# penn-graphics-research/HOT

Measured on AMD Instinct MI355X. Metric: ms per nonlinear (L-BFGS) iteration; P2G+G2P Mparticles/s; achieved HBM GB/s vs roofline, lower is better.
Workload: dtype f64; 1 GPU; C2: one 63^3-cell cube x 8 ppc (63^3 cells per GPU), fixed-corotated E=50000 nu=0.3, dx=0.01, dt=1/24, -lsolver 3 -mg_level 3 -smoother 5 -coarseSolver 2 --project --linesearch --bcproject --usecn -cneps 1e-7; particles_per_gpu=2000376, particles_total=2000376, nodes_total=267566, levels=3, parallelism=1 GPU

## Files before the change

### hot_amd/csrc/force.hip

```cpp
#include "hot_impl.h"
#include "hot_constitutive.h"
#include "hot_collision.h"
#include <cmath>

namespace hot {

template <class T>
__device__ __forceinline__ int tile_slot2(int t, const int32_t* __restrict__ nb8)
{
    using G = Geo<T>;
    constexpr int TY = G::BY + 2, TZ = G::BZ + 2;
    int tz = t % TZ, ty = (t / TZ) % TY, tx = t / (TZ * TY);
    int ox = tx >> G::xb, oy = ty >> G::yb, oz = tz >> G::zb;
    int elem = ((tx & (G::BX - 1)) << (G::yb + G::zb)) | ((ty & (G::BY - 1)) << G::zb) | (tz & (G::BZ - 1));
    return nb8[ox * 4 + oy * 2 + oz] * G::EPB + elem;
}

template <class T>
__global__ void k_hs_flag(const int32_t* __restrict__ id2coord, const double* __restrict__ hs, int nhs, int32_t* flags, int nn, T dx)
{
    int n = blockIdx.x * blockDim.x + threadIdx.x;
    if (n >= nn) return;
    bool inside = false;
    for (int h = 0; h < nhs; ++h) {
// ... 288 lines not shown
                    gv[0] += v0 * g0, gv[1] += v1 * g0, gv[2] += v2 * g0;
                    gv[3] += v0 * g1, gv[4] += v1 * g1, gv[5] += v2 * g1;
                    gv[6] += v0 * g2, gv[7] += v1 * g2, gv[8] += v2 * g2;
                }
            }
        }
        return;
    }
    T gx[3] = { 0, 0, 0 }, gy[3] = { 0, 0, 0 }, gz[3] = { 0, 0, 0 };
#pragma unroll
    for (int i = 0; i < 3; ++i) {
        T a[3] = { 0, 0, 0 }, b[3] = { 0, 0, 0 }, c[3] = { 0, 0, 0 };
#pragma unroll
        for (int j = 0; j < 3; ++j) {
            const int t = t0 + i * sx + j * sy;
            const T v0[3] = { n0[t], n0[t + 1], n0[t + 2] }, v1[3] = { n1[t], n1[t + 1], n1[t + 2] }, v2[3] = { n2[t], n2[t + 1], n2[t + 2] };
            const T s0 = w[2][0] * v0[0] + w[2][1] * v0[1] + w[2][2] * v0[2], d0 = dw[2][0] * v0[0] + dw[2][1] * v0[1] + dw[2][2] * v0[2];
            const T s1 = w[2][0] * v1[0] + w[2][1] * v1[1] + w[2][2] * v1[2], d1 = dw[2][0] * v1[0] + dw[2][1] * v1[1] + dw[2][2] * v1[2];
            const T s2 = w[2][0] * v2[0] + w[2][1] * v2[1] + w[2][2] * v2[2], d2 = dw[2][0] * v2[0] + dw[2][1] * v2[1] + dw[2][2] * v2[2];
            a[0] += w[1][j] * s0, a[1] += w[1][j] * s1, a[2] += w[1][j] * s2;
            b[0] += dw[1][j] * s0, b[1] += dw[1][j] * s1, b[2] += dw[1][j] * s2;
            c[0] += w[1][j] * d0, c[1] += w[1][j] * d1, c[2] += w[1][j] * d2;
        }
#pragma unroll
        for (int q = 0; q < 3; ++q) gx[q] += dw[0][i] * a[q], gy[q] += w[0][i] * b[q], gz[q] += w[0][i] * c[q];
    }
#pragma unroll
    for (int q = 0; q < 3; ++q) gv[q] = one_over_dx * gx[q], gv[3 + q] = one_over_dx * gy[q], gv[6 + q] = one_over_dx * gz[q];
}

template <class T, bool ENERGY_ONLY = false>
__global__ __launch_bounds__(256) __attribute__((amdgpu_waves_per_eu(ENERGY_ONLY ? (sizeof(T) == 8 ? 4 : 6) : (sizeof(T) == 8 ? 3 : 4)))) void k_state(const T* __restrict__ X, const T* __restrict__ Fn, const T* __restrict__ Vol, const T* __restrict__ Mu, const T* __restrict__ Lam,
    T* __restrict__ Ft, T* __restrict__ stress_out, T* __restrict__ gradV_out, int64_t Np, const int32_t* __restrict__ group_first, const int32_t* __restrict__ group_origin,
    const int32_t* __restrict__ group_nb, const int32_t* __restrict__ gIdx, const T* __restrict__ vn, const T* __restrict__ dv, T dx, T one_over_dx, T dt, double* energy, GridRed gr)
{
    using G = Geo<T>;
    constexpr int TY = G::BY + 2, TZ = G::BZ + 2, TILE = (G::BX + 2) * TY * TZ;
    __shared__ T nv[3][TILE];
    __shared__ double red[4];
    const int g = blockIdx.x;
    const int first = group_first[g], last = group_first[g + 1];
    const int p0 = first + threadIdx.x;
    T xpre[3] = { 0, 0, 0 }, fpre[9];
#pragma unroll
    for (int c = 0; c < 9; ++c) fpre[c] = (T)0;
    if (p0 < last) {
#pragma unroll
        for (int d = 0; d < 3; ++d) xpre[d] = X[(int64_t)d * Np + p0];
#pragma unroll
        for (int c = 0; c < 9; ++c) fpre[c] = Fn[(int64_t)c * Np + p0];
    }
    for (int t = threadIdx.x; t < TILE; t += 256) {
        int idx = gIdx[(int64_t)g * TILE + t];
        T a = 0, b = 0, c = 0;
        if (idx >= 0) a = vn[3 * idx] + dv[3 * idx], b = vn[3 * idx + 1] + dv[3 * idx + 1], c = vn[3 * idx + 2] + dv[3 * idx + 2];
        nv[0][t] = a, nv[1][t] = b, nv[2][t] = c;
    }
    __syncthreads();
    const int ox = group_origin[3 * g], oy = group_origin[3 * g + 1], oz = group_origin[3 * g + 2];
    double e = 0, es = 0;
    for (int p = first + threadIdx.x; p < last; p += 256) {
        Mat3<T> Fnew;
        {
            T xp[3];
#pragma unroll
            for (int d = 0; d < 3; ++d) xp[d] = p == p0 ? xpre[d] : X[(int64_t)d * Np + p];
            int base[3];
            T w[3][3], dw[3][3];
#pragma unroll
            for (int d = 0; d < 3; ++d) bspline<T>(one_over_dx, xp[d], base[d], w[d], dw[d]);
            const int cx = base[0] - ox, cy = base[1] - oy, cz = base[2] - oz;
            T gv[9];
            gather_grad(nv[0], nv[1], nv[2], ((cx * TY) + cy) * TZ + cz, TY * TZ, TZ, w, dw, one_over_dx, gv);
            if (gradV_out) {
#pragma unroll
                for (int c = 0; c < 9; ++c) gradV_out[(int64_t)c * Np + p] = gv[c];
            }
            Mat3<T> A, Fo;
#pragma unroll
            for (int c = 0; c < 9; ++c) A.a[c] = dt * gv[c] + ((c % 4 == 0) ? (T)1 : (T)0), Fo.a[c] = p == p0 ? fpre[c] : Fn[(int64_t)c * Np + p];
            Fnew = m3_mul(A, Fo);
        }
        T mu = Mu[p], la = Lam[p];
        T vol = Vol[p];
        if constexpr (ENERGY_ONLY) {
            e += (double)(vol * corotated_psi_sigma(Fnew, mu, la));
            continue;
        }
#pragma unroll
        for (int c = 0; c < 9; ++c) Ft[(int64_t)c * Np + p] = Fnew.a[c];
        T psi, psis;
        Mat3<T> P;
        corotated_state(Fnew, mu, la, psi, P, &psis);
        e += (double)(vol * psi);
        es += (double)(vol * psis);
        asm volatile("" ::: "memory");
#pragma unroll
        for (int c = 0; c < 3; ++c) {
            T f0 = Fn[(int64_t)(0 * 3 + c) * Np + p], f1 = Fn[(int64_t)(1 * 3 + c) * Np + p], f2 = Fn[(int64_t)(2 * 3 + c) * Np + p];
#pragma unroll
            for (int r = 0; r < 3; ++r) stress_out[(int64_t)(c * 3 + r) * Np + p] = vol * (P(r, 0) * f0 + P(r, 1) * f1 + P(r, 2) * f2);
        }
    }
    double tot = block_sum_256<double>(e, red);
    if constexpr (ENERGY_ONLY)
        grid_sum_store(tot, 0.0, 1, gr, energy, nullptr, red);
    else {
        const double tots = block_sum_256<double>(es, red);
        grid_sum_store(tot, tots, 2, gr, energy, energy + 3, red);
    }
}

template <class T, int K>
struct TrialAlphas {
    T a[K];
};
template <class T, int K>
__global__ __launch_bounds__(256) __attribute__((amdgpu_waves_per_eu(3))) void k_state_trials(const T* __restrict__ X, const T* __restrict__ Fn, const T* __restrict__ Vol,
    const T* __restrict__ Mu, const T* __restrict__ Lam, int64_t Np, const int32_t* __restrict__ group_first, const int32_t* __restrict__ group_origin, const int32_t* __restrict__ gIdx,
    const T* __restrict__ vn, const T* __restrict__ dv0, const T* __restrict__ ddv, TrialAlphas<T, K> al, T one_over_dx, T dt, double* energy, GridRed gr)
{
    using G = Geo<T>;
    constexpr int TY = G::BY + 2, TZ = G::BZ + 2, TILE = (G::BX + 2) * TY * TZ;
    __shared__ T nv[2][3][TILE];
    __shared__ double red[4 * K];
    __shared__ double esum[K][256];
    const int g = blockIdx.x;
    const int first = group_first[g], last = group_first[g + 1];
    for (int t = threadIdx.x; t < TILE; t += 256) {
        const int idx = gIdx[(int64_t)g * TILE + t];
        T a = 0, b = 0, c = 0, d0 = 0, d1 = 0, d2 = 0;
        if (idx >= 0) {
            a = vn[3 * idx] + dv0[3 * idx], b = vn[3 * idx + 1] + dv0[3 * idx + 1], c = vn[3 * idx + 2] + dv0[3 * idx + 2];
            d0 = ddv[3 * idx], d1 = ddv[3 * idx + 1], d2 = ddv[3 * idx + 2];
        }
        nv[0][0][t] = a, nv[0][1][t] = b, nv[0][2][t] = c;
        nv[1][0][t] = d0, nv[1][1][t] = d1, nv[1][2][t] = d2;
    }
    __syncthreads();
    const int ox = group_origin[3 * g], oy = group_origin[3 * g + 1], oz = group_origin[3 * g + 2];
#pragma unroll
    for (int k = 0; k < K; ++k) esum[k][threadIdx.x] = 0;
    for (int p = first + threadIdx.x; p < last; p += 256) {
        Mat3<T> A0, A1;
        {
            T xp[3];
#pragma unroll
            for (int d = 0; d < 3; ++d) xp[d] = X[(int64_t)d * Np + p];
            int base[3];
            T w[3][3], dw[3][3];
#pragma unroll
            for (int d = 0; d < 3; ++d) bspline<T>(one_over_dx, xp[d], base[d], w[d], dw[d]);
            const int t0 = (((base[0] - ox) * TY) + (base[1] - oy)) * TZ + (base[2] - oz);
            Mat3<T> Fo;
#pragma unroll
            for (int c = 0; c < 9; ++c) Fo.a[c] = Fn[(int64_t)c * Np + p];
            T gv[9];
            gather_grad(nv[0][0], nv[0][1], nv[0][2], t0, TY * TZ, TZ, w, dw, one_over_dx, gv);
            Mat3<T> A;
#pragma unroll
            for (int c = 0; c < 9; ++c) A.a[c] = dt * gv[c] + ((c % 4 == 0) ? (T)1 : (T)0);
            A0 = m3_mul(A, Fo);
#pragma unroll
            for (int d = 0; d < 3; ++d)
#pragma unroll
                for (int i = 0; i < 3; ++i) asm volatile("" : "+v"(w[d][i]), "+v"(dw[d][i]));
            gather_grad(nv[1][0], nv[1][1], nv[1][2], t0, TY * TZ, TZ, w, dw, one_over_dx, gv);
#pragma unroll
            for (int c = 0; c < 9; ++c) A.a[c] = dt * gv[c];
            A1 = m3_mul(A, Fo);
        }
        const T mu = Mu[p], la = Lam[p], vol = Vol[p];
#pragma unroll 1
        for (int k = 0; k < K; ++k) {
            T ak = al.a[0];
#pragma unroll
            for (int kk = 1; kk < K; ++kk) ak = kk == k ? al.a[kk] : ak;
            Mat3<T> Fk;
#pragma unroll
            for (int c = 0; c < 9; ++c) Fk.a[c] = A0.a[c] + ak * A1.a[c];
            esum[k][threadIdx.x] += (double)(vol * corotated_psi_sigma(Fk, mu, la));
        }
    }
    double e[K];
#pragma unroll
    for (int k = 0; k < K; ++k) e[k] = esum[k][threadIdx.x];
    block_sum_256_n<K>(e, [](int) { return true; }, red);
    grid_sum_store_n<K>(e, [](int k) { return k; }, K, gr, energy, red);
}

template <class T, int K>
__global__ __launch_bounds__(256) void k_inertia_energy_trials(const T* __restrict__ dv0, const T* __restrict__ ddv, TrialAlphas<T, K> al, const T* __restrict__ mass, int nn, T g0, T g1, T g2,
    double* out , GridRed gr, const uint8_t* __restrict__ mask )
{
    __shared__ double red[8 * K];
    double s[2 * K];
#pragma unroll
    for (int k = 0; k < 2 * K; ++k) s[k] = 0;
    const int stride = gridDim.x * 256;
    for (int n0 = blockIdx.x * 256 + threadIdx.x; n0 < nn; n0 += 4 * stride) {
        T b[4][3], d[4][3], m[4];
#pragma unroll
        for (int u = 0; u < 4; ++u) {
            const int n = n0 + u * stride < nn ? n0 + u * stride : n0;
#pragma unroll
            for (int c = 0; c < 3; ++c) b[u][c] = dv0[3 * n + c], d[u][c] = ddv[3 * n + c];
            m[u] = mass[n];
        }
#pragma unroll
        for (int u = 0; u < 4; ++u)
            if (n0 + u * stride < nn && (!mask || mask[n0 + u * stride])) {
#pragma unroll
                for (int k = 0; k < K; ++k) {
                    const T a0 = b[u][0] + d[u][0] * al.a[k], a1 = b[u][1] + d[u][1] * al.a[k], a2 = b[u][2] + d[u][2] * al.a[k];
                    s[k] += (double)((a0 * a0 + a1 * a1 + a2 * a2) * m[u]);
                    s[K + k] += (double)((g0 * a0 + g1 * a1 + g2 * a2) * m[u]);
                }
            }
    }
    block_sum_256_n<2 * K>(s, [](int) { return true; }, red);
    grid_sum_store_n<2 * K>(s, [](int k) { return k; }, 2 * K, gr, out, red);
}

template <class T>
void Ctx<T>::trial_batch(const T* ddv, T alpha, int K, double* Ek_out)
{
    HOT_CHECK(K == 2 || K == 4 || K == 8 || K == 16, HOT_ERR_INVALID, "trial_batch: 2 / 4 / 8 / 16 trials");
    if (halo_mode()) {
        halo_gather(*levels[0], dv0.p);
        halo_gather(*levels[0], const_cast<T*>(ddv));
    }
    constexpr int S0 = 140, S1 = 160;
    const int grid = std::min(div_up(Nn, 1024), 1024);
    auto run = [&](auto kc) {
        constexpr int KK = decltype(kc)::value;
        TrialAlphas<T, KK> al;
        T a = alpha;
        for (int k = 0; k < KK; ++k) al.a[k] = a, a *= (T)0.5;
        GridRed g1 = gred_n(Ng, KK);
        g1.mirror = hscal + S0;
        HOT_LAUNCH(this, KK == 2 ? "state_trials2" : (KK == 4 ? "state_trials4" : (KK == 8 ? "state_trials8" : "state_trials16")), (k_state_trials<T, KK>), Ng, 256, 0, pX.p, pFn.p, pVol.p, pMu.p, pLam.p, Np, group_first.p, group_origin.p, tileDof.p, vn.p, dv0.p, ddv, al, (T)1 / dx, dt,
            dscal.p + S0, g1);
        GridRed g2 = gred_n(grid, 2 * KK);
        g2.mirror = hscal + S1, g2.ticket = hscal + 251, g2.ticket_val = new_ticket();
        HOT_LAUNCH(this, "inertia_trials", (k_inertia_energy_trials<T, KK>), grid, 256, 0, dv0.p, ddv, al, mass.p, Nn, (T)cfg.gravity[0], (T)cfg.gravity[1], (T)cfg.gravity[2], dscal.p + S1, g2, vmask);
    };
    if (K == 2) run(std::integral_constant<int, 2>());
    else if (K == 4) run(std::integral_constant<int, 4>());
    else if (K == 8) run(std::integral_constant<int, 8>());
    else run(std::integral_constant<int, 16>());
    wait_ticket();
    if (sharded()) {
        double buf[48];
        const int nb = halo_mode() ? 3 * K : K;
        for (int k = 0; k < K; ++k) buf[k] = hscal[S0 + k];
        for (int k = 0; k < 2 * K; ++k) buf[K + k] = hscal[S1 + k];
        c_allreduce(buf, nb, HOT_COMM_F64, HOT_COMM_SUM, false);
        for (int k = 0; k < K; ++k) hscal[S0 + k] = buf[k];
        if (halo_mode())
            for (int k = 0; k < 2 * K; ++k) hscal[S1 + k] = buf[K + k];
    }
    for (int k = 0; k < K; ++k) {
        double r = (double)(T)hscal[S0 + k];
        r += hscal[S1 + k] / 2;
        r -= (double)dt * hscal[S1 + K + k];
        Ek_out[k] = r;
    }
}

#ifdef HOT_AB_KERNELS
#include "ab_src/force_ab1.hip"
#endif

#ifdef HOT_AB_KERNELS
#include "ab_src/force_ab2.hip"
#endif

template <class T>
__global__ __launch_bounds__(256) void k_inertia_energy(const T* __restrict__ dv, const T* __restrict__ mass, int nn, T g0, T g1, T g2, double* out, GridRed gr, const uint8_t* __restrict__ mask)
{
    __shared__ double red[4];
    double ke = 0, ge = 0;
    const int stride = gridDim.x * 256;
    for (int n0 = blockIdx.x * 256 + threadIdx.x; n0 < nn; n0 += 4 * stride) {
        T a[4], b[4], c[4], m[4];
#pragma unroll
        for (int u = 0; u < 4; ++u) {
            const int n = n0 + u * stride < nn ? n0 + u * stride : n0;
            a[u] = dv[3 * n], b[u] = dv[3 * n + 1], c[u] = dv[3 * n + 2], m[u] = mass[n];
        }
#pragma unroll
        for (int u = 0; u < 4; ++u)
            if (n0 + u * stride < nn && (!mask || mask[n0 + u * stride])) {
                ke += (double)((a[u] * a[u] + b[u] * b[u] + c[u] * c[u]) * m[u]);
                ge += (double)((g0 * a[u] + g1 * b[u] + g2 * c[u]) * m[u]);
            }
    }
    double k = block_sum_256<double>(ke, red);
    double gg = block_sum_256<double>(ge, red);
    grid_sum_store(k, gg, 2, gr, out, out + 1, red);
}

template <class T>
__global__ __launch_bounds__(256) void k_force_cells2(const T* __restrict__ X, const T* __restrict__ stress, int64_t Np, const int32_t* __restrict__ group_first,
    const int32_t* __restrict__ group_origin, const int32_t* __restrict__ group_cell0, const int32_t* __restrict__ cell_first, T* __restrict__ part, T one_over_dx, T scale)
{
    using G = Geo<T>;
    constexpr int TY = G::BY + 2, TZ = G::BZ + 2, TILE = (G::BX + 2) * TY * TZ, THREADS = 256;
    constexpr int CH = sizeof(T) == 4 ? 512 : 256;
    using AT = AccT<T>;
    __shared__ AT acc[3][TILE];
    __shared__ T sp[12][CH];
    __shared__ int32_t segs[G::EPB + 2];
    __shared__ int32_t nseg;
    const int g = blockIdx.x, tid = threadIdx.x;
    for (int t = tid; t < 3 * TILE; t += THREADS) (&acc[0][0])[t] = (AT)0;
    const int first = group_first[g], last = group_first[g + 1];
    const int c0 = group_cell0[g], c1 = group_cell0[g + 1];
    const int ox = group_origin[3 * g], oy = group_origin[3 * g + 1], oz = group_origin[3 * g + 2];
    for (int ch = first; ch < last; ch += CH) {
        if (tid == 0) nseg = 0;
        __syncthreads();
        for (int l = tid; l < CH && ch + l < last; l += THREADS) {
            const int p = ch + l;
#pragma unroll
            for (int c = 0; c < 9; ++c) sp[c][l] = scale * stress[(int64_t)c * Np + p];
#pragma unroll
            for (int d = 0; d < 3; ++d) sp[9 + d][l] = X[(int64_t)d * Np + p];
        }
        for (int c = c0 + tid; c < c1; c += THREADS) {
            const int s0 = max(cell_first[c], ch), s1 = min(cell_first[c + 1], min(ch + CH, last));
            if (s1 > s0) segs[atomicAdd(&nseg, 1)] = (s0 - ch) | ((s1 - ch) << 16);
        }
        __syncthreads();
        const int ni = nseg * 6;
        for (int it = tid; it < ni; it += THREADS) {
            const int sd = segs[it / 6], j = (it % 6) >> 1, hf = it & 1, s0 = sd & 0xffff, s1 = sd >> 16;
            const int mid = (s0 + s1 + 1) >> 1, l0 = hf ? mid : s0, l1 = hf ? s1 : mid;
            if (l0 >= l1) continue;
            T a[3][3][3];
#pragma unroll
            for (int e = 0; e < 27; ++e) (&a[0][0][0])[e] = (T)0;
            int b0 = 0, b1 = 0, b2 = 0;
            for (int l = l0; l < l1; ++l) {
                T wx[3], dwx[3], wy3[3], dwy3[3], wz[3], dwz[3];
                bspline<T>(one_over_dx, sp[9][l], b0, wx, dwx);
                bspline<T>(one_over_dx, sp[10][l], b1, wy3, dwy3);
                bspline<T>(one_over_dx, sp[11][l], b2, wz, dwz);
                const T wy = j == 0 ? wy3[0] : (j == 1 ? wy3[1] : wy3[2]), dwy = j == 0 ? dwy3[0] : (j == 1 ? dwy3[1] : dwy3[2]);
                T S[9];
#pragma unroll
                for (int c = 0; c < 9; ++c) S[c] = sp[c][l];
#pragma unroll
                for (int i = 0; i < 3; ++i) {
                    const T wi = wx[i], dwi = one_over_dx * dwx[i];
                    const T wij = wi * wy, dwij_i = dwi * wy, dwij_j = wi * one_over_dx * dwy;
#pragma unroll
                    for (int k = 0; k < 3; ++k) {
                        const T g0 = dwij_i * wz[k], g1 = dwij_j * wz[k], g2 = wij * one_over_dx * dwz[k];
                        a[i][k][0] += -(S[0] * g0 + S[3] * g1 + S[6] * g2);
                        a[i][k][1] += -(S[1] * g0 + S[4] * g1 + S[7] * g2);
                        a[i][k][2] += -(S[2] * g0 + S[5] * g1 + S[8] * g2);
                    }
                }
            }
#pragma unroll
            for (int i = 0; i < 3; ++i)
#pragma unroll
                for (int k = 0; k < 3; ++k) {
                    const int t = ((b0 - ox + i) * TY + (b1 - oy + j)) * TZ + (b2 - oz + k);
                    lds_atomic_add(&acc[0][t], (AT)a[i][k][0]), lds_atomic_add(&acc[1][t], (AT)a[i][k][1]), lds_atomic_add(&acc[2][t], (AT)a[i][k][2]);
                }
        }
    }
    __syncthreads();
    T* out = part + (int64_t)g * 3 * TILE;
    for (int t = tid; t < 3 * TILE; t += THREADS) out[t] = (T)(&acc[0][0])[t];
}

template <class T>
__global__ __launch_bounds__(256) void k_force_det(const T* __restrict__ X, const T* __restrict__ stress, int64_t Np, const int32_t* __restrict__ group_first,
    const int32_t* __restrict__ group_origin, const int32_t* __restrict__ group_cell0, const int32_t* __restrict__ cell_first, T* __restrict__ part, T one_over_dx, T scale)
{
    using G = Geo<T>;
    constexpr int TY = G::BY + 2, TZ = G::BZ + 2, TILE = (G::BX + 2) * TY * TZ, THREADS = 256, CH = 256;
    static_assert(TILE <= THREADS, "one thread per tile node");
    using AT = AccT<T>;
    __shared__ T sp[12][CH];
    __shared__ T slab[3][G::EPB][27];
    __shared__ int32_t segs[G::EPB];
    __shared__ int32_t stamp[G::EPB];
    __shared__ int32_t nseg;
    const int g = blockIdx.x, tid = threadIdx.x;
    const int first = group_first[g], last = group_first[g + 1], c0 = group_cell0[g], c1 = group_cell0[g + 1];
    const int ox = group_origin[3 * g], oy = group_origin[3 * g + 1], oz = group_origin[3 * g + 2];
    const int nz = tid % TZ, ny = (tid / TZ) % TY, nx = tid / (TZ * TY);
    AT acc[3] = { (AT)0, (AT)0, (AT)0 };
    if (tid < G::EPB) stamp[tid] = 0;
    for (int ch = first, n = 1; ch < last; ch += CH, ++n) {
        if (tid == 0) nseg = 0;
        __syncthreads();
        for (int l = tid; l < CH && ch + l < last; l += THREADS) {
            const int64_t p = ch + l;
#pragma unroll
            for (int c = 0; c < 9; ++c) sp[c][l] = scale * stress[(int64_t)c * Np + p];
#pragma unroll
            for (int d = 0; d < 3; ++d) sp[9 + d][l] = X[(int64_t)d * Np + p];
        }
        for (int c = c0 + tid; c < c1; c += THREADS) {
            const int s0 = max(cell_first[c], ch), s1 = min(cell_first[c + 1], min(ch + CH, last));
            if (s1 > s0) segs[atomicAdd(&nseg, 1)] = (s0 - ch) | ((s1 - ch) << 16);
        }
        __syncthreads();
        const int ni = nseg * 6;
        for (int it = tid; it < ni; it += THREADS) {
            const int sd = segs[it / 6], j = (it % 6) >> 1, hf = it & 1, s0 = sd & 0xffff, s1 = sd >> 16;
            const int mid = (s0 + s1 + 1) >> 1, l0 = hf ? mid : s0, l1 = hf ? s1 : mid;
            T a[3][3][3];
#pragma unroll
            for (int e = 0; e < 27; ++e) (&a[0][0][0])[e] = (T)0;
            const int b0 = base_node_of<T>(one_over_dx, sp[9][s0]), b1 = base_node_of<T>(one_over_dx, sp[10][s0]), b2 = base_node_of<T>(one_over_dx, sp[11][s0]);
            for (int l = l0; l < l1; ++l) {
                int e0, e1, e2;
                T wx[3], dwx[3], wy3[3], dwy3[3], wz[3], dwz[3];
                bspline<T>(one_over_dx, sp[9][l], e0, wx, dwx);
                bspline<T>(one_over_dx, sp[10][l], e1, wy3, dwy3);
                bspline<T>(one_over_dx, sp[11][l], e2, wz, dwz);
                const T wy = j == 0 ? wy3[0] : (j == 1 ? wy3[1] : wy3[2]), dwy = j == 0 ? dwy3[0] : (j == 1 ? dwy3[1] : dwy3[2]);
                T S[9];
#pragma unroll
                for (int c = 0; c < 9; ++c) S[c] = sp[c][l];
#pragma unroll
                for (int i = 0; i < 3; ++i) {
                    const T wi = wx[i], dwi = one_over_dx * dwx[i];
                    const T wij = wi * wy, dwij_i = dwi * wy, dwij_j = wi * one_over_dx * dwy;
#pragma unroll
                    for (int k = 0; k < 3; ++k) {
                        const T g0 = dwij_i * wz[k], g1 = dwij_j * wz[k], g2 = wij * one_over_dx * dwz[k];
                        a[i][k][0] += -(S[0] * g0 + S[3] * g1 + S[6] * g2);
                        a[i][k][1] += -(S[1] * g0 + S[4] * g1 + S[7] * g2);
                        a[i][k][2] += -(S[2] * g0 + S[5] * g1 + S[8] * g2);
                    }
                }
            }
#pragma unroll
            for (int e = 0; e < 27; ++e) (&a[0][0][0])[e] += dpp_move<0xb1, 0xf>((&a[0][0][0])[e]);
            const int cl = ((b0 - ox) << (G::yb + G::zb)) | ((b1 - oy) << G::zb) | (b2 - oz);
#pragma unroll
            for (int e = 0; e < 27; ++e) {
                const int ik = e / 3, q = e % 3, i = ik / 3, k = ik % 3;
                if ((e < 14) == (hf == 0)) slab[q][cl][(i * 3 + j) * 3 + k] = (&a[0][0][0])[e];
            }
            if (hf == 0 && j == 0) stamp[cl] = n;
        }
        __syncthreads();
        if (tid < TILE) {
#pragma unroll
            for (int i = 0; i < 3; ++i)
#pragma unroll
                for (int j = 0; j < 3; ++j)
#pragma unroll
                    for (int k = 0; k < 3; ++k) {
                        const int cx = nx - i, cy = ny - j, cz = nz - k;
                        if ((unsigned)cx < (unsigned)G::BX && (unsigned)cy < (unsigned)G::BY && (unsigned)cz < (unsigned)G::BZ) {
                            const int cl = (cx << (G::yb + G::zb)) | (cy << G::zb) | cz;
                            if (stamp[cl] == n) {
#pragma unroll
                                for (int q = 0; q < 3; ++q) acc[q] += (AT)slab[q][cl][(i * 3 + j) * 3 + k];
                            }
                        }
                    }
        }
    }
    if (tid < TILE) {
        T* out = part + (int64_t)g * 3 * TILE;
#pragma unroll
        for (int q = 0; q < 3; ++q) out[q * TILE + tid] = (T)acc[q];
    }
}

template <class T>
void Ctx<T>::force_pass()
{
    int64_t slots = (int64_t)Nb * EPB;
    if (cfg.deterministic)
        HOT_LAUNCH(this, "force_scatter_det", k_force_det<T>, Ng, 256, 0, pX.p, pStress.p, Np, group_first.p, group_origin.p, group_cell0.p, cell_first.p, gPart.p, (T)1 / dx, dt);
    else
#ifdef HOT_AB_KERNELS
    if (ab_flag("HOT_FORCE_V1"))
        HOT_LAUNCH(this, "force_scatter", k_force_scatter<T>, Ng, 256, 0, pX.p, pStress.p, Np, group_first.p, group_origin.p, group_nb.p, gPart.p, (T)1 / dx, dt);
    else if (ab_flag("HOT_FORCE_CELLS1"))
        HOT_LAUNCH(this, "force_scatter", k_force_cells<T>, Ng, FORCE_THREADS, 0, pX.p, pStress.p, Np, group_first.p, group_origin.p, group_cell0.p, cell_first.p, gPart.p, (T)1 / dx, dt);
    else
#endif
        HOT_LAUNCH(this, "force_scatter", k_force_cells2<T>, Ng, 256, 0, pX.p, pStress.p, Np, group_first.p, group_origin.p, group_cell0.p, cell_first.p, gPart.p, (T)1 / dx, dt);
    reduce_tiles(3, gF.p, gF.p + slots, gF.p + 2 * slots, nullptr, nullptr, "force_reduce");
    if (halo_mode()) {
        T* arr[3] = { gF.p, gF.p + slots, gF.p + 2 * slots };
        tile_exchange(arr, 3);
    }
    else if (sharded())
        allreduce_tiles(gF.p, 3);
}

template <class T>
double Ctx<T>::state_pass(const T* dv_in, bool want_force, bool energy_only)
{
    if (halo_mode()) halo_gather(*levels[0], const_cast<T*>(dv_in));
    if (energy_only)
        HOT_LAUNCH(this, "state_energy", (k_state<T, true>), Ng, 256, 0, pX.p, pFn.p, pVol.p, pMu.p, pLam.p, (T*)nullptr, (T*)nullptr, (T*)nullptr, Np, group_first.p, group_origin.p,
            group_nb.p, tileDof.p, vn.p, dv_in, dx, (T)1 / dx, dt, dscal.p, gred(Ng, hscal));
    else
        HOT_LAUNCH(this, "state_update", (k_state<T, false>), Ng, 256, 0, pX.p, pFn.p, pVol.p, pMu.p, pLam.p, pFt.p, pStress.p, keep_debug ? pGradV.p : (T*)nullptr, Np, group_first.p, group_origin.p,
            group_nb.p, tileDof.p, vn.p, dv_in, dx, (T)1 / dx, dt, dscal.p, gred2(Ng, hscal, hscal + 3));
    if (want_force) force_pass();
    {
        const int grid = std::min(div_up(Nn, 1024), 1024);
        HOT_LAUNCH(this, "inertia_energy", k_inertia_energy<T>, grid, 256, 0, dv_in, mass.p, Nn, (T)cfg.gravity[0], (T)cfg.gravity[1], (T)cfg.gravity[2], dscal.p + 1, gred(grid, hscal + 1, true), vmask);
    }
    wait_ticket();
    if (energy_only) hscal[3] = hscal[0];
    if (halo_mode())
        c_allreduce(hscal, 4, HOT_COMM_F64, HOT_COMM_SUM, false);
    else if (sharded()) {
        double two[2] = { hscal[0], hscal[3] };
        c_allreduce(two, 2, HOT_COMM_F64, HOT_COMM_SUM, false);
        hscal[0] = two[0], hscal[3] = two[1];
    }
    double result = (double)(T)hscal[0];
    result += hscal[1] / 2;
    result -= (double)dt * hscal[2];
    if (!energy_only) {
        Ek_sigma = (double)(T)hscal[3];
        Ek_sigma += hscal[1] / 2;
        Ek_sigma -= (double)dt * hscal[2];
    }
    return result;
}

template <class T>
void Ctx<T>::update_state(const void* dv_in, double* energy)
{
    need(Nn > 0 && dt > 0, "hot_update_state before hot_begin_step");
    if (dv_in) HOT_HIP(hipMemcpyAsync(dv.p, dv_in, 3 * (size_t)Nn * sizeof(T), hipMemcpyDefault, stream));
    Ek = state_pass(dv.p, true);
    if (energy) *energy = Ek;
}

template <class T>
void Ctx<T>::get_particle_state(void* F, void* stress, void* gradV)
{
    need(Np > 0, "no particles");
    int64_t n = Np;
    DBuf<T> tmp;
    tmp.reserve(9 * n);
    auto out = [&](const T* src, void* dst) {
        if (!dst) return;
        HOT_HIP(hipMemcpyAsync(tmp.p, src, 9 * n * sizeof(T), hipMemcpyDeviceToDevice, stream));
        std::vector<T> h(9 * n), o(9 * n);
        std::vector<int32_t> s2o(n);
        HOT_HIP(hipMemcpyAsync(h.data(), tmp.p, 9 * n * sizeof(T), hipMemcpyDeviceToHost, stream));
        HOT_HIP(hipMemcpyAsync(s2o.data(), slot2orig.p, n * sizeof(int32_t), hipMemcpyDeviceToHost, stream));
        sync();
        for (int64_t p = 0; p < n; ++p)
            for (int c = 0; c < 9; ++c) o[(int64_t)s2o[p] * 9 + c] = h[(int64_t)c * n + p];
        HOT_HIP(hipMemcpy(dst, o.data(), 9 * n * sizeof(T), hipMemcpyDefault));
    };
    out(pFt.p, F), out(pStress.p, stress), out(pGradV.p, gradV);
}

template <class T>
__device__ __forceinline__ void mat3_vec(const T* __restrict__ M, const T* v, T* o)
{
    o[0] = M[0] * v[0] + M[3] * v[1] + M[6] * v[2];
    o[1] = M[1] * v[0] + M[4] * v[1] + M[7] * v[2];
    o[2] = M[2] * v[0] + M[5] * v[1] + M[8] * v[2];
}
template <class T>
__device__ __forceinline__ void bc_project(int c, const T* __restrict__ P, const uint8_t* __restrict__ slip, bool slipmode, T* v)
{
    if (slipmode) {
        if (slip[c])
            v[0] = (T)0;
        else
            v[0] = v[1] = v[2] = (T)0;
    }
    else {
        T o[3];
        mat3_vec(P + 9 * c, v, o);
        v[0] = o[0], v[1] = o[1], v[2] = o[2];
    }
}

template <class T>
__global__ void k_residual(const T* __restrict__ gF, const int32_t* __restrict__ dofSlot, const T* __restrict__ mass, const T* __restrict__ dv, const int32_t* __restrict__ bcIdx,
    const T* __restrict__ bcP, const T* __restrict__ bcR, const uint8_t* __restrict__ bcSlip, T* r, T* r2 , int nn, int64_t slots, T g0, T g1, T g2, T dt, int slipmode)
{
    int n = blockIdx.x * blockDim.x + threadIdx.x;
    if (n >= nn) return;
    int64_t s = dofSlot[n];
    T m = mass[n];
    T v[3] = { g0 * dt * m + gF[s] - dv[3 * n] * m, g1 * dt * m + gF[slots + s] - dv[3 * n + 1] * m, g2 * dt * m + gF[2 * slots + s] - dv[3 * n + 2] * m };
    int c = bcIdx[n];
    if (c >= 0) {
        if (slipmode && bcSlip[c]) {
            T o[3];
            mat3_vec(bcR + 9 * c, v, o);
            v[0] = o[0], v[1] = o[1], v[2] = o[2];
        }
        bc_project(c, bcP, bcSlip, slipmode != 0, v);
    }
    r[3 * n] = v[0], r[3 * n + 1] = v[1], r[3 * n + 2] = v[2];
    r2[3 * n] = v[0], r2[3 * n + 1] = v[1], r2[3 * n + 2] = v[2];
}
template <class T>
__global__ void k_project(const int32_t* __restrict__ bcNode, const T* __restrict__ bcP, const uint8_t* __restrict__ bcSlip, T* v, int nc, int slipmode)
{
    int c = blockIdx.x * blockDim.x + threadIdx.x;
    if (c >= nc) return;
    int n = bcNode[c];
    T x[3] = { v[3 * n], v[3 * n + 1], v[3 * n + 2] };
    bc_project(c, bcP, bcSlip, slipmode != 0, x);
    v[3 * n] = x[0], v[3 * n + 1] = x[1], v[3 * n + 2] = x[2];
}
template <class T>
__global__ void k_transform(const int32_t* __restrict__ bcNode, const T* __restrict__ M, const uint8_t* __restrict__ bcSlip, T* v, int nc)
{
    int c = blockIdx.x * blockDim.x + threadIdx.x;
    if (c >= nc || !bcSlip[c]) return;
    int n = bcNode[c];
    T x[3] = { v[3 * n], v[3 * n + 1], v[3 * n + 2] }, o[3];
    mat3_vec(M + 9 * c, x, o);
    v[3 * n] = o[0], v[3 * n + 1] = o[1], v[3 * n + 2] = o[2];
}

template <class T>
void Ctx<T>::residual_dev(T* r)
{
    int slipmode = (cfg.systemBCProject && cfg.boundaryType == 1) ? 1 : 0;
    HOT_LAUNCH(this, "residual", k_residual<T>, div_up(Nn, 256), 256, 0, gF.p, dofSlot.p, mass.p, dv.p, bcIdx.p, bcP.p, bcR.p, bcSlip.p, r, rhs.p, Nn, (int64_t)Nb * EPB, (T)cfg.gravity[0],
        (T)cfg.gravity[1], (T)cfg.gravity[2], dt, slipmode);
}
template <class T>
void Ctx<T>::project_dev(T* v)
{
    if (Nc == 0) return;
    int slipmode = (cfg.systemBCProject && cfg.boundaryType == 1) ? 1 : 0;
    HOT_LAUNCH(this, "project", k_project<T>, div_up(Nc, 256), 256, 0, bcNode.p, bcP.p, bcSlip.p, v, Nc, slipmode);
}
template <class T>
void Ctx<T>::transform_dev(T* v, bool inverse)
{
    if (Nc == 0 || !(cfg.systemBCProject && cfg.boundaryType == 1)) return;
    HOT_LAUNCH(this, "transform", k_transform<T>, div_up(Nc, 256), 256, 0, bcNode.p, inverse ? bcRinv.p : bcR.p, bcSlip.p, v, Nc);
}

template <class T>
void Ctx<T>::residual(void* r)
{
    need(Nn > 0 && dt > 0, "hot_residual before hot_begin_step/hot_update_state");
    residual_dev(work0.p);
    if (halo_mode()) gather_all(*levels[0], work0.p);
    download(r, work0.p, 3 * (size_t)Nn);
    sync();
}
template <class T>
void Ctx<T>::project(void* v)
{
    need(Nn > 0, "no grid");
    HOT_HIP(hipMemcpyAsync(work0.p, v, 3 * (size_t)Nn * sizeof(T), hipMemcpyDefault, stream));
    project_dev(work0.p);
    download(v, work0.p, 3 * (size_t)Nn);
    sync();
}

template <class T>
__global__ void k_cn_tol(const T* __restrict__ gCN, const int32_t* __restrict__ dofSlot, const T* __restrict__ mass, T* tol, int nn, T scale)
{
    int n = blockIdx.x * blockDim.x + threadIdx.x;
    if (n < nn) tol[n] = gCN[dofSlot[n]] * scale / mass[n];
}
template <class T>
__global__ __launch_bounds__(256) void k_max_dpdf(const T* __restrict__ Mu, const T* __restrict__ Lam, int64_t np, unsigned long long* out)
{
    __shared__ double red[4];
    double mx = 0;
    for (int64_t p = (int64_t)blockIdx.x * 256 + threadIdx.x; p < np; p += (int64_t)gridDim.x * 256) {
        T mu = Mu[p], la = Lam[p];
        double v = (double)hsqrt((T)3 * ((T)2 * mu + la) * ((T)2 * mu + la) + (T)6 * la * la + (T)12 * mu * mu);
        mx = v > mx ? v : mx;
    }
    for (int o = 32; o > 0; o >>= 1) {
        double other = __shfl_xor(mx, o, 64);
        mx = other > mx ? other : mx;
    }
    if ((threadIdx.x & 63) == 0) red[threadIdx.x >> 6] = mx;
    __syncthreads();
    if (threadIdx.x == 0) {
        for (int k = 1; k < 4; ++k) mx = red[k] > mx ? red[k] : mx;
        atomicMax(out, (unsigned long long)__double_as_longlong(mx));
    }
}
template <class T>
void Ctx<T>::cn_tolerance_dev()
{
    T scale = (T)cfg.cneps * 24 * dx * dx * dt;
    HOT_LAUNCH(this, "cn_tolerance", k_cn_tol<T>, div_up(Nn, 256), 256, 0, gCN.p, dofSlot.p, mass.p, cnTol.p, Nn, scale);
    HOT_HIP(hipMemsetAsync(dscal.p + 8, 0, sizeof(double), stream));
    HOT_LAUNCH(this, "max_dpdf_norm", k_max_dpdf<T>, std::min(div_up(Np, 256), 1024), 256, 0, pMu.p, pLam.p, Np, (unsigned long long*)(dscal.p + 8));
    HOT_HIP(hipMemcpyAsync(hscal + 8, dscal.p + 8, sizeof(double), hipMemcpyDeviceToHost, stream));
    sync();
    if (sharded()) c_allreduce(hscal + 8, 1, HOT_COMM_F64, HOT_COMM_MAX, false);
    max_cn_tolerance = (T)cfg.cneps * dt * 24 * (T)std::sqrt((double)Nn) * dx * dx * (T)hscal[8];
}
template <class T>
void Ctx<T>::cn_tolerance(void* tol)
{
    need(Nn > 0 && dt > 0, "hot_cn_tolerance before hot_begin_step");
    need(cfg.useCN, "hot_cn_tolerance needs cfg.useCN (the accumulation is fused into P2G)");
    cn_tolerance_dev();
    if (halo_mode()) gather_all(*levels[0], cnTol.p, 1);
    download(tol, cnTol.p, Nn);
    sync();
}

template <class T>
__global__ __launch_bounds__(256) void k_matfree(const T* __restrict__ X, const T* __restrict__ Fn, const T* __restrict__ Ft, const T* __restrict__ Vol, const T* __restrict__ Mu,
    const T* __restrict__ Lam, int64_t Np, const int32_t* __restrict__ group_first, const int32_t* __restrict__ group_origin, const int32_t* __restrict__ group_nb,
    const int32_t* __restrict__ gIdx, const T* __restrict__ x, T* __restrict__ part, T dx, T one_over_dx, T dt, int project)
{
    using G = Geo<T>;
    constexpr int TY = G::BY + 2, TZ = G::BZ + 2, TILE = (G::BX + 2) * TY * TZ;
    __shared__ T nv[3][TILE];
    using AT = AccT<T>;
    __shared__ AT acc[3][TILE];
    __shared__ int32_t nb8[8];
    const int g = blockIdx.x;
    if (threadIdx.x < 8) nb8[threadIdx.x] = group_nb[g * 8 + threadIdx.x];
    __syncthreads();
    for (int t = threadIdx.x; t < TILE; t += 256) {
        int idx = gIdx[tile_slot2<T>(t, nb8)];
        T a = 0, b = 0, c = 0;
        if (idx >= 0) a = x[3 * idx], b = x[3 * idx + 1], c = x[3 * idx + 2];
        nv[0][t] = a, nv[1][t] = b, nv[2][t] = c;
        acc[0][t] = acc[1][t] = acc[2][t] = (AT)0;
    }
    __syncthreads();
    const int first = group_first[g], last = group_first[g + 1];
    const int ox = group_origin[3 * g], oy = group_origin[3 * g + 1], oz = group_origin[3 * g + 2];
    for (int p = first + threadIdx.x; p < last; p += 256) {
        T xp[3] = { X[p], X[Np + p], X[2 * Np + p] };
        int base[3];
        T w[3][3], dw[3][3];
#pragma unroll
        for (int d = 0; d < 3; ++d) bspline<T>(one_over_dx, xp[d], base[d], w[d], dw[d]);
        const int cx = base[0] - ox, cy = base[1] - oy, cz = base[2] - oz;
        Mat3<T> gx;
#pragma unroll
        for (int c = 0; c < 9; ++c) gx.a[c] = (T)0;
#pragma unroll
        for (int i = 0; i < 3; ++i)
#pragma unroll
            for (int j = 0; j < 3; ++j)
#pragma unroll
                for (int k = 0; k < 3; ++k) {
                    T g0 = one_over_dx * dw[0][i] * w[1][j] * w[2][k], g1 = w[0][i] * one_over_dx * dw[1][j] * w[2][k], g2 = w[0][i] * w[1][j] * one_over_dx * dw[2][k];
                    int t = ((cx + i) * TY + (cy + j)) * TZ + (cz + k);
                    T v0 = nv[0][t], v1 = nv[1][t], v2 = nv[2][t];
                    gx.a[0] += v0 * g0, gx.a[1] += v1 * g0, gx.a[2] += v2 * g0;
                    gx.a[3] += v0 * g1, gx.a[4] += v1 * g1, gx.a[5] += v2 * g1;
                    gx.a[6] += v0 * g2, gx.a[7] += v1 * g2, gx.a[8] += v2 * g2;
                }
        Mat3<T> Fo, Fc;
#pragma unroll
        for (int c = 0; c < 9; ++c) Fo.a[c] = Fn[(int64_t)c * Np + p], Fc.a[c] = Ft[(int64_t)c * Np + p];
        HessBlocks<T> h;
        corotated_hessian(Fc, Mu[p], Lam[p], project != 0, h);
        Mat3<T> dP = hess_apply(h, m3_mul(gx, Fo));
        T vol = Vol[p];
        Mat3<T> S;
#pragma unroll
        for (int c = 0; c < 3; ++c)
#pragma unroll
            for (int r = 0; r < 3; ++r) S(r, c) = vol * (dP(r, 0) * Fo(c, 0) + dP(r, 1) * Fo(c, 1) + dP(r, 2) * Fo(c, 2));
        T sc = dt * dt;
        for (int n = 0; n < 27; ++n) {
            int i = n / 9, j = (n / 3) % 3, k = n % 3;
            T g0 = one_over_dx * dw[0][i] * w[1][j] * w[2][k], g1 = w[0][i] * one_over_dx * dw[1][j] * w[2][k], g2 = w[0][i] * w[1][j] * one_over_dx * dw[2][k];
            int t = ((cx + i) * TY + (cy + j)) * TZ + (cz + k);
            lds_atomic_add(&acc[0][t], (AT)(sc * (S(0, 0) * g0 + S(0, 1) * g1 + S(0, 2) * g2)));
            lds_atomic_add(&acc[1][t], (AT)(sc * (S(1, 0) * g0 + S(1, 1) * g1 + S(1, 2) * g2)));
            lds_atomic_add(&acc[2][t], (AT)(sc * (S(2, 0) * g0 + S(2, 1) * g1 + S(2, 2) * g2)));
        }
    }
    __syncthreads();
    T* out = part + (int64_t)g * 3 * TILE;
    for (int t = threadIdx.x; t < 3 * TILE; t += 256) out[t] = (T)(&acc[0][0])[t];
}
template <class T>
__global__ __launch_bounds__(256) void k_matfree_stress_det(const T* __restrict__ X, const T* __restrict__ Fn, const T* __restrict__ Ft, const T* __restrict__ Vol, const T* __restrict__ Mu,
    const T* __restrict__ Lam, int64_t Np, const int32_t* __restrict__ group_first, const int32_t* __restrict__ group_origin, const int32_t* __restrict__ group_nb,
    const int32_t* __restrict__ gIdx, const T* __restrict__ x, T* __restrict__ out, T one_over_dx, int project)
{
    using G = Geo<T>;
    constexpr int TY = G::BY + 2, TZ = G::BZ + 2, TILE = (G::BX + 2) * TY * TZ;
    __shared__ T nv[3][TILE];
    __shared__ int32_t nb8[8];
    const int g = blockIdx.x;
    if (threadIdx.x < 8) nb8[threadIdx.x] = group_nb[g * 8 + threadIdx.x];
    __syncthreads();
    for (int t = threadIdx.x; t < TILE; t += 256) {
        int idx = gIdx[tile_slot2<T>(t, nb8)];
        T a = 0, b = 0, c = 0;
        if (idx >= 0) a = x[3 * idx], b = x[3 * idx + 1], c = x[3 * idx + 2];
        nv[0][t] = a, nv[1][t] = b, nv[2][t] = c;
    }
    __syncthreads();
    const int first = group_first[g], last = group_first[g + 1];
    const int ox = group_origin[3 * g], oy = group_origin[3 * g + 1], oz = group_origin[3 * g + 2];
    for (int p = first + threadIdx.x; p < last; p += 256) {
        T xp[3] = { X[p], X[Np + p], X[2 * Np + p] };
        int base[3];
        T w[3][3], dw[3][3];
#pragma unroll
        for (int d = 0; d < 3; ++d) bspline<T>(one_over_dx, xp[d], base[d], w[d], dw[d]);
        const int cx = base[0] - ox, cy = base[1] - oy, cz = base[2] - oz;
        Mat3<T> gx;
#pragma unroll
        for (int c = 0; c < 9; ++c) gx.a[c] = (T)0;
#pragma unroll
        for (int i = 0; i < 3; ++i)
#pragma unroll
            for (int j = 0; j < 3; ++j)
#pragma unroll
                for (int k = 0; k < 3; ++k) {
                    T g0 = one_over_dx * dw[0][i] * w[1][j] * w[2][k], g1 = w[0][i] * one_over_dx * dw[1][j] * w[2][k], g2 = w[0][i] * w[1][j] * one_over_dx * dw[2][k];
                    int t = ((cx + i) * TY + (cy + j)) * TZ + (cz + k);
                    T v0 = nv[0][t], v1 = nv[1][t], v2 = nv[2][t];
                    gx.a[0] += v0 * g0, gx.a[1] += v1 * g0, gx.a[2] += v2 * g0;
                    gx.a[3] += v0 * g1, gx.a[4] += v1 * g1, gx.a[5] += v2 * g1;
                    gx.a[6] += v0 * g2, gx.a[7] += v1 * g2, gx.a[8] += v2 * g2;
                }
        Mat3<T> Fo, Fc;
#pragma unroll
        for (int c = 0; c < 9; ++c) Fo.a[c] = Fn[(int64_t)c * Np + p], Fc.a[c] = Ft[(int64_t)c * Np + p];
        HessBlocks<T> h;
        corotated_hessian(Fc, Mu[p], Lam[p], project != 0, h);
        Mat3<T> dP = hess_apply(h, m3_mul(gx, Fo));
        T vol = Vol[p];
#pragma unroll
        for (int c = 0; c < 3; ++c)
#pragma unroll
            for (int r = 0; r < 3; ++r) out[(int64_t)(c * 3 + r) * Np + p] = vol * (dP(r, 0) * Fo(c, 0) + dP(r, 1) * Fo(c, 1) + dP(r, 2) * Fo(c, 2));
    }
}

template <class T>
__global__ void k_matfree_finish(const T* __restrict__ gOut, const int32_t* __restrict__ dofSlot, const T* __restrict__ mass, const T* __restrict__ x, T* y, int nn, int64_t slots)
{
    int n = blockIdx.x * blockDim.x + threadIdx.x;
    if (n >= nn) return;
    int64_t s = dofSlot[n];
    T m = mass[n];
    y[3 * n] = m * x[3 * n] + gOut[s], y[3 * n + 1] = m * x[3 * n + 1] + gOut[slots + s], y[3 * n + 2] = m * x[3 * n + 2] + gOut[2 * slots + s];
}

template <class T>
void Ctx<T>::matfree_dev(const T* x, T* y)
{
    int64_t slots = (int64_t)Nb * EPB;
    DBuf<T>& tile = ap;
    tile.reserve(3 * slots);
    if (halo_mode()) halo_gather(*levels[0], const_cast<T*>(x));
    if (cfg.deterministic) {
        pMfS.reserve(9 * (size_t)Np);
        HOT_LAUNCH(this, "matfree_stress_det", k_matfree_stress_det<T>, Ng, 256, 0, pX.p, pFn.p, pFt.p, pVol.p, pMu.p, pLam.p, Np, group_first.p, group_origin.p, group_nb.p, gIdx.p, x, pMfS.p,
            (T)1 / dx, cfg.project);
        HOT_LAUNCH(this, "matfree_hessian_product_det", k_force_det<T>, Ng, 256, 0, pX.p, pMfS.p, Np, group_first.p, group_origin.p, group_cell0.p, cell_first.p, gPart.p, (T)1 / dx, -dt * dt);
    }
    else
        HOT_LAUNCH(this, "matfree_hessian_product", k_matfree<T>, Ng, 256, 0, pX.p, pFn.p, pFt.p, pVol.p, pMu.p, pLam.p, Np, group_first.p, group_origin.p, group_nb.p, gIdx.p, x, gPart.p, dx,
            (T)1 / dx, dt, cfg.project);
    reduce_tiles(3, tile.p, tile.p + slots, tile.p + 2 * slots, nullptr, nullptr, "matfree_reduce");
    if (halo_mode()) {
        T* arr[3] = { tile.p, tile.p + slots, tile.p + 2 * slots };
        tile_exchange(arr, 3);
    }
    else if (sharded())
        allreduce_tiles(tile.p, 3);
    HOT_LAUNCH(this, "matfree_finish", k_matfree_finish<T>, div_up(Nn, 256), 256, 0, tile.p, dofSlot.p, mass.p, x, y, Nn, slots);
}
template <class T>
void Ctx<T>::matfree_multiply(const void* x, void* y)
{
    need(Nn > 0 && dt > 0, "hot_matfree_multiply before hot_update_state");
    HOT_HIP(hipMemcpyAsync(work0.p, x, 3 * (size_t)Nn * sizeof(T), hipMemcpyDefault, stream));
    matfree_dev(work0.p, work1.p);
    if (halo_mode()) gather_all(*levels[0], work1.p);
    download(y, work1.p, 3 * (size_t)Nn);
    sync();
}

template struct Ctx<float>;
template struct Ctx<double>;

}
```

### hot_amd/csrc/hot_impl.h

```cpp
#pragma once
#include "hot_ctx.h"
#include <atomic>
#include <functional>

namespace hot {

template <class T>
struct GsImg {
    static constexpr size_t hdr_elems = 2 * 64 * 9;
    static constexpr size_t cap_entries = 1340 + 1;
    static constexpr size_t per_dir = cap_entries * 9, per_block = hdr_elems + 2 * per_dir;
    static constexpr size_t idx_per_dir = 64 * 64;
};

struct GsPlan {
    enum Path {
        CHAINED,
        COLOUR,
        PAIR,
        PER_COLOUR,
        SIMPLE,
    } path;
    int sb;
    int nmerge;
// ... 9 lines not shown
template <class T>
__host__ __device__ inline int home_rank(const uint64_t* split, int R, int x, int y, int z, int level)
{
    using G = Geo<T>;
    const uint64_t page = G::linear_offset((x & ~3) << level, (y & ~3) << level, (z & ~3) << level) >> 12;
    int r = 0;
    while (r < R - 1 && page >= split[r]) ++r;
    return r;
}

template <class T>
struct Level {
    int n = 0;
    int id = 0;
    bool built = false;
    long long nnzb = 0;
    DBuf<int32_t> coord;
    DBuf<int32_t> col;
    DBuf<T> val;
    DBuf<T> diagVal, diagInv;
    DBuf<T> diagBlockInv;
    DBuf<uint32_t> ckey;
    DBuf<int32_t> gs_order;
    DBuf<int32_t> gs_block_start;
    double lMin = 1e-8, lMax = 1e2;
    DBuf<T> apv;
    DBuf<int32_t> apc;
    DBuf<int32_t> gs_pad;
    DBuf<int32_t> gs_col;
    DBuf<T> gs_img;
    DBuf<uint16_t> gs_imgi;
    DBuf<T> gs_p1;
    DBuf<int2> gs_slot;
    int gs_nslot = 0;
    int32_t gs_slot_rng[2][2][8] = {};
    DBuf<int32_t> gs_rowpn;
    DBuf<int4> gs_srec;
    int32_t gs_slot_rng2[4][2][8] = {};
    bool gs_fused_ready = false;
    bool gs_img_ready = false;
    long long gs_img_shift[8] = {};
    DBuf<T> gs_w;
    bool gs_w_ready = false;
    DBuf<int32_t> rowcnt;
    bool split = false;
    DBuf<int32_t> ic_col, ic_rowcnt, ic_pad;
    DBuf<T> ic_val, ic_l, ic_d, ic_dinv, ic_dinvT;
    bool ic_ready = false;
    double ic_shift = 0;
    int color_block_begin[9] = { 0 };
    int nblocks = 0;
    DBuf<int32_t> pcol;
    DBuf<T> pw;
    DBuf<int32_t> child;
    DBuf<uint64_t> hkeys;
    DBuf<unsigned long long> hrank;
    DBuf<int32_t> hid;
    HashMap map;
    DBuf<T> residual, initialResidual, sol, du, dAu, tmp;
    bool colored = false;
    bool part = false;
    std::vector<int> nstart;
    DBuf<uint8_t> owner;
    DBuf<uint8_t> own;
    DBuf<uint8_t> block_owner;
    std::vector<uint8_t> block_owner_h;
    std::vector<int> csplit;
    std::pair<int, int> colour_run(int c, int rank, int ranks) const
    {
        const int b0 = color_block_begin[c];
        if (!part) return { b0, color_block_begin[c + 1] };
        return { b0 + csplit[c * (ranks + 1) + rank], b0 + csplit[c * (ranks + 1) + rank + 1] };
    }
    std::vector<int> xbeg, xcnt;
    DBuf<int32_t> dxtab;
    int xmax_full = 0, xmax_col[8] = { 0 };
    const uint8_t* mask() const { return part ? own.p : nullptr; }
    DBuf<T> gsD, gsDinv, gsE;
    bool l1 = false;
    const T* gs_d() const { return l1 ? gsD.p : diagVal.p; }
    const T* gs_dinv() const { return l1 ? gsDinv.p : diagBlockInv.p; }
    struct Halo {
        bool built = false;
        std::vector<int64_t> scnt, soff, rcnt, roff;
        std::vector<int64_t> scol, rcol;
        DBuf<int32_t> send, recv;
        DBuf<uint8_t> need;
        int64_t stot = 0, rtot = 0;
    } halo;
};

template <class T>
struct Ctx : CtxBase {
    using G = Geo<T>;
    static constexpr int EPB = G::EPB;
    static constexpr int TX = G::BX + 2, TY = G::BY + 2, TZ = G::BZ + 2, TILE = TX * TY * TZ;

    T dx = 0, dt = 0;
    int64_t Np = 0;
    DBuf<T> pX, pV, pM, pC, pF, pVol, pMu, pLam, pJp, pFn, pFt, pStress, pGradV;
    DBuf<int32_t> slot2orig;
    DBuf<int32_t> pGid;
    DBuf<int32_t> pCls;
    bool have_cls = false;
    int ncls = 0;
    hot_plasticity_class cls_host[16] = {};
    DBuf<T> clsTab;
    void clear_plasticity_classes() { have_cls = false, ncls = 0; }
    int32_t max_particle_class(int32_t* min_out);
    void reserve_particles(int64_t n);
    void migrate_particles();
    void set_particle_ids(const int32_t* ids) override;
    void get_particle_ids(int32_t* ids) override;
    DBuf<T> spare1, spare3, spare9;
    DBuf<int32_t> sparei;
    bool keep_debug = true;
    DBuf<uint64_t> keys, keys2;
    DBuf<uint32_t> vals, vals2;
    DBuf<char> sort_tmp;
    size_t sort_tmp_bytes = 0;
    DBuf<int32_t> flags, scan;
    DBuf<char> scan_tmp;
    size_t scan_tmp_bytes = 0;
    int Ng = 0, Nb = 0, Nn = 0;
    DBuf<int32_t> group_first;
    DBuf<uint64_t> group_page;
    DBuf<int32_t> group_nb;
    DBuf<int32_t> group_origin;
    DBuf<uint64_t> blocks;
    DBuf<uint64_t> bh_keys;
    DBuf<unsigned long long> bh_rank;
    DBuf<int32_t> bh_id;
    HashMap block_map;
    int Ncell = 0;
    DBuf<int32_t> cell_first;
    DBuf<int32_t> group_cell0;
    DBuf<uint64_t> ch_keys;
    DBuf<unsigned long long> ch_rank;
    DBuf<int32_t> ch_id;
    HashMap cell_map;
    DBuf<T> pMfS;
    DBuf<T> pDP;
    void build_cell_table();
    void matfree_diagonal(T* dinv);
    void assemble_tiles(Level<T>& L);
    void assemble_rows(Level<T>& L);
    void build_gs_winv(Level<T>& L);
    DBuf<int32_t> tile_tab;
    DBuf<int32_t> block_group;
    DBuf<int32_t> block_rev;
    DBuf<T> gPart;
    void reduce_tiles(int Q, T* o0, T* o1, T* o2, T* o3, T* o4, const char* name);
    DBuf<T> gM, gMV, gF, gCN;
    DBuf<int32_t> gIdx;
    DBuf<int32_t> tileDof;
    DBuf<int32_t> block_count;
    DBuf<int32_t> dofSlot, id2coord, bcIdx;
    DBuf<T> mass, vn, dv, dv0, cnTol, nodeV;
    int Nc = 0;
    DBuf<int32_t> bcNode;
    DBuf<T> bcP, bcR, bcRinv, bcDv;
    DBuf<uint8_t> bcSlip, bcHasDv;
    std::vector<double> hs_origin, hs_normal;
    std::vector<hot_collision_object> cobjs;
    DBuf<char> d_cobjs;
    DBuf<double> d_hs;
    double Ek = 0, Ek_sigma = 0;
    bool updated = false;
    int ls_prev_trials = 1;
    T max_cn_tolerance = 0;
    DBuf<T> rhs, work0, work1, work2, work3, solve_keep;
    hot_comm comm{};
    bool sharded() const { return comm.size > 1; }
    std::vector<int> block_first;
    std::vector<uint64_t> page_split;
    std::vector<int> nstart0;
    DBuf<char> xsend, xrecv;
    DBuf<uint8_t> written;
    void set_comm(const hot_comm* c) override;
    void write_partio(const char* path) override;
    void write_restart(const char* path) override;
    void read_restart(const char* path) override;
    void c_allreduce(void* buf, int64_t n, int dtype, int op, bool on_device);
    void c_allgather(const void* send, void* recv, int64_t bytes, bool on_device);
    void c_alltoallv(const void* send, const int64_t* soff, const int64_t* sbytes, void* recv, const int64_t* roff, const int64_t* rbytes);
    void merge_block_lists();
    void color_level(Level<T>& L);
    void level_ownership(Level<T>& L);
    void exchange(Level<T>& L, T* x, int colour, int ncomp = 3);
    void exchange_rows(Level<T>& L, const uint8_t* touched);
    void allreduce_tiles(T* tiles, int q);
    bool halo_mode() const { return sharded() && !cfg.shard_replicated; }
    int64_t comm_calls = 0, comm_calls_index = 0, comm_bytes_index = 0, comm_bytes_data = 0;
    bool comm_index_phase = false;
    struct IndexPhase {
        Ctx<T>* c;
        bool old;
        IndexPhase(Ctx<T>* c_) : c(c_), old(c_->comm_index_phase) { c->comm_index_phase = true; }
        ~IndexPhase() { c->comm_index_phase = old; }
    };
    const char* comm_tag = "other";
    struct CommTag {
        Ctx<T>* c;
        const char* old;
        CommTag(Ctx<T>* c_, const char* t) : c(c_), old(c_->comm_tag) { c->comm_tag = t; }
        ~CommTag() { c->comm_tag = old; }
    };
    void account(int64_t bytes)
    {
        ++comm_calls, comm_calls_index += comm_index_phase ? 1 : 0, (comm_index_phase ? comm_bytes_index : comm_bytes_data) += bytes;
        if (prof.on) {
            auto& r = prof.recs[std::string("commMB_") + (comm_index_phase ? "index" : comm_tag)];
            r.calls++, r.ms += (double)bytes * 1e-6;
        }
    }
    void export_comm_stats() { stats.comm_calls = comm_calls, stats.comm_calls_index = comm_calls_index, stats.comm_bytes_index = comm_bytes_index, stats.comm_bytes_data = comm_bytes_data; }
    DBuf<uint8_t> touch;
    DBuf<uint64_t> sharers;
    DBuf<int32_t> tpos;
    DBuf<int32_t> tlist;
    std::vector<int64_t> tcnt, toff;
    void build_tile_plan();
    void tile_exchange(T* const* arrays, int q);
    void build_halo(Level<T>& L, const std::function<void(uint8_t*)>& mark_extra);
    void halo_gather(Level<T>& L, T* x, int colour = -1, int ncomp = 3);
    void gather_colour(Level<T>& L, T* x, int colour, int ncomp);
    void gather_all(Level<T>& L, T* x, int ncomp = 3);
    void replicate_numbering();
    void level0_ownership();
    void mark_stencil(Level<T>& L, uint8_t* need);
    const uint8_t* vmask = nullptr;
    struct MaskScope {
        Ctx<T>* c;
        const uint8_t* old;
        MaskScope(Ctx<T>* c_, const uint8_t* m) : c(c_), old(c_->vmask) { c->vmask = m; }
        ~MaskScope() { c->vmask = old; }
    };
    void reduce_scalars(double* dev, int n)
    {
        if (!vmask || n <= 0) return;
        CommTag tag(this, "scalars");
        c_allreduce(dev, n, HOT_COMM_F64, HOT_COMM_SUM, true);
    }
    static constexpr int REAL = sizeof(T) == 4 ? HOT_COMM_F32 : HOT_COMM_F64;
    DBuf<double> dscal;
    DBuf<T> speed_part;
    DBuf<double> red_part;
    DBuf<unsigned> red_count;
    GridRed gred(size_t grid, double* mirror = nullptr, bool ticket = false)
    {
        if (2 * grid > red_part.cap) {
            HOT_HIP(hipStreamSynchronize(stream));
            red_part.reserve(2 * grid, 1.5);
        }
        GridRed g{ red_part.p, red_count.p, mirror, nullptr, 0.0 };
        if (ticket) g.ticket = hscal + 251, g.ticket_val = new_ticket();
        return g;
    }
    GridRed gred2(size_t grid, double* mirror, double* mirror1)
    {
        GridRed g = gred(grid, mirror);
        g.mirror1 = mirror1;
        return g;
    }
    GridRed gred_n(size_t grid, int nv)
    {
        if ((size_t)nv * grid > red_part.cap) {
            HOT_HIP(hipStreamSynchronize(stream));
            red_part.reserve((size_t)nv * grid, 1.5);
        }
        return GridRed{ red_part.p, red_count.p, nullptr, nullptr, 0.0 };
    }
    double last_ticket = 0;
    double new_ticket() { return last_ticket += 1.0; }
    void wait_ticket()
    {
        const double want = last_ticket;
        volatile double* t = hscal + 251;
        const double t0 = wall_ms();
        for (unsigned spin = 0; *t != want; ++spin) {
            __builtin_ia32_pause();
            if ((spin & 1023u) == 1023u && wall_ms() - t0 > 20.0) {
                HOT_HIP(hipStreamSynchronize(stream));
                if (*(volatile int*)(hscal + 250) != 0) sync();
                HOT_CHECK(*t == want, HOT_ERR_DEVICE, "a reduction launch did not deliver its result");
                break;
            }
        }
        std::atomic_thread_fence(std::memory_order_acquire);
        if (*(volatile int*)(hscal + 250) != 0) sync();
    }
    DBuf<uint64_t> col_hk;
    DBuf<unsigned long long> col_hr;
    DBuf<int32_t> col_hi, col_cb;
    bool cg_bar_dirty = false;
    DBuf<double> cg_dep;
    unsigned cg_phase = 0;
    int cg_G = 0;
    bool attr_cg_set = false;
    int cg_group = 2;
    bool attr_tiles_set = false, attr_rows_set = false, attr_rows_det_set = false, attr_gs_set = false, attr_winv_set = false;
    double* hscal = nullptr;
    DBuf<T> hist_dx[9], hist_dg[9];
    std::vector<Level<T>*> levels;
    std::vector<Level<T>*> level_pool[12];
    Level<T>* acquire_level(int id)
    {
        Level<T>* l;
        if (!level_pool[id].empty()) {
            l = level_pool[id].back();
            level_pool[id].pop_back();
        }
        else
            l = new Level<T>();
        l->id = id, l->n = 0, l->nnzb = 0, l->nblocks = 0, l->built = false, l->split = false, l->part = false, l->colored = false, l->halo.built = false, l->ic_ready = false;
        return l;
    }
    void release_levels(size_t keep = 0)
    {
        while (levels.size() > keep) {
            Level<T>* l = levels.back();
            levels.pop_back();
            level_pool[l->id < 12 ? l->id : 11].push_back(l);
        }
    }
    DBuf<T> ap;
    std::vector<Ctx<T>*> gmg;
    DBuf<int32_t> orig2slot;
    Ctx<T>* build_gmg_grid(int level);

    Ctx(const hot_config& c);
    ~Ctx();
    template <class U>
    void upload(DBuf<U>& dst, const void* src, size_t n)
    {
        dst.reserve(n);
        if (n) HOT_HIP(hipMemcpyAsync(dst.p, src, n * sizeof(U), hipMemcpyDefault, stream));
    }
    template <class U>
    void download(void* dst, const U* src, size_t n)
    {
        if (dst && n) HOT_HIP(hipMemcpyAsync(dst, src, n * sizeof(U), hipMemcpyDefault, stream));
    }
    static constexpr int ERR_RETRY = -100;
    static constexpr int REARM_STEPS = 32, MAX_TIMEOUTS = 3;
    bool gs_no_chain = false, gs_chain_timed_out = false;
    int gs_timeouts = 0, steps_since_timeout = 0;
    void rearm_chain()
    {
        if (!gs_chain_timed_out || gs_timeouts >= MAX_TIMEOUTS || ++steps_since_timeout < REARM_STEPS) return;
        gs_chain_timed_out = false, steps_since_timeout = 0;
        if (!sharded()) gs_no_chain = false;
    }
    int n_cu = 0;
    int device_cus()
    {
        if (n_cu == 0) {
            int dev = 0;
            HOT_HIP(hipGetDevice(&dev));
            HOT_HIP(hipDeviceGetAttribute(&n_cu, hipDeviceAttributeMultiprocessorCount, dev));
        }
        return n_cu;
    }
    int unset_level = -1;
    int retry_scope = 0, fake_syncs = 0;
    void sync()
    {
        HOT_HIP(hipStreamSynchronize(stream));
        if (retry_scope > 0 && !gs_no_chain && ab_int("HOT_GS_FAKE_TIMEOUT", 0) > 0 && ++fake_syncs == ab_int("HOT_GS_FAKE_TIMEOUT", 0)) *(volatile int*)(hscal + 250) = 1;
        if (*(volatile int*)(hscal + 250) != 0) {
            *(volatile int*)(hscal + 250) = 0;
            cg_bar_dirty = true;
            ++gs_timeouts, steps_since_timeout = 0;
            if (cfg.deterministic) {
                if (gs_timeouts > MAX_TIMEOUTS)
                    throw Error{ HOT_ERR_DEVICE, "deterministic mode: a chained Gauss-Seidel sweep or persistent PCG timed out more than 3 times on this context; the launch-per-pass fallback would change the bits, so the operation fails" };
                throw Error{ ERR_RETRY, "k_gs_sweep: wait on a neighbouring block timed out; deterministic mode: redoing the operation with the same launch structure" };
            }
            gs_no_chain = gs_chain_timed_out = true;
            throw Error{ ERR_RETRY, "k_gs_sweep: wait on a neighbouring block timed out; redoing the operation with one launch per pass" };
        }
    }
    template <class Fn>
    void with_gs_retry(Fn&& fn)
    {
        struct Scope {
            int& n;
            Scope(int& n_) : n(n_) { ++n; }
            ~Scope() { --n; }
        } scope(retry_scope);
        for (;;) {
            try {
                fn();
                return;
            }
            catch (const Error& e) {
                if (e.code != ERR_RETRY) throw;
                if (!cfg.deterministic) break;
            }
        }
        fn();
    }
    int32_t exclusive_scan_i32(const int32_t* in, int32_t* out, size_t n);
    void need(bool cond, const char* what) { HOT_CHECK(cond, HOT_ERR_INVALID, what); }

    void set_particles(int64_t Np, const void* X, const void* V, const void* mass, const void* C, const void* F, const void* vol, const void* mu, const void* lambda, const void* Jp) override;
    void get_particles(void* X, void* V, void* C, void* F, void* mu, void* lambda, void* Jp) override;
    void sort() override;
    void get_counts(int64_t* Np, int32_t* Ng, int32_t* Nb, int32_t* Nn) override;
    void get_indexing(int32_t* order, uint64_t* base_offset, int32_t* group, uint64_t* block_offset, uint64_t* blocks) override;
    void p2g() override;
    void get_grid(int32_t* id2coord, void* mass, void* v) override;
    void set_bc(int32_t Nc, const int32_t* node_id, const void* P, const void* R, const void* Rinv, const uint8_t* slip, const void* dvc) override;
    void set_halfspaces(int32_t n, const double* origin, const double* normal) override;
    void set_collision_objects(int32_t n, const hot_collision_object* objs) override;
    void begin_step(double dt) override;
    void get_dv(void* dv) override;
    void set_dv(const void* dv) override;
    void update_state(const void* dv, double* energy) override;
    void get_particle_state(void* F, void* stress, void* gradV) override;
    void residual(void* r) override;
    void project(void* v) override;
    void cn_tolerance(void* tol) override;
    void build_hessian() override;
    void matfree_multiply(const void* x, void* y) override;
    void build_mg() override;
    void get_level(int32_t level, int32_t* nrows, int32_t* colsize, int32_t* id2coord) override;
    void get_matrix(int32_t level, int32_t* entryCol, void* entryVal) override;
    long long get_level_nnzb(int32_t level) override
    {
        need(level >= 0 && level < (int)levels.size(), "level out of range");
        if (levels[level]->nnzb < 0) count_nnzb(*levels[level]);
        return levels[level]->nnzb;
    }
    long long get_level_inblock_nnzb(int32_t level) override
    {
        need(level >= 0 && level < (int)levels.size() && levels[level]->split, "hot_get_level_inblock_nnzb: level out of range or not coloured (hot_build_mg)");
        Level<T>& L = *levels[level];
        std::vector<int32_t> rc(4 * (size_t)L.n);
        HOT_HIP(hipMemcpyAsync(rc.data(), L.rowcnt.p, rc.size() * sizeof(int32_t), hipMemcpyDeviceToHost, stream));
        sync();
        long long tot = 0;
        for (int i = 0; i < L.n; ++i) tot += rc[4 * (size_t)i + 1] + rc[4 * (size_t)i + 2];
        return tot;
    }
    void get_prolongation(int32_t level, int32_t* entryCol, void* weight) override;
    void spmv(int32_t level, const void* x, void* y) override;
    void restrict_(int32_t level, const void* fine, void* coarse) override;
    void prolong(int32_t level, const void* coarse, void* fine) override;
    void smooth(int32_t level, int32_t kind, int32_t iterations, double tol, void* u, void* r, const void* r0) override;
    void vcycle(const void* in, void* out) override;
    void solve(hot_stats* st) override;
    void g2p(double dt, int32_t* flags) override;
    void constitutive_eval(int32_t n, const void* F, const void* mu, const void* lambda, int32_t project, void* psi, void* P, void* dPdF) override;
    void plasticity_eval(int32_t kind, int32_t n, void* F, void* mu, void* lambda, void* Jp) override;
    void set_plasticity_classes(int32_t n, const hot_plasticity_class* classes, const int32_t* particle_class) override;
    void get_plasticity_classes(int32_t* n, hot_plasticity_class* classes, int32_t* particle_class) override;
    void plasticity_eval_classes(int32_t n, void* F, void* mu, void* lambda, void* Jp, const int32_t* cls) override;
    void advance(double dt, hot_stats* st) override;
    void calculate_dt(double max_dt, double* dt, double* max_speed, double* min_corner, double* max_corner) override;
    void advance_frame(double frame_dt, double min_dt, double max_dt, int32_t* substeps, int32_t* iterations_total, hot_stats* st) override;

    void eval_halfspaces();
    void eval_collision_objects();
    void trial_batch(const T* ddv, T alpha, int K, double* Ek_out);
    double state_pass(const T* dv_in, bool want_force, bool energy_only = false);
    void force_pass();
    void residual_dev(T* r);
    void project_dev(T* v);
    void transform_dev(T* v, bool inverse);
    void cn_tolerance_dev();
    void build_diagonal(Level<T>& L);
    void build_ic(Level<T>& L);
    void count_nnzb(Level<T>& L);
    std::string lname(const char* base, int level) { return std::string(base) + "_L" + std::to_string(level); }
    void spmv_dev(Level<T>& L, const T* x, T* y);
    void scale_dev(Level<T>& L, const T* in, T* out);
    void block_apply_dev(const T* D, const T* in, T* out, int n);
    void estimate_2norm(Level<T>& L, double tol);
    int minres_dev(const std::function<void(const T*, T*)>& Amul, const std::function<void(const T*, T*)>& prec, T* x, const T* b, T relative_tolerance, T tolerance, int max_iterations);
    void scal(size_t n, T a, T* x);
    int smoother_kind(int level, bool top = false) const;
    GsPlan gs_plan(const Level<T>& L) const;
    GsBuild gs_build(const Level<T>& L) const;
    bool gs_marks_wanted(int level) const;
    void restrict_dev(int level, const T* fine, T* coarse, T* zero_coarse = nullptr);
    void prolong_dev(int level, const T* coarse, T* fine);
    void smooth_dev(int level, int kind, int iterations, T tol, T* u, T* r, T* du, T* dAu, bool final_residual = true);
    void gs_smooth_dev(int level, int iterations, T* u, T* r, T* du, T* dAu, bool final_residual, bool tmp_marked);
    void ic_smooth_dev(Level<T>& L, T* u, T* r, T* dAu);
    void vcycle_dev(const T* in, T* out);
    void precondition_dev(const T* in, T* out);
    void matfree_dev(const T* x, T* y);
    void axpy(size_t n, T a, const T* x, T* y);
    void axpy_dev(size_t n, const double* a, double sign, const T* x, T* y);
    void copy(size_t n, const T* x, T* y);
    void zero(size_t n, T* y);
    void dot_to(size_t n, const T* x, const T* y, double* out, double* mirror = nullptr);
    double dot_host(size_t n, const T* x, const T* y);
    bool should_exit(const T* r);
    T line_search(T* ddv, T* residual_out, T alpha);
    bool lbfgs_solve();
    bool newton_solve();
    void compute_step_dev(const T* residual, T* step);
    DBuf<T> nw_step, nw_r, nw_p, nw_q, nw_t, nw_diag;
    void line_search_api(void* ddv, void* residual, double alpha, double* alpha_out) override;
    void should_exit_api(const void* residual, int32_t* exit_now, double* scaled) override;
    void transform_api(void* v, bool inverse) override;
    void compute_step_api(const void* residual, void* step) override;
};

inline int div_up(size_t a, size_t b) { return (int)((a + b - 1) / b); }

__device__ __forceinline__ int xcd_block() { return (int)((blockIdx.x & 7) * (gridDim.x >> 3) + (blockIdx.x >> 3)); }
static inline int xcd_grid(int nwg) { return 8 * div_up(nwg, 8); }
template <class U>
__device__ __forceinline__ U nt_load(const U* p)
{
    return *p;
}
template <class T>
struct GsUnset;
template <>
struct GsUnset<double> {
    static constexpr unsigned long long bits = 0x7ff4dead0badf00dull;
    static __device__ __forceinline__ bool is(double v) { return (unsigned long long)__double_as_longlong(v) == bits; }
};
template <>
struct GsUnset<float> {
    static constexpr unsigned bits = 0x7fa0f00du;
    static __device__ __forceinline__ bool is(float v) { return (unsigned)__float_as_int(v) == bits; }
};
template <class T>
__device__ __forceinline__ void gs_store_unset(T* p)
{
    if constexpr (sizeof(T) == 8)
        *(unsigned long long*)p = GsUnset<double>::bits;
    else
        *(unsigned*)p = GsUnset<float>::bits;
}
template <class T>
__global__ void k_gs_fill_unset(size_t n, T* x);

#define HOT_LAUNCH(ctx, name, kernel, grid, block, shmem, ...)                       \
    do {                                                                             \
        (ctx)->prof.begin(name, (ctx)->stream);                                      \
        hipLaunchKernelGGL(kernel, dim3(grid), dim3(block), shmem, (ctx)->stream, __VA_ARGS__); \
        (ctx)->prof.end((ctx)->stream);                                              \
    } while (0)

}
```

### hot_amd/csrc/mg_solve.hip

```cpp
#include "hot_impl.h"
#include "hot_svd.h"

namespace hot {

template <class T>
__global__ void k_axpy(size_t n, T a, const T* __restrict__ x, T* y)
{
    size_t i = (size_t)blockIdx.x * blockDim.x + threadIdx.x;
    if (i < n) y[i] += a * x[i];
}
template <class T>
__global__ void k_axpy_dev(size_t n, const double* a, double sign, const T* __restrict__ x, T* y)
{
    size_t i = (size_t)blockIdx.x * blockDim.x + threadIdx.x;
    T s = (T)(sign * (*a));
    if (i < n) y[i] += s * x[i];
}
template <class T>
__global__ void k_xpay_dev(size_t n, const double* a, const T* __restrict__ x, T* y)
{
    size_t i = (size_t)blockIdx.x * blockDim.x + threadIdx.x;
    T s = (T)(*a);
    if (i < n) y[i] = x[i] + s * y[i];
}
template <class T>
__global__ __launch_bounds__(256) void k_dot(size_t n, const T* __restrict__ x, const T* __restrict__ y, double* out, GridRed gr, const uint8_t* __restrict__ mask)
{
    __shared__ double red[4];
    double s = 0;
    const size_t stride = (size_t)gridDim.x * 256;
    for (size_t i0 = (size_t)blockIdx.x * 256 + threadIdx.x; i0 < n; i0 += 4 * stride) {
        T xv[4], yv[4];
        bool on[4];
#pragma unroll
        for (int u = 0; u < 4; ++u) {
            const size_t i = i0 + u * stride, ic = i < n ? i : i0;
            on[u] = i < n && (!mask || mask[ic / 3]);
            xv[u] = on[u] ? x[ic] : (T)0, yv[u] = on[u] ? y[ic] : (T)0;
        }
#pragma unroll
        for (int u = 0; u < 4; ++u)
            if (on[u]) s += (double)(xv[u] * yv[u]);
    }
    double t = block_sum_256<double>(s, red);
    grid_sum_store(t, 0.0, 1, gr, out, nullptr, red);
}
template <class T>
void Ctx<T>::axpy(size_t n, T a, const T* x, T* y)
{
    HOT_LAUNCH(this, "axpy", k_axpy<T>, div_up(n, 256), 256, 0, n, a, x, y);
}
template <class T>
void Ctx<T>::axpy_dev(size_t n, const double* a, double sign, const T* x, T* y)
{
    HOT_LAUNCH(this, "axpy", k_axpy_dev<T>, div_up(n, 256), 256, 0, n, a, sign, x, y);
}
template <class T>
__global__ __launch_bounds__(256) void k_copy(size_t n, const T* __restrict__ x, T* __restrict__ y)
{
    for (size_t i = (size_t)blockIdx.x * 256 + threadIdx.x; i < n; i += (size_t)gridDim.x * 256) y[i] = x[i];
}
template <class T>
__global__ __launch_bounds__(256) void k_vcycle_start(size_t n, const T* __restrict__ x, T* __restrict__ y, T* __restrict__ y2, T* __restrict__ z)
{
    for (size_t i = (size_t)blockIdx.x * 256 + threadIdx.x; i < n; i += (size_t)gridDim.x * 256) {
        const T v = x[i];
        y[i] = v, z[i] = (T)0;
        if (y2) y2[i] = v;
    }
}
template <class T>
void Ctx<T>::copy(size_t n, const T* x, T* y)
{
    if (n) HOT_LAUNCH(this, "copy", k_copy<T>, (int)std::min<size_t>(div_up(n, 256), 2048), 256, 0, n, x, y);
}
template <class T>
void Ctx<T>::zero(size_t n, T* y)
{
    HOT_HIP(hipMemsetAsync(y, 0, n * sizeof(T), stream));
}
template <class T>
void Ctx<T>::dot_to(size_t n, const T* x, const T* y, double* out, double* mirror)
{
    const int grid = std::min(div_up(n, 1024), 256);
    if (vmask) {
        HOT_LAUNCH(this, "dot", k_dot<T>, grid, 256, 0, n, x, y, out, gred(grid), vmask);
        reduce_scalars(out, 1);
        if (mirror) HOT_HIP(hipMemcpyAsync(mirror, out, sizeof(double), hipMemcpyDeviceToHost, stream));
        return;
    }
    HOT_LAUNCH(this, "dot", k_dot<T>, grid, 256, 0, n, x, y, out, gred(grid, mirror), (const uint8_t*)nullptr);
}
template <class T>
double Ctx<T>::dot_host(size_t n, const T* x, const T* y)
{
    const int grid = std::min(div_up(n, 1024), 256);
    HOT_LAUNCH(this, "dot", k_dot<T>, grid, 256, 0, n, x, y, dscal.p + 100, gred(grid, hscal + 100, true), vmask);
    wait_ticket();
    if (vmask) c_allreduce(hscal + 100, 1, HOT_COMM_F64, HOT_COMM_SUM, false);
    return hscal[100];
}

template <class T>
__global__ __launch_bounds__(256) void k_spmv(const int32_t* __restrict__ col, const T* __restrict__ val, const T* __restrict__ x, T* __restrict__ y, int n, const uint8_t* __restrict__ own)
{
    const int lane = threadIdx.x & 63;
    const int row = xcd_block() * 4 + (threadIdx.x >> 6);
    if (row >= n || (own && !own[row])) return;
    const int32_t* c = col + (int64_t)row * 125;
    const T* v = val + (int64_t)row * 1125;
    T s0 = 0, s1 = 0, s2 = 0;
#pragma unroll
    for (int r = 0; r < 2; ++r) {
        int k = lane + 64 * r;
        if (k < 125) {
            int j = c[k];
            const T* b = v + k * 9;
            T x0 = x[3 * (int64_t)j], x1 = x[3 * (int64_t)j + 1], x2 = x[3 * (int64_t)j + 2];
            s0 += b[0] * x0 + b[3] * x1 + b[6] * x2;
            s1 += b[1] * x0 + b[4] * x1 + b[7] * x2;
            s2 += b[2] * x0 + b[5] * x1 + b[8] * x2;
        }
    }
    s0 = wave_sum(s0), s1 = wave_sum(s1), s2 = wave_sum(s2);
    if (lane == 0) y[3 * (int64_t)row] = s0, y[3 * (int64_t)row + 1] = s1, y[3 * (int64_t)row + 2] = s2;
}
template <class T>
__global__ __launch_bounds__(256) void k_apmv_sub(const int32_t* __restrict__ apc, const T* __restrict__ apv, const T* __restrict__ e, T* __restrict__ r, int n, const uint8_t* __restrict__ own,
    T* unset )
{
    const int lane = threadIdx.x & 63;
    const int row = xcd_block() * 4 + (threadIdx.x >> 6);
    if (row >= n) return;
    if (unset && lane < 3) gs_store_unset(unset + 3 * (int64_t)row + lane);
    if (own && !own[row]) return;
    const int j = nt_load(apc + (int64_t)row * 64 + lane);
    const int slot = __popcll(__ballot(j >= 0) & ((1ull << lane) - 1ull));
    T s0 = (T)0, s1 = (T)0, s2 = (T)0;
    if (j >= 0) {
        const T* bp = apv + ((int64_t)row * 64 + slot) * 9;
        T b[9];
#pragma unroll
        for (int t = 0; t < 9; ++t) b[t] = nt_load(bp + t);
        const T x0 = e[3 * (int64_t)j], x1 = e[3 * (int64_t)j + 1], x2 = e[3 * (int64_t)j + 2];
        s0 = b[0] * x0 + b[3] * x1 + b[6] * x2;
        s1 = b[1] * x0 + b[4] * x1 + b[7] * x2;
        s2 = b[2] * x0 + b[5] * x1 + b[8] * x2;
    }
    s0 = wave_sum(s0), s1 = wave_sum(s1), s2 = wave_sum(s2);
    if (lane == 0) r[3 * (int64_t)row] -= s0, r[3 * (int64_t)row + 1] -= s1, r[3 * (int64_t)row + 2] -= s2;
}
__device__ __forceinline__ bool cg_active(double zTr, double tol) { return !(zTr < tol); }
template <class T>
__global__ void k_cg_setup(double* s, double* hm)
{
    const double tol = (double)(T)(s[7] * 0.25);
    s[8] = tol;
    s[1] = s[2] = s[3] = s[4] = s[5] = s[6] = s[9] = 0.0;
    hm[0] = s[0], hm[1] = 0.0, hm[2] = tol;
}
template <class T>
__global__ __launch_bounds__(256) void k_cg_spmv_dot(const int32_t* __restrict__ col, const T* __restrict__ val, const T* __restrict__ du, T* __restrict__ dAu, int n, double* s, GridRed gr)
{
    __shared__ double red[4];
    const bool roll = s[6] != 0.0;
    const double cur = roll ? s[4] : s[0];
    if (blockIdx.x == 0 && threadIdx.x == 0 && roll) s[0] = s[4];
    if (!cg_active(cur, s[8])) return;
    const int lane = threadIdx.x & 63;
    const int row = blockIdx.x * 4 + (threadIdx.x >> 6);
    double part = 0;
    if (row < n) {
        const int32_t* c = col + (int64_t)row * 125;
        const T* v = val + (int64_t)row * 1125;
        T s0 = 0, s1 = 0, s2 = 0;
#pragma unroll
        for (int r = 0; r < 2; ++r) {
            int k = lane + 64 * r;
            if (k < 125) {
                int j = c[k];
                const T* b = v + k * 9;
                T x0 = du[3 * (int64_t)j], x1 = du[3 * (int64_t)j + 1], x2 = du[3 * (int64_t)j + 2];
                s0 += b[0] * x0 + b[3] * x1 + b[6] * x2;
                s1 += b[1] * x0 + b[4] * x1 + b[7] * x2;
                s2 += b[2] * x0 + b[5] * x1 + b[8] * x2;
            }
        }
        s0 = wave_sum(s0), s1 = wave_sum(s1), s2 = wave_sum(s2);
        if (lane == 0) {
            dAu[3 * (int64_t)row] = s0, dAu[3 * (int64_t)row + 1] = s1, dAu[3 * (int64_t)row + 2] = s2;
            part = (double)(s0 * du[3 * (int64_t)row]) + (double)(s1 * du[3 * (int64_t)row + 1]) + (double)(s2 * du[3 * (int64_t)row + 2]);
        }
    }
    if (lane == 0) red[threadIdx.x >> 6] = part;
    __syncthreads();
    const double t = threadIdx.x == 0 ? red[0] + red[1] + red[2] + red[3] : 0.0;
    __syncthreads();
    grid_sum_store(t, 0.0, 1, gr, s + 1, nullptr, red);
}
template <class T>
__global__ __launch_bounds__(256) void k_cg_update(const T* __restrict__ Dinv, const T* __restrict__ du, const T* __restrict__ dAu, T* __restrict__ u, T* __restrict__ r, T* __restrict__ z, int n, double* s, GridRed gr)
{
    __shared__ double red[4];
    const int i = blockIdx.x * 256 + threadIdx.x;
    if (!cg_active(s[0], s[8])) return;
    const double omega = s[0] / s[1];
    const T wp = (T)omega, wm = (T)(-omega);
    double part = 0;
    if (i < n) {
        T rr[3];
#pragma unroll
        for (int c = 0; c < 3; ++c) {
            u[3 * (int64_t)i + c] += wp * du[3 * (int64_t)i + c];
            rr[c] = r[3 * (int64_t)i + c] + wm * dAu[3 * (int64_t)i + c];
            r[3 * (int64_t)i + c] = rr[c];
        }
        const T* d = Dinv + 9 * (int64_t)i;
        const T z0 = d[0] * rr[0] + d[3] * rr[1] + d[6] * rr[2], z1 = d[1] * rr[0] + d[4] * rr[1] + d[7] * rr[2], z2 = d[2] * rr[0] + d[5] * rr[1] + d[8] * rr[2];
        z[3 * (int64_t)i] = z0, z[3 * (int64_t)i + 1] = z1, z[3 * (int64_t)i + 2] = z2;
        part = (double)(z0 * rr[0]) + (double)(z1 * rr[1]) + (double)(z2 * rr[2]);
    }
    const double t = block_sum_256<double>(part, red);
    grid_sum_store(t, 0.0, 1, gr, s + 4, nullptr, red);
}
template <class T>
__global__ void k_cg_direction(size_t n3, const T* __restrict__ z, T* __restrict__ du, double* s, double* hm, double* ticket, double ticket_val)
{
    const size_t i = (size_t)blockIdx.x * blockDim.x + threadIdx.x;
    const bool act = cg_active(s[0], s[8]);
    if (act && i < n3) du[i] = z[i] + (T)(s[4] / s[0]) * du[i];
    if (i == 0) {
        if (act) {
            s[6] = 1.0;
            const double cnt = s[9] + 1.0;
            s[9] = cnt;
            hm[0] = s[4], hm[1] = cnt;
        }
        if (ticket) host_ticket_store(ticket, ticket_val);
    }
}
template <class T, int RPW = 0>
__global__ __launch_bounds__(1024) void k_cg_persist(const int32_t* __restrict__ col, const T* __restrict__ val, const T* __restrict__ Dinv, const T* __restrict__ init, T* __restrict__ u,
    T* __restrict__ r, T* __restrict__ z, T* du, T* __restrict__ dAu, int n, int max_iters, unsigned phase0 , double* dep , int SS , double* hm, double* ticket, double ticket_val,
    int* err )
{
    __shared__ double red[32], sres[2];
    __shared__ int s_bail;
    enum { CG_DI = 0, CG_U = 9, CG_R = 12, CG_Z = 15, CG_D = 18, CG_AD = 21 };
    __shared__ T cg_row[RPW > 0 ? 16 : 1][RPW > 0 ? RPW : 1][24];
    const int tid = threadIdx.x, lane = tid & 63, w = __builtin_amdgcn_readfirstlane(tid >> 6);
    const int G = gridDim.x, wg = blockIdx.x;
    unsigned phase = phase0;
    if (tid == 0) s_bail = 0;
    auto ldu = [&](int64_t j, int c) { return __hip_atomic_load(du + 3 * j + c, __ATOMIC_RELAXED, __HIP_MEMORY_SCOPE_AGENT); };
    auto sdu = [&](int64_t j, int c, T v) { __hip_atomic_store(du + 3 * j + c, v, __ATOMIC_RELAXED, __HIP_MEMORY_SCOPE_AGENT); };
    auto all_sum = [&](double v0, double v1, double& o0, double& o1) -> bool {
        asm volatile("s_waitcnt vmcnt(0)" ::: "memory");
        if (lane == 0) red[w] = v0, red[16 + w] = v1;
        __syncthreads();
        double* d = dep + (size_t)(phase & 3u) * G * SS;
        if (tid == 0) {
            double t0 = 0, t1 = 0;
            for (int k = 0; k < 16; ++k) t0 += red[k], t1 += red[16 + k];
            double* dn = dep + (size_t)((phase + 2u) & 3u) * G * SS + (size_t)wg * SS;
            __hip_atomic_store((unsigned long long*)dn, GsUnset<double>::bits, __ATOMIC_RELAXED, __HIP_MEMORY_SCOPE_AGENT);
            __hip_atomic_store((unsigned long long*)(dn + 1), GsUnset<double>::bits, __ATOMIC_RELAXED, __HIP_MEMORY_SCOPE_AGENT);
            __hip_atomic_store(d + (size_t)wg * SS, t0, __ATOMIC_RELAXED, __HIP_MEMORY_SCOPE_AGENT);
            __hip_atomic_store(d + (size_t)wg * SS + 1, t1, __ATOMIC_RELAXED, __HIP_MEMORY_SCOPE_AGENT);
        }
        if (w < 2) {
            const double* dv = d + w;
            double a = 0;
            int spins = 0, bail = 0;
            for (;;) {
                bool all = true;
                a = 0;
                for (int k = lane; k < G; k += 64) {
                    const double x = __hip_atomic_load(dv + (size_t)k * SS, __ATOMIC_RELAXED, __HIP_MEMORY_SCOPE_AGENT);
                    all = all && !GsUnset<double>::is(x);
                    a += x;
                }
                if (__all(all)) break;
                __builtin_amdgcn_s_sleep(1);
                if (++spins > (1 << 21) || ((spins & 255) == 0 && *(volatile int*)err)) {
                    *(volatile int*)err = 1;
                    bail = 1;
                    break;
                }
            }
            a = wave_sum(a);
            if (lane == 0) {
                sres[w] = a;
                if (bail) s_bail = 1;
            }
        }
        __syncthreads();
        if (s_bail) return false;
        o0 = wave_first(sres[0]), o1 = wave_first(sres[1]);
        ++phase;
        return true;
    };
    auto scale = [&](int64_t i, const T (&v)[3], T (&o)[3]) {
        const T* d = Dinv + 9 * i;
        o[0] = d[0] * v[0] + d[3] * v[1] + d[6] * v[2], o[1] = d[1] * v[0] + d[4] * v[1] + d[7] * v[2], o[2] = d[2] * v[0] + d[5] * v[1] + d[8] * v[2];
    };
    const int stride = 16 * G;
    if constexpr (RPW > 0) {
        int rowq[RPW];
        int32_t mc[RPW][2];
        T mv[RPW][2][9];
        double p0 = 0, p1 = 0;
#pragma unroll
        for (int q = 0; q < RPW; ++q) {
            const int row = wg * 16 + w + q * stride;
            rowq[q] = row < n ? row : -1;
            const int64_t rc = row < n ? row : 0;
#pragma unroll
            for (int h = 0; h < 2; ++h) {
                const int k = min(lane + 64 * h, 124);
                mc[q][h] = col[rc * 125 + k];
#pragma unroll
                for (int e = 0; e < 9; ++e) mv[q][h][e] = (lane + 64 * h < 125) ? val[rc * 1125 + k * 9 + e] : (T)0;
            }
            if (lane == 0) {
                T* st = cg_row[w][q];
                T di[9], a[3], za[3], rr[3], zz[3];
#pragma unroll
                for (int e = 0; e < 9; ++e) di[e] = Dinv[9 * rc + e], st[CG_DI + e] = di[e];
#pragma unroll
                for (int c = 0; c < 3; ++c) a[c] = init[3 * rc + c], rr[c] = r[3 * rc + c], st[CG_U + c] = u[3 * rc + c], st[CG_AD + c] = (T)0;
#pragma unroll
                for (int c = 0; c < 3; ++c) za[c] = di[c] * a[0] + di[3 + c] * a[1] + di[6 + c] * a[2], zz[c] = di[c] * rr[0] + di[3 + c] * rr[1] + di[6 + c] * rr[2];
                if (rowq[q] >= 0) {
                    p0 += (double)(za[0] * a[0]) + (double)(za[1] * a[1]) + (double)(za[2] * a[2]);
                    p1 += (double)(zz[0] * rr[0]) + (double)(zz[1] * rr[1]) + (double)(zz[2] * rr[2]);
                    for (int c = 0; c < 3; ++c) sdu(row, c, zz[c]);
                }
#pragma unroll
                for (int c = 0; c < 3; ++c) st[CG_R + c] = rr[c], st[CG_Z + c] = zz[c], st[CG_D + c] = zz[c];
            }
        }
        double zTr0, zTr;
        if (!all_sum(p0, p1, zTr0, zTr)) return;
        const double tol = (double)(T)(zTr0 * 0.25);
        extern __shared__ double cg_lds[];
        T* ldsdu = (T*)cg_lds;
        const int n3 = 3 * n;
        auto pull_du = [&]() {
            const int n16 = n3 >> 1;
            for (int e0 = 0; e0 < n16; e0 += 4 * 1024) {
                double2 v[4];
#pragma unroll
                for (int k = 0; k < 4; ++k) {
                    const unsigned eb = 16u * (unsigned)min(e0 + k * 1024 + tid, n16 - 1);
                    asm volatile("global_load_dwordx4 %0, %1, %2 sc0 sc1" : "=v"(v[k]) : "v"(eb), "s"(du) : "memory");
                }
                asm volatile("s_waitcnt vmcnt(0)" ::: "memory");
#pragma unroll
                for (int k = 0; k < 4; ++k) {
                    const int e = e0 + k * 1024 + tid;
                    if (e < n16) ((double2*)ldsdu)[e] = v[k];
                }
            }
            if ((n3 & 1) && tid == 0) ldsdu[n3 - 1] = ldu(n - 1, 2);
            __syncthreads();
        };
        int cnt = 0;
#ifdef HOT_AB_KERNELS
        unsigned long long tk[8] = { 0, 0, 0, 0, 0, 0, 0, 0 }, t0_ = wall_clock64();
#define CG_TK(i) \
    do { \
        const unsigned long long t_ = wall_clock64(); \
        tk[i] += t_ - t0_, t0_ = t_; \
    } while (0)
#else
#define CG_TK(i)
#endif
        for (; cnt < max_iters && cg_active(zTr, tol); ++cnt) {
            pull_du();
            CG_TK(0);
            double pd = 0;
#pragma unroll
            for (int q = 0; q < RPW; ++q) {
                T s0 = 0, s1 = 0, s2 = 0;
#pragma unroll
                for (int h = 0; h < 2; ++h) {
                    if (lane + 64 * h < 125) {
                        const int j = mc[q][h];
                        const T* b = mv[q][h];
                        const T x0 = ldsdu[3 * j], x1 = ldsdu[3 * j + 1], x2 = ldsdu[3 * j + 2];
                        s0 += b[0] * x0 + b[3] * x1 + b[6] * x2;
                        s1 += b[1] * x0 + b[4] * x1 + b[7] * x2;
                        s2 += b[2] * x0 + b[5] * x1 + b[8] * x2;
                    }
                }
                s0 = wave_sum(s0), s1 = wave_sum(s1), s2 = wave_sum(s2);
                if (lane == 0) {
                    T* st = cg_row[w][q];
                    st[CG_AD] = s0, st[CG_AD + 1] = s1, st[CG_AD + 2] = s2;
                    if (rowq[q] >= 0) pd += (double)(s0 * st[CG_D]) + (double)(s1 * st[CG_D + 1]) + (double)(s2 * st[CG_D + 2]);
                }
            }
            CG_TK(1);
            double dAd, unused;
            if (!all_sum(pd, 0.0, dAd, unused)) return;
            CG_TK(2);
            const double omega = zTr / dAd;
            const T wp = (T)omega, wm = (T)(-omega);
            double pz = 0;
            if (lane == 0) {
#pragma unroll
                for (int q = 0; q < RPW; ++q) {
                    T* st = cg_row[w][q];
                    T rr[3], zz[3];
#pragma unroll
                    for (int c = 0; c < 3; ++c) st[CG_U + c] += wp * st[CG_D + c], rr[c] = st[CG_R + c] + wm * st[CG_AD + c];
#pragma unroll
                    for (int c = 0; c < 3; ++c) zz[c] = st[CG_DI + c] * rr[0] + st[CG_DI + 3 + c] * rr[1] + st[CG_DI + 6 + c] * rr[2];
                    if (rowq[q] >= 0) pz += (double)(zz[0] * rr[0]) + (double)(zz[1] * rr[1]) + (double)(zz[2] * rr[2]);
#pragma unroll
                    for (int c = 0; c < 3; ++c) st[CG_R + c] = rr[c], st[CG_Z + c] = zz[c];
                }
            }
            CG_TK(3);
            double zTrNew;
            if (!all_sum(pz, 0.0, zTrNew, unused)) return;
            CG_TK(4);
            const T beta = (T)(zTrNew / zTr);
            if (lane == 0) {
#pragma unroll
                for (int q = 0; q < RPW; ++q) {
                    T* st = cg_row[w][q];
                    T dd[3];
#pragma unroll
                    for (int c = 0; c < 3; ++c) dd[c] = st[CG_Z + c] + beta * st[CG_D + c], st[CG_D + c] = dd[c];
                    if (rowq[q] >= 0)
                        for (int c = 0; c < 3; ++c) sdu(rowq[q], c, dd[c]);
                }
// ... 138 lines not shown
        const T w = ((q / 9 != 1) ? (T)0.5 : (T)1) * (((q / 3) % 3 != 1) ? (T)0.5 : (T)1) * ((q % 3 != 1) ? (T)0.5 : (T)1);
        s = (ci[q] < 0 || (fine_own && !fine_own[ci[q]])) ? s : s + w * fv[q];
    }
    coarse[e] = s;
}
template <class T>
__global__ void k_prolong(const int32_t* __restrict__ pcol, const T* __restrict__ pw, const T* __restrict__ coarse, T* fine, int n, const uint8_t* __restrict__ own)
{
    int e = blockIdx.x * blockDim.x + threadIdx.x;
    if (e >= 3 * n) return;
    int i = e / 3, d = e - 3 * i;
    if (own && !own[i]) return;
    T s = 0;
    for (int l = 0; l < 8; ++l) s += pw[8 * (int64_t)i + l] * coarse[3 * (int64_t)pcol[8 * (int64_t)i + l] + d];
    fine[e] = s;
}
template <class T>
int Ctx<T>::smoother_kind(int level, bool top) const
{
    const bool baseline = cfg.useBaselineMultigrid != 0;
    const int splitLevel = cfg.topDownMGS ? 1 : cfg.levelCnt - 1;
    return (level < splitLevel && !top) ? (baseline ? 5 : cfg.smoother) : (baseline ? 2 : cfg.coarseSolver);
}
template <class T>
bool Ctx<T>::gs_marks_wanted(int level) const
{
    return smoother_kind(level) == 5 && gs_plan(*levels[level]).marks;
}
template <class T>
void Ctx<T>::restrict_dev(int level, const T* fine, T* coarse, T* zero_coarse)
{
    Level<T>& C = *levels[level + 1];
    Level<T>& F = *levels[level];
    if (F.part && halo_mode()) {
        if (zero_coarse) zero(3 * (size_t)C.n, zero_coarse);
        if (C.part) {
            halo_gather(F, const_cast<T*>(fine));
            HOT_LAUNCH(this, "restrict", k_restrict<T>, div_up(3 * (size_t)C.n, 256), 256, 0, C.child.p, fine, coarse, C.n, C.own.p, (const uint8_t*)nullptr, (T*)nullptr);
        }
        else {
            HOT_LAUNCH(this, "restrict", k_restrict<T>, div_up(3 * (size_t)C.n, 256), 256, 0, C.child.p, fine, coarse, C.n, (const uint8_t*)nullptr, F.own.p, (T*)nullptr);
            CommTag tag(this, "coarse_vector_allreduce");
            c_allreduce(coarse, 3 * (int64_t)C.n, REAL, HOT_COMM_SUM, true);
        }
        return;
    }
    T* mark = gs_marks_wanted(level + 1) ? C.tmp.p : (T*)nullptr;
    HOT_LAUNCH(this, "restrict", k_restrict<T>, div_up(3 * (size_t)C.n, 256), 256, 0, C.child.p, fine, coarse, C.n, (const uint8_t*)nullptr, (const uint8_t*)nullptr, mark, zero_coarse);
    unset_level = mark ? level + 1 : -1;
}
template <class T>
void Ctx<T>::prolong_dev(int level, const T* coarse, T* fine)
{
    Level<T>& F = *levels[level];
    Level<T>& C = *levels[level + 1];
    const bool hm = F.part && halo_mode();
    if (hm && C.part) halo_gather(C, const_cast<T*>(coarse));
    HOT_LAUNCH(this, "prolong", k_prolong<T>, div_up(3 * (size_t)F.n, 256), 256, 0, F.pcol.p, F.pw.p, coarse, fine, F.n, hm ? F.own.p : (const uint8_t*)nullptr);
}

template <class T>
__global__ void k_scale(const T* __restrict__ D, const T* __restrict__ r, T* mr, int n)
{
    int i = blockIdx.x * blockDim.x + threadIdx.x;
    if (i >= n) return;
    const T* d = D + 9 * (int64_t)i;
    T a = r[3 * (int64_t)i], b = r[3 * (int64_t)i + 1], c = r[3 * (int64_t)i + 2];
    mr[3 * (int64_t)i] = d[0] * a + d[3] * b + d[6] * c;
    mr[3 * (int64_t)i + 1] = d[1] * a + d[4] * b + d[7] * c;
    mr[3 * (int64_t)i + 2] = d[2] * a + d[5] * b + d[8] * c;
}

template <class T>
__global__ void k_cheb_start(T* v, size_t n3)
{
    size_t e = (size_t)blockIdx.x * blockDim.x + threadIdx.x;
    if (e < n3) v[e] = ((((unsigned)e * 2654435761u) >> 16) & 1u) ? (T)1 : (T)-1;
}
template <class T>
__global__ void k_abs(T* v, size_t n3)
{
    size_t e = (size_t)blockIdx.x * blockDim.x + threadIdx.x;
    if (e < n3) v[e] = v[e] < 0 ? -v[e] : v[e];
}
template <class T>
__global__ void k_div1(T* v, T c, size_t n3)
{
    size_t e = (size_t)blockIdx.x * blockDim.x + threadIdx.x;
    if (e < n3) v[e] = v[e] / c;
}
template <class T>
void Ctx<T>::estimate_2norm(Level<T>& L, double tol)
{
    MaskScope mscope(this, halo_mode() ? L.mask() : nullptr);
    constexpr int MaxIters = 512;
    size_t n3 = 3 * (size_t)L.n;
    T *v = L.du.p, *x = L.dAu.p;
    HOT_LAUNCH(this, "cheb_start", k_cheb_start<T>, div_up(n3, 256), 256, 0, v, n3);
    spmv_dev(L, v, x);
    HOT_LAUNCH(this, "cheb_abs", k_abs<T>, div_up(n3, 256), 256, 0, x, n3);
    T e = (T)std::sqrt(dot_host(n3, x, x));
    if (e == 0) {
        L.lMin = L.lMax = 0;
        return;
    }
    HOT_LAUNCH(this, "cheb_div", k_div1<T>, div_up(n3, 256), 256, 0, x, e, n3);
    T e0 = 0;
    for (int iter = 0; iter < MaxIters && std::abs(e - e0) > (T)tol * e; ++iter) {
        e0 = e;
        spmv_dev(L, x, v);
        spmv_dev(L, v, x);
        T normx = (T)std::sqrt(dot_host(n3, x, x));
        e = normx / (T)std::sqrt(dot_host(n3, v, v));
        HOT_LAUNCH(this, "cheb_div", k_div1<T>, div_up(n3, 256), 256, 0, x, normx, n3);
    }
    L.lMax = e;
    L.lMin = L.lMax / 30;
}

template <class T>
void Ctx<T>::block_apply_dev(const T* D, const T* in, T* out, int n)
{
    HOT_LAUNCH(this, "diag_scale", k_scale<T>, div_up(n, 256), 256, 0, D, in, out, n);
}
template <class T>
void Ctx<T>::scale_dev(Level<T>& L, const T* in, T* out)
{
    HOT_LAUNCH(this, "diag_scale", k_scale<T>, div_up(L.n, 256), 256, 0, L.diagInv.p, in, out, L.n);
}

template <class T>
__global__ void k_cg_scalars(double* s, int what)
{
    if (what == 0) {
        s[2] = s[0] / s[1];
        s[3] = -s[2];
    }
    else {
        s[5] = s[4] / s[0];
        s[0] = s[4];
    }
}

template <class T>
void Ctx<T>::smooth_dev(int level, int kind, int iterations, T tolerance, T* u, T* r, T* du, T* dAu, bool final_residual)
{
    Level<T>& L = *levels[level];
    size_t n3 = 3 * (size_t)L.n;
    MaskScope mscope(this, halo_mode() ? L.mask() : nullptr);
    const bool tmp_marked = unset_level == level;
    unset_level = -1;
    auto Aproject = [&](T* v) {
        if (level == 0 && !cfg.systemBCProject) project_dev(v);
    };
    auto scaler = [&](const T* in, T* out) { scale_dev(L, in, out); };
    if (kind == 0) {
        for (; iterations--;) {
            scaler(r, du);
            scal(n3, (T)cfg.topomega, du);
            axpy(n3, (T)1, du, u);
            if (!final_residual && iterations == 0) break;
            spmv_dev(L, du, dAu);
            Aproject(dAu);
            axpy(n3, (T)-1, dAu, r);
        }
    }
    else if (kind == 1) {
        for (; iterations--;) {
            double rr = dot_host(n3, r, r);
            if (std::sqrt(rr) < (double)tolerance) break;
            scaler(r, du);
            spmv_dev(L, du, dAu);
            Aproject(dAu);
            double a = dot_host(n3, du, r), b = dot_host(n3, du, dAu);
            T omega = (T)(a / b);
            axpy(n3, omega, du, u);
            axpy(n3, -omega, dAu, r);
        }
    }
    else if (kind == 2) {
        T* z = L.tmp.p;
        double* s = dscal.p + 40;
        const bool cg_unfused = ab_flag("HOT_CG_UNFUSED");
        const bool fused = !cg_unfused && !(level == 0 && !cfg.systemBCProject) && !L.part;
        int cnt = 0;
        double zTrk = 0, tol = 0;
        if (fused && sizeof(T) == 8 && L.n <= 65536 && !gs_no_chain && !sharded() && !ab_flag("HOT_CG_LAUNCHES")) {
            const int G = std::min(std::min(ab_int("HOT_CG_WGS", 256), device_cus()), div_up(L.n, 16));
            const int cg_ss = ab_int("HOT_CG_SLOT_STRIDE", 32);
            if (!cg_dep.p || cg_bar_dirty || cg_G != G) {
                cg_dep.reserve((size_t)4 * 256 * cg_ss);
                HOT_LAUNCH(this, "gs_fill_unset", k_gs_fill_unset<double>, div_up((size_t)4 * 256 * cg_ss, 256), 256, 0, (size_t)4 * 256 * cg_ss, cg_dep.p);
                cg_bar_dirty = false, cg_G = G, cg_phase = 0;
            }
            const bool cg_resident = L.n <= 2 * 16 * G && 3 * (size_t)L.n * sizeof(double) <= 150 * 1024 && !ab_flag("HOT_CG_STREAM");
            if (cg_resident && !attr_cg_set) {
                HOT_HIP(hipFuncSetAttribute((const void*)k_cg_persist<T, 2>, hipFuncAttributeMaxDynamicSharedMemorySize, 150 * 1024));
                attr_cg_set = true;
            }
            if (cg_resident)
                HOT_LAUNCH(this, lname("cg_persistent", L.id).c_str(), (k_cg_persist<T, 2>), G, 1024, 3 * (size_t)L.n * sizeof(double), L.col.p, L.val.p, L.diagInv.p, L.initialResidual.p, u, r, z, du, dAu, L.n, iterations, cg_phase, cg_dep.p, cg_ss,
                    hscal + 40, hscal + 251, new_ticket(), (int*)(hscal + 250));
            else
                HOT_LAUNCH(this, lname("cg_persistent", L.id).c_str(), k_cg_persist<T>, G, 1024, 0, L.col.p, L.val.p, L.diagInv.p, L.initialResidual.p, u, r, z, du, dAu, L.n, iterations, cg_phase, cg_dep.p, cg_ss,
                    hscal + 40, hscal + 251, new_ticket(), (int*)(hscal + 250));
            wait_ticket();
            cnt = (int)hscal[41];
            if (ab_flag("HOT_CG_DBG"))
                fprintf(stderr, "cg_persistent level %d: %d rows, %d workgroups, %d iterations; ticks pull %.0f product %.0f barrier1 %.0f update %.0f barrier2 %.0f direction %.0f barrier3 %.0f\n", L.id, L.n, G, cnt,
                    hscal[48], hscal[49], hscal[50], hscal[51], hscal[52], hscal[53], hscal[54]);
            cg_phase = (cg_phase + 1u + 3u * (unsigned)cnt) & 3u;
            HOT_CHECK((unsigned)hscal[43] == cg_phase, HOT_ERR_DEVICE, "k_cg_persist passed another number of barriers than the host counts: the next launch would start on the wrong set of deposit slots");
            iterations = 0;
        }
        else if (fused) {
            scaler(L.initialResidual.p, z);
            dot_to(n3, z, L.initialResidual.p, s + 7);
            scaler(r, z);
            copy(n3, z, du);
            dot_to(n3, z, r, s);
            HOT_LAUNCH(this, "cg_setup", k_cg_setup<T>, 1, 1, 0, s, hscal + 40);
            int group = std::max(1, std::min(cg_group, 16));
            bool active = true;
            while (iterations > 0 && active) {
                const int g = std::min(group, iterations);
                for (int k = 0; k < g; ++k) {
                    HOT_LAUNCH(this, lname("spmv", L.id).c_str(), k_cg_spmv_dot<T>, div_up(L.n, 4), 256, 0, L.col.p, L.val.p, du, dAu, L.n, s, gred(div_up(L.n, 4)));
                    HOT_LAUNCH(this, "cg_update", k_cg_update<T>, div_up(L.n, 256), 256, 0, L.diagInv.p, du, dAu, u, r, z, L.n, s, gred(div_up(L.n, 256)));
                    const bool last = k + 1 == g;
                    HOT_LAUNCH(this, "cg_direction", k_cg_direction<T>, div_up(n3, 256), 256, 0, n3, z, du, s, hscal + 40, last ? hscal + 251 : (double*)nullptr, last ? new_ticket() : 0.0);
                }
                iterations -= g;
                wait_ticket();
                active = !(hscal[40] < hscal[42]);
                group = 2;
            }
            cnt = (int)hscal[41];
            cg_group = cnt;
            iterations = 0;
        }
        else {
            scaler(L.initialResidual.p, z);
            double zTrk0 = dot_host(n3, z, L.initialResidual.p);
            scaler(r, z);
            copy(n3, z, du);
            zTrk = dot_host(n3, z, r);
            tol = (double)(T)(zTrk0 * 0.25);
            HOT_HIP(hipMemcpyAsync(s, &zTrk, sizeof(double), hipMemcpyHostToDevice, stream));
        }
        for (; iterations-- > 0;) {
            if (zTrk < tol) break;
            spmv_dev(L, du, dAu);
            Aproject(dAu);
            dot_to(n3, dAu, du, s + 1);
            HOT_LAUNCH(this, "cg_scalars", k_cg_scalars<T>, 1, 1, 0, s, 0);
            axpy_dev(n3, s + 2, 1.0, du, u);
            axpy_dev(n3, s + 3, 1.0, dAu, r);
            scaler(r, z);
            dot_to(n3, z, r, s + 4);
            HOT_LAUNCH(this, "cg_scalars", k_cg_scalars<T>, 1, 1, 0, s, 1);
            HOT_LAUNCH(this, "xpay", k_xpay_dev<T>, div_up(n3, 256), 256, 0, n3, s + 5, z, du);
            HOT_HIP(hipMemcpyAsync(hscal + 40, s, sizeof(double), hipMemcpyDeviceToHost, stream));
            sync();
            zTrk = hscal[40];
            ++cnt;
        }
        stats.linear_iterations += cnt;
    }
    else if (kind == 6) {
        T* p = L.tmp.p;
        T d = (T)((L.lMax + L.lMin) / 2), c = (T)((L.lMax - L.lMin) / 2);
        int cnt = 1;
        iterations--;
        scaler(r, p);
        T alpha = 1 / d, beta;
        copy(n3, p, du);
        spmv_dev(L, du, dAu);
        Aproject(dAu);
        axpy(n3, alpha, du, u);
        axpy(n3, -alpha, dAu, r);
        for (; iterations-- > 0; ++cnt) {
            scaler(r, p);
            beta = (T)0.5 * c * c * alpha * alpha;
            if (cnt > 1) beta *= (T)0.5;
            alpha = 1 / (d - beta / alpha);
            scal(n3, beta, du);
            axpy(n3, (T)1, p, du);
            spmv_dev(L, du, dAu);
            Aproject(dAu);
            axpy(n3, alpha, du, u);
            if (!final_residual && iterations <= 0) break;
            axpy(n3, -alpha, dAu, r);
        }
    }
    else if (kind == 7)
        ic_smooth_dev(L, u, r, dAu);
    else if (kind == 5)
        gs_smooth_dev(level, iterations, u, r, du, dAu, final_residual, tmp_marked);
    else
        HOT_CHECK(false, HOT_ERR_INVALID, "unsupported smoother kind");
}

template <class T>
void Ctx<T>::vcycle_dev(const T* in, T* out)
{
    int levelCnt = (int)levels.size();
    int times = cfg.times, levelscale = cfg.levelscale;
    int splitLevel;
    auto downIter = [&](int level) { return times + level * levelscale; };
    auto upIter = [&](int level) { return cfg.topDownMGS ? 0 : times + level * levelscale; };
    const bool baseline = cfg.useBaselineMultigrid != 0;
    auto topIter = [&](int level) {
        if (cfg.topDownMGS || baseline) return 10000;
        if (cfg.levelCnt == 1) return times + level * levelscale;
        if (!(cfg.coarseSolver == 2 || cfg.coarseSolver == 6)) return (times + level * levelscale) * 3;
        return 10000;
    };
    splitLevel = cfg.topDownMGS ? 1 : cfg.levelCnt - 1;
    T tolTop = (T)(cfg.cneps * cfg.cneps);
    auto run = [&](bool regular, int level, T* sol, int its, bool final_residual = true) {
        Level<T>& L = *levels[level];
        smooth_dev(level, smoother_kind(level, !regular), its, regular ? (T)0 : tolTop, sol, L.residual.p, L.du.p, L.dAu.p, final_residual);
    };
    stats.vcycles++;
    Level<T>& L0 = *levels[0];
    size_t n0 = 3 * (size_t)L0.n;
    HOT_LAUNCH(this, "vcycle_start", k_vcycle_start<T>, (int)std::min<size_t>(div_up(n0, 256), 2048), 256, 0, n0, in, L0.residual.p, levelCnt > 1 ? (T*)nullptr : L0.initialResidual.p, out);
    if (levelCnt > 1) restrict_dev(0, L0.residual.p, levels[1]->initialResidual.p);
    for (int l = 1; l < levelCnt - 1; ++l) restrict_dev(l, levels[l]->initialResidual.p, levels[l + 1]->initialResidual.p);
    int level;
    for (level = 0; level < levelCnt - 1; ++level) {
        T* sol = level == 0 ? out : levels[level]->sol.p;
        run(level < splitLevel, level, sol, level < splitLevel ? upIter(level) : topIter(level));
        restrict_dev(level, levels[level]->residual.p, levels[level + 1]->residual.p, levels[level + 1]->sol.p);
    }
    run(false, level, level == 0 ? out : levels[level]->sol.p, topIter(level));
    for (--level; level >= 0; --level) {
        Level<T>& L = *levels[level];
        T* sol = level == 0 ? out : L.sol.p;
        size_t n3 = 3 * (size_t)L.n;
        prolong_dev(level, levels[level + 1]->sol.p, L.du.p);
        axpy(n3, (T)1, L.du.p, sol);
        const bool full_spmv = ab_flag("HOT_MG_FULL_SPMV");
        if (full_spmv) {
            spmv_dev(L, L.du.p, L.dAu.p);
            axpy(n3, (T)-1, L.dAu.p, L.residual.p);
        }
        else
        {
            T* mark = gs_marks_wanted(level) ? L.tmp.p : (T*)nullptr;
            HOT_LAUNCH(this, lname("apmv", L.id).c_str(), k_apmv_sub<T>, xcd_grid(div_up(L.n, 4)), 256, 0, L.apc.p, L.apv.p, levels[level + 1]->sol.p, L.residual.p, L.n, L.mask(), mark);
            unset_level = mark ? level : -1;
        }
        if (L.part && !halo_mode() && smoother_kind(level) != 5)
            exchange(L, L.residual.p, -1);
        run(level < splitLevel, level, sol, level < splitLevel ? downIter(level) : topIter(level), false);
    }
}

template <class T>
void Ctx<T>::precondition_dev(const T* in, T* out)
{
    HOT_CHECK(!levels.empty() && levels[0]->built, HOT_ERR_INVALID, "preconditioner used before hot_build_mg");
    vcycle_dev(in, out);
}

template <class T>
void Ctx<T>::spmv(int32_t level, const void* x, void* y)
{
    need(level >= 0 && level < (int)levels.size(), "level out of range");
    Level<T>& L = *levels[level];
    size_t n3 = 3 * (size_t)L.n;
    DBuf<T> a, b;
    a.reserve(n3), b.reserve(n3);
    HOT_HIP(hipMemcpyAsync(a.p, x, n3 * sizeof(T), hipMemcpyDefault, stream));
    spmv_dev(L, a.p, b.p);
    if (halo_mode()) gather_all(L, b.p);
    download(y, b.p, n3);
    sync();
}
template <class T>
void Ctx<T>::restrict_(int32_t level, const void* fine, void* coarse)
{
    need(level >= 0 && level + 1 < (int)levels.size(), "level out of range");
    size_t nf = 3 * (size_t)levels[level]->n, nc = 3 * (size_t)levels[level + 1]->n;
    DBuf<T> a, b;
    a.reserve(nf), b.reserve(nc);
    HOT_HIP(hipMemcpyAsync(a.p, fine, nf * sizeof(T), hipMemcpyDefault, stream));
    restrict_dev(level, a.p, b.p);
    if (halo_mode()) gather_all(*levels[level + 1], b.p);
    download(coarse, b.p, nc);
    sync();
}
template <class T>
void Ctx<T>::prolong(int32_t level, const void* coarse, void* fine)
{
    need(level >= 0 && level + 1 < (int)levels.size(), "level out of range");
    size_t nf = 3 * (size_t)levels[level]->n, nc = 3 * (size_t)levels[level + 1]->n;
    DBuf<T> a, b;
    a.reserve(nc), b.reserve(nf);
    HOT_HIP(hipMemcpyAsync(a.p, coarse, nc * sizeof(T), hipMemcpyDefault, stream));
    prolong_dev(level, a.p, b.p);
    if (halo_mode()) gather_all(*levels[level], b.p);
    download(fine, b.p, nf);
    sync();
}
template <class T>
void Ctx<T>::smooth(int32_t level, int32_t kind, int32_t iterations, double tol, void* u, void* r, const void* r0)
{
    need(level >= 0 && level < (int)levels.size() && levels[level]->built, "hot_smooth: level not built (hot_build_mg)");
    Level<T>& L = *levels[level];
    size_t n3 = 3 * (size_t)L.n;
    DBuf<T> du_, dr_, r0_;
    du_.reserve(n3), dr_.reserve(n3), r0_.reserve(n3);
    HOT_HIP(hipMemcpyAsync(r0_.p, r0 ? r0 : r, n3 * sizeof(T), hipMemcpyDefault, stream));
    with_gs_retry([&] {
        HOT_HIP(hipMemcpyAsync(du_.p, u, n3 * sizeof(T), hipMemcpyDefault, stream));
        HOT_HIP(hipMemcpyAsync(dr_.p, r, n3 * sizeof(T), hipMemcpyDefault, stream));
        HOT_HIP(hipMemcpyAsync(L.initialResidual.p, r0_.p, n3 * sizeof(T), hipMemcpyDeviceToDevice, stream));
        smooth_dev(level, kind, iterations, (T)tol, du_.p, dr_.p, L.du.p, L.dAu.p);
        if (halo_mode()) gather_all(L, du_.p), gather_all(L, dr_.p);
        sync();
    });
    download(u, du_.p, n3);
    download(r, dr_.p, n3);
    sync();
}
template <class T>
void Ctx<T>::vcycle(const void* in, void* out)
{
    need(!levels.empty() && levels[0]->built, "hot_vcycle before hot_build_mg");
    size_t n3 = 3 * (size_t)Nn;
    HOT_HIP(hipMemcpyAsync(work0.p, in, n3 * sizeof(T), hipMemcpyDefault, stream));
    with_gs_retry([&] {
        vcycle_dev(work0.p, work1.p);
        if (halo_mode()) gather_all(*levels[0], work1.p);
        sync();
    });
    download(out, work1.p, n3);
    sync();
}

template struct Ctx<float>;
template struct Ctx<double>;

}
```

### hot_amd/csrc/solve.hip

```cpp
#include "hot_impl.h"
#include "hot_svd.h"
#include "hot_collision.h"
#include <cmath>

namespace hot {

template <class T>
__global__ __launch_bounds__(256) void k_scaled_norm(const T* __restrict__ r, const T* __restrict__ tol, int nn, int useCN, double* out, GridRed gr, const uint8_t* __restrict__ mask)
{
    __shared__ double red[4];
    double s = 0;
    const int stride = gridDim.x * 256;
    for (int n0 = blockIdx.x * 256 + threadIdx.x; n0 < nn; n0 += 2 * stride) {
        const int n1 = n0 + stride < nn ? n0 + stride : n0;
        if (mask) {
            double q = 0;
            for (int u = 0; u < 2; ++u) {
                const int n = u ? n1 : n0;
                if ((u && n1 == n0) || !mask[n]) continue;
                const T a = r[3 * n], b = r[3 * n + 1], c = r[3 * n + 2], t = useCN ? tol[n] : (T)1;
                T qq = a * a + b * b + c * c;
                if (useCN) qq = qq / (t * t);
                q += (double)qq;
            }
            s += q;
            continue;
        }
        const T a0 = r[3 * n0], b0 = r[3 * n0 + 1], c0 = r[3 * n0 + 2], t0 = useCN ? tol[n0] : (T)1;
        const T a1 = r[3 * n1], b1 = r[3 * n1 + 1], c1 = r[3 * n1 + 2], t1 = useCN ? tol[n1] : (T)1;
        T q = a0 * a0 + b0 * b0 + c0 * c0;
        if (useCN) q = q / (t0 * t0);
        s += (double)q;
        if (n1 != n0) {
            T q1 = a1 * a1 + b1 * b1 + c1 * c1;
            if (useCN) q1 = q1 / (t1 * t1);
            s += (double)q1;
        }
    }
    double t = block_sum_256<double>(s, red);
    grid_sum_store(t, 0.0, 1, gr, out, nullptr, red);
}
template <class T>
__global__ void k_combine(size_t n, const T* __restrict__ a, T alpha, const T* __restrict__ b, T* out, T* out2)
{
    size_t i = (size_t)blockIdx.x * blockDim.x + threadIdx.x;
    if (i < n) out[i] = out2[i] = a[i] + b[i] * alpha;
}
template <class T>
__global__ void k_scal(size_t n, T alpha, T* x)
{
    size_t i = (size_t)blockIdx.x * blockDim.x + threadIdx.x;
    if (i < n) x[i] *= alpha;
}
__global__ void k_lbfgs_scalar(double* s, int i, int what)
{
    if (what == 0)
        s[50 + i] = s[70] * s[60 + i];
    else
        s[80] = s[50 + i] - s[70] * s[60 + i];
}

constexpr int LB_MAXV = 17;
constexpr int LB_B = 512, LB_E = 536, LB_G = 560, LB_M = 600;
template <class T>
struct LbVecs {
    const T* dx[8];
    const T* dg[8];
    int ph[8];
    int m;
};
template <class T>
__global__ __launch_bounds__(256) void k_lbfgs_dots(size_t n, LbVecs<T> hv, int use_dg, const T* __restrict__ y, double* out, GridRed gr, const uint8_t* __restrict__ mask)
{
    __shared__ double red[4 * 8];
    double acc[8];
#pragma unroll
    for (int k = 0; k < 8; ++k) acc[k] = 0;
    const size_t stride = (size_t)gridDim.x * 256;
    for (size_t i = (size_t)blockIdx.x * 256 + threadIdx.x; i < n; i += stride) {
        if (mask && !mask[i / 3]) continue;
        const T yv = y[i];
#pragma unroll
        for (int k = 0; k < 8; ++k)
            if (k < hv.m) acc[k] += (double)(use_dg ? hv.dg[k][i] : hv.dx[k][i]) * (double)yv;
    }
    const int m = hv.m;
    block_sum_256_n<8>(acc, [m](int k) { return k < m; }, red);
    grid_sum_store_n<8>(acc, [m](int k) { return k < m ? k : -1; }, m, gr, out, red);
}
template <class T>
__global__ __launch_bounds__(256) void k_lbfgs_apply(size_t n, double* s, LbVecs<T> hv, int mode, T* __restrict__ y, T* __restrict__ keep, const uint8_t* __restrict__ mask)
{
    __shared__ double coef[8];
    if (threadIdx.x == 0) {
        const int m = hv.m;
        double t[8];
        if (mode == 0) {
            for (int i = m - 1; i >= 0; --i) {
                double v = s[LB_B + i];
                for (int j = i + 1; j < m; ++j) v -= t[j] * s[LB_M + 9 * hv.ph[i] + hv.ph[j]];
                t[i] = v * s[60 + hv.ph[i]];
                coef[i] = -t[i];
                if (blockIdx.x == 0) s[50 + hv.ph[i]] = t[i];
            }
        }
        else {
            for (int i = 0; i < m; ++i) {
                double v = s[LB_E + i];
                for (int j = 0; j < i; ++j) v += t[j] * s[LB_M + 9 * hv.ph[j] + hv.ph[i]];
                t[i] = s[50 + hv.ph[i]] - s[60 + hv.ph[i]] * v;
                coef[i] = t[i];
            }
        }
    }
    __syncthreads();
    const size_t stride = (size_t)gridDim.x * 256;
    for (size_t i = (size_t)blockIdx.x * 256 + threadIdx.x; i < n; i += stride) {
        if (mask && !mask[i / 3]) continue;
        T v = y[i];
        if (keep) keep[i] = v;
        if (mode == 0) {
#pragma unroll
            for (int k = 7; k >= 0; --k)
                if (k < hv.m) v = v + (T)coef[k] * hv.dg[k][i];
        }
        else {
#pragma unroll
            for (int k = 0; k < 8; ++k)
                if (k < hv.m) v = v + (T)coef[k] * hv.dx[k][i];
        }
        y[i] = v;
    }
}
template <class T>
__global__ __launch_bounds__(256) void k_lbfgs_pair(size_t n, LbVecs<T> hv, const T* __restrict__ dxw, T* __restrict__ dgw, const T* __restrict__ rnew, double* out, GridRed gr, const uint8_t* __restrict__ mask)
{
    __shared__ double red[4 * LB_MAXV];
    double acc[LB_MAXV];
#pragma unroll
    for (int k = 0; k < LB_MAXV; ++k) acc[k] = 0;
    const size_t stride = (size_t)gridDim.x * 256;
    for (size_t i = (size_t)blockIdx.x * 256 + threadIdx.x; i < n; i += stride) {
        if (mask && !mask[i / 3]) continue;
        const T g = dgw[i] - rnew[i], x = dxw[i];
        dgw[i] = g;
        acc[0] += (double)g * (double)x;
#pragma unroll
        for (int k = 0; k < 8; ++k)
            if (k < hv.m) acc[1 + k] += (double)x * (double)hv.dg[k][i];
#pragma unroll
        for (int k = 0; k < 8; ++k)
            if (k < hv.m) acc[9 + k] += (double)hv.dx[k][i] * (double)g;
    }
    const int m = hv.m;
    block_sum_256_n<LB_MAXV>(acc, [m](int k) { return k == 0 || ((k - 1) & 7) < m; }, red);
    grid_sum_store_n<LB_MAXV>(acc, [m](int k) { return k == 0 ? 0 : (((k - 1) & 7) < m ? (k <= 8 ? k : k - 8 + m) : -1); }, 2 * m + 1, gr, out, red);
}
template <class T>
__global__ void k_lbfgs_file(double* s, LbVecs<T> hv, int wk, double* host_curv)
{
    const double* g = s + LB_G;
    s[71] = g[0];
    *host_curv = g[0];
    s[60 + wk] = (double)((T)1 / (T)g[0]);
    for (int j = 0; j < hv.m; ++j) s[LB_M + 9 * wk + hv.ph[j]] = g[1 + j], s[LB_M + 9 * hv.ph[j] + wk] = g[1 + hv.m + j];
}
template <class T>
__global__ void k_lbfgs_rho(double* s, int src, int dst)
{
    s[dst] = (double)((T)1 / (T)s[src]);
}

template <class T>
bool Ctx<T>::should_exit(const T* r)
{
    if (Nn == 0) return true;
    {
        const int grid = std::min(div_up(Nn, 512), 1024);
        HOT_LAUNCH(this, "exit_norm", k_scaled_norm<T>, grid, 256, 0, r, cnTol.p, Nn, cfg.useCN, dscal.p + 90, gred(grid, hscal + 90, true), vmask);
    }
    wait_ticket();
    if (vmask) c_allreduce(hscal + 90, 1, HOT_COMM_F64, HOT_COMM_SUM, false);
    double v = hscal[90];
    HOT_CHECK(v == v, HOT_ERR_NUMERIC, "NaN in the residual norm");
    if (!cfg.useCN) {
        double res = std::sqrt(v);
        stats.final_scaled_residual = res;
        return res < cfg.cneps;
    }
    stats.final_scaled_residual = std::sqrt(v / Nn);
    return (T)v < (T)Nn;
}

template <class T>
T Ctx<T>::line_search(T* ddv, T* residual_out, T alpha)
{
    size_t n3 = 3 * (size_t)Nn;
    T* dvnew = work3.p;
    transform_dev(ddv, true);
    const double Ek0 = Ek, Ek0_sigma = Ek_sigma;
    int guard = 0;
    const int eo_mode = cfg.ls_energy_only;
    bool eo = eo_mode == 2 || (eo_mode == 0 && ls_prev_trials > 1), last_eo = false;
    int trials = 0;
    const bool batched = !ab_flag("HOT_LS_NO_BATCH");
    bool last_from_batch = false;
    int batches = 0;
    do {
        if (eo && batched && guard + 2 <= 59) {
            const int pv = ls_prev_trials;
            int K = batches == 0 ? (pv <= 2 ? 2 : (pv <= 4 ? 4 : (pv <= 8 ? 8 : 16))) : 8;
            ++batches;
            while (guard + K > 59) K >>= 1;
            double Eb[16];
            trial_batch(ddv, alpha, K, Eb);
            int k = 0;
            for (;; ++k) {
                Ek = Eb[k];
                ++trials, stats.linesearch_trials++;
                if (ab_flag("HOT_DEBUG")) fprintf(stderr, "[hot]   linesearch alpha=%g Ek=%.12e Ek0=%.12e (batch of %d)\n", (double)alpha, Ek, Ek0, K);
                alpha *= (T)0.5;
                if (Ek <= Ek0_sigma || k == K - 1) break;
                ++guard;
            }
            last_eo = true, last_from_batch = true;
            continue;
        }
        last_from_batch = false;
        HOT_LAUNCH(this, "linesearch_combine", k_combine<T>, div_up(n3, 256), 256, 0, n3, dv0.p, alpha, ddv, dvnew, dv.p);
        Ek = state_pass(dv.p, false, eo);
        last_eo = eo;
        if (eo_mode != 1) eo = true;
        ++trials;
        stats.linesearch_trials++;
        alpha *= (T)0.5;
        if (ab_flag("HOT_DEBUG")) fprintf(stderr, "[hot]   linesearch alpha=%g Ek=%.12e Ek0=%.12e\n", (double)alpha * 2, Ek, Ek0);
    } while (!(Ek <= (last_eo ? Ek0_sigma : Ek0)) && ++guard < 60);
    if (last_from_batch)
        HOT_LAUNCH(this, "linesearch_combine", k_combine<T>, div_up(n3, 256), 256, 0, n3, dv0.p, alpha * 2, ddv, dvnew, dv.p);
    if (!(Ek == Ek)) {
        double dd = dot_host(n3, ddv, ddv), d0 = dot_host(n3, dv0.p, dv0.p);
        char msg[256];
        snprintf(msg, sizeof(msg), "NaN energy in line search (iteration %d, after %d halvings, |direction|^2 %g, |dv|^2 %g, E0 %g)", stats.iterations, guard, dd, d0, Ek0);
        HOT_CHECK(false, HOT_ERR_NUMERIC, msg);
    }
    alpha *= 2;
    ls_prev_trials = trials;
    if (last_eo) Ek = state_pass(dv.p, false, false);
    HOT_LAUNCH(this, "scal", k_scal<T>, div_up(n3, 256), 256, 0, n3, alpha, ddv);
    transform_dev(ddv, false);
    force_pass();
    residual_dev(residual_out);
    updated = true;
    std::swap(dv0.p, work3.p), std::swap(dv0.cap, work3.cap);
    return alpha;
}

template <class T>
bool Ctx<T>::lbfgs_solve()
{
    constexpr int historySize = 8;
    size_t n3 = 3 * (size_t)Nn;
    T* x = dv.p;
    T* residual = work2.p;
    for (int k = 0; k < historySize + 1; ++k) hist_dx[k].reserve(n3, 1.25), hist_dg[k].reserve(n3, 1.25);
    if (!updated) {
        Ek = state_pass(x, true);
        residual_dev(residual);
    }
    std::vector<int> order;
    std::vector<int> freeSlots;
    for (int k = historySize; k >= 0; --k) freeSlots.push_back(k);
    auto push_back = [&]() {
        if ((int)order.size() == historySize + 1) {
            freeSlots.push_back(order.front());
            order.erase(order.begin());
        }
        order.push_back(freeSlots.back());
        freeSlots.pop_back();
    };
    auto pop_back = [&]() {
        freeSlots.push_back(order.back());
        order.pop_back();
    };
    push_back();
    double* s = dscal.p;
    bool pending = false;
    auto resolve_pair = [&]() {
        if (!pending) return;
        pending = false;
        T dgTdx = (T)1 / (T)hscal[91];
        if (dgTdx <= (T)0 || !(dgTdx == dgTdx)) {
            if (!(dgTdx <= (T)0)) HOT_CHECK(false, HOT_ERR_NUMERIC, "NaN curvature in L-BFGS");
            pop_back();
            stats.dropped_pairs++;
        }
        push_back();
    };
    for (int it = 0; it < cfg.max_iterations; ++it) {
        stats.iterations = it;
        bool ex = should_exit(residual);
        resolve_pair();
        if (ab_flag("HOT_DEBUG")) fprintf(stderr, "[hot] lbfgs it=%d scaled_res=%.6e Ek=%.12e hist=%d\n", it, stats.final_scaled_residual, Ek, (int)order.size() - 1);
        if (ex) {
            stats.converged = 1;
            return true;
        }
        bool rebuild = cfg.useAdaptiveHessian ? ((it & 0xf) == 0) : (it == 0);
        if (rebuild) {
            build_hessian();
            build_mg();
            while (!order.empty()) pop_back();
            push_back();
        }
        int wk = order.back();
        const int m = (int)order.size() - 1;
        const bool unfused = ab_flag("HOT_LBFGS_UNFUSED");
#ifndef HOT_LB_PER_WG
#define HOT_LB_PER_WG 1024
#define HOT_LB_MAX_WG 1024
#endif
        const int vgrid = (int)std::min<size_t>(div_up(n3, HOT_LB_PER_WG), HOT_LB_MAX_WG);
        LbVecs<T> hv{};
        if (unfused) {
            copy(n3, residual, hist_dg[wk].p);
            for (int i = m - 1; i >= 0; --i) {
                int ph = order[i];
                dot_to(n3, hist_dx[ph].p, residual, s + 70);
                HOT_LAUNCH(this, "lbfgs_scalar", k_lbfgs_scalar, 1, 1, 0, s, ph, 0);
                axpy_dev(n3, s + 50 + ph, -1.0, hist_dg[ph].p, residual);
            }
        }
        else {
            for (int i = 0; i < m; ++i) hv.dx[i] = hist_dx[order[i]].p, hv.dg[i] = hist_dg[order[i]].p, hv.ph[i] = order[i];
            hv.m = m;
            if (m > 0) {
                HOT_LAUNCH(this, "lbfgs_dots", k_lbfgs_dots<T>, vgrid, 256, 0, n3, hv, 0, residual, s + LB_B, gred_n(vgrid, 8), vmask);
                reduce_scalars(s + LB_B, m);
            }
            HOT_LAUNCH(this, "lbfgs_apply", k_lbfgs_apply<T>, vgrid, 256, 0, n3, s, hv, 0, residual, hist_dg[wk].p, vmask);
        }
        precondition_dev(residual, hist_dx[wk].p);
        project_dev(hist_dx[wk].p);
        if (unfused) {
            for (int i = 0; i < m; ++i) {
                int ph = order[i];
                dot_to(n3, hist_dg[ph].p, hist_dx[wk].p, s + 70);
                HOT_LAUNCH(this, "lbfgs_scalar", k_lbfgs_scalar, 1, 1, 0, s, ph, 1);
                axpy_dev(n3, s + 80, 1.0, hist_dx[ph].p, hist_dx[wk].p);
            }
        }
        else if (m > 0) {
            HOT_LAUNCH(this, "lbfgs_dots", k_lbfgs_dots<T>, vgrid, 256, 0, n3, hv, 1, hist_dx[wk].p, s + LB_E, gred_n(vgrid, 8), vmask);
            reduce_scalars(s + LB_E, m);
            HOT_LAUNCH(this, "lbfgs_apply", k_lbfgs_apply<T>, vgrid, 256, 0, n3, s, hv, 1, hist_dx[wk].p, (T*)nullptr, vmask);
        }
        if (cfg.linesearch) line_search(hist_dx[wk].p, residual, (T)1);
        transform_dev(hist_dx[wk].p, true);
        axpy(n3, (T)1, hist_dx[wk].p, x);
        transform_dev(hist_dx[wk].p, false);
        if (!updated) {
            Ek = state_pass(x, true);
            residual_dev(residual);
        }
        if (unfused) {
            axpy(n3, (T)-1, residual, hist_dg[wk].p);
            dot_to(n3, hist_dg[wk].p, hist_dx[wk].p, s + 71, hscal + 91);
            HOT_LAUNCH(this, "lbfgs_rho", k_lbfgs_rho<T>, 1, 1, 0, s, 71, 60 + wk);
        }
        else {
            HOT_LAUNCH(this, "lbfgs_pair", k_lbfgs_pair<T>, vgrid, 256, 0, n3, hv, hist_dx[wk].p, hist_dg[wk].p, residual, s + LB_G, gred_n(vgrid, LB_MAXV), vmask);
            reduce_scalars(s + LB_G, 2 * m + 1);
            HOT_LAUNCH(this, "lbfgs_file", k_lbfgs_file<T>, 1, 1, 0, s, hv, wk, hscal + 91);
        }
        pending = true;
    }
    sync();
    resolve_pair();
    stats.iterations = cfg.max_iterations;
    return false;
}

template <class T>
__global__ void k_sub(size_t n, const T* __restrict__ a, const T* __restrict__ b, T* out)
{
    size_t i = (size_t)blockIdx.x * blockDim.x + threadIdx.x;
    if (i < n) out[i] = a[i] - b[i];
}

template <class T>
__global__ void k_mass_scale(const T* __restrict__ mass, const T* __restrict__ in, T* out, int nn)
{
    int e = blockIdx.x * blockDim.x + threadIdx.x;
    if (e >= 3 * nn) return;
    out[e] = in[e] * ((T)1 / mass[e / 3]);
}
template <class T>
__global__ void k_minres_comb(size_t n, T* y, T a, const T* __restrict__ x1, T b, const T* __restrict__ x2, T c)
{
    size_t i = (size_t)blockIdx.x * blockDim.x + threadIdx.x;
    if (i < n) y[i] = (y[i] - a * x1[i] - b * x2[i]) / c;
}
template <class T>
__global__ void k_div2(size_t n, T* y, T* z, T c)
{
    size_t i = (size_t)blockIdx.x * blockDim.x + threadIdx.x;
    if (i < n) y[i] = y[i] / c, z[i] = z[i] / c;
}

template <class T>
int Ctx<T>::minres_dev(const std::function<void(const T*, T*)>& Amul, const std::function<void(const T*, T*)>& prec, T* x, const T* b, T relative_tolerance, T tolerance, int max_iterations)
{
    size_t n3 = 3 * (size_t)Nn;
    DBuf<T> bufs[7];
    for (auto& v : bufs) v.reserve(n3), zero(n3, v.p);
    T *mk = bufs[0].p, *mkm1 = bufs[1].p, *mkm2 = bufs[2].p, *z = bufs[3].p, *qkm1 = bufs[4].p, *qk = bufs[5].p, *qkp1 = bufs[6].p;
    T gamma = 0, delta = 0, epsilon = 0, beta_kp1 = 0, alpha_k = 0, beta_k = 0, tk = 0;
    struct G2 {
        T c = 1, s = 0;
        void compute(T a, T b)
        {
            T d = a * a + b * b;
            c = 1, s = 0;
            T sq = std::sqrt(d);
            if (sq) {
                T t = 1 / sq;
                c = a * t, s = -b * t;
            }
        }
        void rot(T& a, T& b) const
        {
            T t1 = a, t2 = b;
            a = c * t1 - s * t2, b = s * t1 + c * t2;
        }
    } Gk, Gkm1, Gkm2;
    Amul(x, qkp1);
    HOT_LAUNCH(this, "sub", k_sub<T>, div_up(n3, 256), 256, 0, n3, b, qkp1, qkp1);
    project_dev(qkp1);
    prec(qkp1, z);
    T rpn = (T)std::sqrt(dot_host(n3, z, qkp1));
    beta_kp1 = rpn;
    HOT_CHECK(beta_kp1 == beta_kp1, HOT_ERR_NUMERIC, "NaN in MINRES");
    T local_tolerance = std::min(relative_tolerance * rpn, tolerance);
    if (rpn < local_tolerance) return 0;
    if (rpn > 0) HOT_LAUNCH(this, "minres_div", k_div2<T>, div_up(n3, 256), 256, 0, n3, qkp1, z, beta_kp1);
    T rhs0 = rpn, rhs1 = 0;
    for (int k = 0; k < max_iterations; ++k) {
        if (rpn < local_tolerance) return k;
        std::swap(mkm2, mkm1);
        std::swap(mkm1, mk);
        copy(n3, z, mk);
        beta_k = beta_kp1;
        std::swap(qkm1, qkp1);
        std::swap(qkm1, qk);
        Amul(mk, qkp1);
        project_dev(qkp1);
        alpha_k = (T)dot_host(n3, mk, qkp1);
        axpy(n3, -alpha_k, qk, qkp1);
        axpy(n3, -beta_k, qkm1, qkp1);
        prec(qkp1, z);
        beta_kp1 = (T)std::sqrt(std::max(0.0, dot_host(n3, z, qkp1)));
        if (beta_kp1 > 0) HOT_LAUNCH(this, "minres_div", k_div2<T>, div_up(n3, 256), 256, 0, n3, qkp1, z, beta_kp1);
        Gkm2 = Gkm1;
        Gkm1 = Gk;
        T e0 = 0, e1 = beta_k;
        Gkm2.rot(e0, e1);
        epsilon = e0;
        T d0 = e1, d1 = alpha_k;
        Gkm1.rot(d0, d1);
        delta = d0;
        T t0 = d1, t1 = beta_kp1;
        Gk.compute(t0, t1);
        Gk.rot(t0, t1);
        gamma = t0;
        Gk.rot(rhs0, rhs1);
        tk = rhs0;
        T res = rhs1;
        rhs0 = res, rhs1 = 0;
        rpn = res < 0 ? -res : res;
        HOT_LAUNCH(this, "minres_comb", k_minres_comb<T>, div_up(n3, 256), 256, 0, n3, mk, delta, mkm1, epsilon, mkm2, gamma);
        axpy(n3, tk, mk, x);
    }
    return max_iterations;
}

template <class T>
void Ctx<T>::compute_step_dev(const T* residual, T* step)
{
    size_t n3 = 3 * (size_t)Nn;
    DBuf<T>&r = nw_r, &p = nw_p, &q = nw_q, &temp = nw_t;
    r.reserve(n3, 1.25), p.reserve(n3, 1.25), q.reserve(n3, 1.25), temp.reserve(n3, 1.25);
    T cg_tolerance = cfg.useCN ? max_cn_tolerance : (T)1e-4;
    zero(n3, step);
    const bool massPrec = !cfg.matrixFree && (cfg.lsolver == 1 || cfg.lsolver == 2) && cfg.Ainv == 2;
    if (cfg.matrixFree) {
        nw_diag.reserve(9 * (size_t)Nn, 1.25);
        matfree_diagonal(nw_diag.p);
    }
    else {
        build_hessian();
        if (!massPrec) build_mg();
    }
    bool diagPrec = (cfg.levelCnt == 1 && cfg.times == 1);
    std::function<void(const T*, T*)> prec = [&](const T* in, T* out) {
        if (cfg.matrixFree)
            block_apply_dev(nw_diag.p, in, out, Nn);
        else if (massPrec)
            HOT_LAUNCH(this, "mass_scale", k_mass_scale<T>, div_up(n3, 256), 256, 0, mass.p, in, out, Nn);
        else if (diagPrec)
            scale_dev(*levels[0], in, out);
        else
            vcycle_dev(in, out);
    };
    std::function<void(const T*, T*)> Amul = [&](const T* xx, T* bb) {
        if (cfg.matrixFree)
            matfree_dev(xx, bb);
        else
            spmv_dev(*levels[0], xx, bb);
    };
    if (cfg.lsolver == 1) {
        T residual_norm = (T)std::sqrt(dot_host(n3, residual, residual));
        T newton_tol = cfg.useCN ? max_cn_tolerance : (T)cfg.cneps;
        T rel = std::min((T)0.5, (T)std::sqrt(std::max(residual_norm, newton_tol)));
        stats.linear_iterations += minres_dev(Amul, prec, step, residual, rel, cg_tolerance, cfg.linear_iteration_cap > 0 ? cfg.linear_iteration_cap : 10000);
        return;
    }
    Amul(step, temp.p);
    HOT_LAUNCH(this, "sub", k_sub<T>, div_up(n3, 256), 256, 0, n3, residual, temp.p, r.p);
    project_dev(r.p);
    prec(r.p, q.p);
    copy(n3, q.p, p.p);
    double zTrk = dot_host(n3, r.p, q.p);
    T rpn = (T)std::sqrt(zTrk);
    T forcing = std::min((T)0.5, (T)std::sqrt(std::max(rpn, cg_tolerance)));
    T local_tol = forcing * rpn;
    int cnt = 0;
    for (; cnt < (cfg.linear_iteration_cap > 0 ? cfg.linear_iteration_cap : 10000); ++cnt) {
        if (rpn < local_tol) break;
        Amul(p.p, temp.p);
        project_dev(temp.p);
        T alpha = (T)(zTrk / dot_host(n3, temp.p, p.p));
        axpy(n3, alpha, p.p, step);
        axpy(n3, -alpha, temp.p, r.p);
        prec(r.p, q.p);
        double zlast = zTrk;
        zTrk = dot_host(n3, q.p, r.p);
        T beta = (T)(zTrk / zlast);
        HOT_LAUNCH(this, "scal", k_scal<T>, div_up(n3, 256), 256, 0, n3, beta, p.p);
        axpy(n3, (T)1, q.p, p.p);
        rpn = (T)std::sqrt(zTrk);
    }
    stats.linear_iterations += cnt;
}

template <class T>
bool Ctx<T>::newton_solve()
{
    size_t n3 = 3 * (size_t)Nn;
    T* x = dv.p;
    T* residual = work2.p;
    nw_step.reserve(n3, 1.25);
    for (int it = 0; it < cfg.max_iterations; ++it) {
        stats.iterations = it;
        if (!updated) {
            Ek = state_pass(x, true);
            residual_dev(residual);
        }
        if (should_exit(residual)) {
            stats.converged = 1;
            return true;
        }
        compute_step_dev(residual, nw_step.p);
        if (cfg.linesearch) line_search(nw_step.p, residual, (T)1);
        transform_dev(nw_step.p, true);
        axpy(n3, (T)1, nw_step.p, x);
        transform_dev(nw_step.p, false);
    }
    stats.iterations = cfg.max_iterations;
    return false;
}

template <class T>
void Ctx<T>::line_search_api(void* ddv, void* residual, double alpha, double* alpha_out)
{
    need(Nn > 0 && dt > 0, "hot_line_search before hot_begin_step / hot_update_state");
    size_t n3 = 3 * (size_t)Nn;
    HOT_HIP(hipMemcpyAsync(work0.p, ddv, n3 * sizeof(T), hipMemcpyDefault, stream));
    T a = line_search(work0.p, work1.p, (T)alpha);
    if (halo_mode()) gather_all(*levels[0], work0.p), gather_all(*levels[0], work1.p);
    download(ddv, work0.p, n3), download(residual, work1.p, n3);
    sync();
    if (alpha_out) *alpha_out = (double)a;
}
template <class T>
void Ctx<T>::should_exit_api(const void* residual, int32_t* exit_now, double* scaled)
{
    need(Nn > 0 && dt > 0, "hot_should_exit before hot_begin_step");
    if (cfg.useCN) cn_tolerance_dev();
    HOT_HIP(hipMemcpyAsync(work0.p, residual, 3 * (size_t)Nn * sizeof(T), hipMemcpyDefault, stream));
    bool e = should_exit(work0.p);
    if (exit_now) *exit_now = e ? 1 : 0;
    if (scaled) *scaled = stats.final_scaled_residual;
}
template <class T>
void Ctx<T>::transform_api(void* v, bool inverse)
{
    need(Nn > 0, "no grid");
    HOT_HIP(hipMemcpyAsync(work0.p, v, 3 * (size_t)Nn * sizeof(T), hipMemcpyDefault, stream));
    transform_dev(work0.p, inverse);
    download(v, work0.p, 3 * (size_t)Nn);
    sync();
}
template <class T>
void Ctx<T>::compute_step_api(const void* residual, void* step)
{
    need(Nn > 0 && dt > 0, "hot_compute_step before hot_update_state");
    need(cfg.lsolver == 1 || cfg.lsolver == 2, "hot_compute_step is the projected-Newton step (lsolver 1 / 2)");
    size_t n3 = 3 * (size_t)Nn;
    if (cfg.useCN) cn_tolerance_dev();
    nw_step.reserve(n3, 1.25);
    HOT_HIP(hipMemcpyAsync(work2.p, residual, n3 * sizeof(T), hipMemcpyDefault, stream));
    with_gs_retry([&] {
        release_levels(halo_mode() ? 1 : 0);
        compute_step_dev(work2.p, nw_step.p);
        if (halo_mode()) gather_all(*levels[0], nw_step.p);
        sync();
    });
    download(step, nw_step.p, n3);
    sync();
}

template <class T>
void Ctx<T>::solve(hot_stats* st)
{
    need(Nn > 0 && dt > 0, "hot_solve before hot_begin_step");
    need(cfg.lsolver == 1 || cfg.lsolver == 2 || cfg.lsolver == 3, "lsolver must be 1 (PN + MINRES), 2 (PN + PCG) or 3 (L-BFGS); 0 performs no linear solve in the reference and 4 is the SimplicialLLT direct solver (out of scope)");
    need(!(cfg.matrixFree && cfg.lsolver == 3), "matrixFree applies to the projected-Newton solvers (lsolver 1 / 2)");
    need(!(cfg.Ainv == 2 && cfg.lsolver == 3), "Ainv 2 (lumped-mass preconditioner) applies to lsolver 1 / 2 (Configurations.h:30)");
    double keep_sort = stats.ms_sort, keep_p2g = stats.ms_p2g, keep_begin = stats.ms_begin;
    std::memset(&stats, 0, sizeof(stats));
    stats.ms_sort = keep_sort, stats.ms_p2g = keep_p2g, stats.ms_begin = keep_begin;
    double t0 = wall_ms();
    if (cfg.useCN) cn_tolerance_dev();
    const size_t n3 = 3 * (size_t)Nn;
    solve_keep.reserve(2 * n3, 1.25);
    copy(n3, dv.p, solve_keep.p), copy(n3, dv0.p, solve_keep.p + n3);
    const double Ek_in = Ek;
    const hot_stats stats_in = stats;
    bool first_try = true;
    with_gs_retry([&] {
        if (!first_try) {
            copy(n3, solve_keep.p, dv.p), copy(n3, solve_keep.p + n3, dv0.p);
            updated = false, Ek = Ek_in, stats = stats_in;
        }
        first_try = false;
        release_levels(halo_mode() ? 1 : 0);
        if (cfg.lsolver == 3)
            lbfgs_solve();
        else
            newton_solve();
        sync();
    });
    prof.collect();
    stats.num_nodes = Nn;
    stats.num_levels = (halo_mode() && cfg.matrixFree) ? 0 : (int)levels.size();
    stats.energy = cfg.linesearch ? Ek : 0.0;
    stats.ms_solve = wall_ms() - t0;
    export_comm_stats();
    if (st) *st = stats;
}

template <class T>
void Ctx<T>::advance(double dt_, hot_stats* st)
{
    double t0 = wall_ms();
    sort();
// ... 108 lines not shown
```

Measured before the change: 3.089 ms/iter.

## Fuse inertia, exit norm, projection, prolongation and vcycle start into neighboring kernels

```diff
diff --git a/hot_amd/csrc/force.hip b/hot_amd/csrc/force.hip
--- a/hot_amd/csrc/force.hip
+++ b/hot_amd/csrc/force.hip
@@ -614,6 +614,43 @@
 }
 
 template <class T>
+__global__ __launch_bounds__(256) void k_combine_inertia(const T* __restrict__ dv0, T alpha, const T* __restrict__ ddv, T* __restrict__ out, T* __restrict__ out2, const T* __restrict__ mass, int nn, T g0, T g1, T g2, double* sums, GridRed gr)
+{
+    __shared__ double red[4];
+    double ke = 0, ge = 0;
+    const int stride = gridDim.x * 256;
+    for (int n0 = blockIdx.x * 256 + threadIdx.x; n0 < nn; n0 += 4 * stride) {
+        T a[4], b[4], c[4], m[4];
+#pragma unroll
+        for (int u = 0; u < 4; ++u) {
+            const bool on = n0 + u * stride < nn;
+            const int n = on ? n0 + u * stride : n0;
+            a[u] = dv0[3 * n] + ddv[3 * n] * alpha, b[u] = dv0[3 * n + 1] + ddv[3 * n + 1] * alpha, c[u] = dv0[3 * n + 2] + ddv[3 * n + 2] * alpha, m[u] = mass[n];
+            if (on) {
+                out[3 * n] = out2[3 * n] = a[u];
+                out[3 * n + 1] = out2[3 * n + 1] = b[u];
+                out[3 * n + 2] = out2[3 * n + 2] = c[u];
+            }
+        }
+#pragma unroll
+        for (int u = 0; u < 4; ++u)
+            if (n0 + u * stride < nn) {
+                ke += (double)((a[u] * a[u] + b[u] * b[u] + c[u] * c[u]) * m[u]);
+                ge += (double)((g0 * a[u] + g1 * b[u] + g2 * c[u]) * m[u]);
+            }
+    }
+    double k = block_sum_256<double>(ke, red);
+    double gg = block_sum_256<double>(ge, red);
+    grid_sum_store(k, gg, 2, gr, sums, sums + 1, red);
+}
+template <class T>
+void Ctx<T>::combine_inertia(T alpha, const T* ddv, T* dvnew)
+{
+    const int grid = std::min(div_up(Nn, 1024), 1024);
+    HOT_LAUNCH(this, "linesearch_combine", k_combine_inertia<T>, grid, 256, 0, dv0.p, alpha, ddv, dvnew, dv.p, mass.p, Nn, (T)cfg.gravity[0], (T)cfg.gravity[1], (T)cfg.gravity[2], dscal.p + 1, gred(grid, hscal + 1));
+}
+
+template <class T>
 __global__ __launch_bounds__(256) void k_force_cells2(const T* __restrict__ X, const T* __restrict__ stress, int64_t Np, const int32_t* __restrict__ group_first,
     const int32_t* __restrict__ group_origin, const int32_t* __restrict__ group_cell0, const int32_t* __restrict__ cell_first, T* __restrict__ part, T one_over_dx, T scale)
 {
@@ -816,17 +853,21 @@
 }
 
 template <class T>
-double Ctx<T>::state_pass(const T* dv_in, bool want_force, bool energy_only)
+double Ctx<T>::state_pass(const T* dv_in, bool want_force, bool energy_only, bool inertia_done )
 {
     if (halo_mode()) halo_gather(*levels[0], const_cast<T*>(dv_in));
     if (energy_only)
         HOT_LAUNCH(this, "state_energy", (k_state<T, true>), Ng, 256, 0, pX.p, pFn.p, pVol.p, pMu.p, pLam.p, (T*)nullptr, (T*)nullptr, (T*)nullptr, Np, group_first.p, group_origin.p,
             group_nb.p, tileDof.p, vn.p, dv_in, dx, (T)1 / dx, dt, dscal.p, gred(Ng, hscal));
-    else
+    else {
+        GridRed g2 = gred2(Ng, hscal, hscal + 3);
+        if (inertia_done) g2.ticket = hscal + 251, g2.ticket_val = new_ticket();
         HOT_LAUNCH(this, "state_update", (k_state<T, false>), Ng, 256, 0, pX.p, pFn.p, pVol.p, pMu.p, pLam.p, pFt.p, pStress.p, keep_debug ? pGradV.p : (T*)nullptr, Np, group_first.p, group_origin.p,
-            group_nb.p, tileDof.p, vn.p, dv_in, dx, (T)1 / dx, dt, dscal.p, gred2(Ng, hscal, hscal + 3));
+            group_nb.p, tileDof.p, vn.p, dv_in, dx, (T)1 / dx, dt, dscal.p, g2);
+    }
+    HOT_CHECK(!inertia_done || (!energy_only && !want_force && !vmask && !sharded()), HOT_ERR_INVALID, "state_pass: the inertia sums ride with the trial point on the full, one-rank trial only");
     if (want_force) force_pass();
-    {
+    if (!inertia_done) {
         const int grid = std::min(div_up(Nn, 1024), 1024);
         HOT_LAUNCH(this, "inertia_energy", k_inertia_energy<T>, grid, 256, 0, dv_in, mass.p, Nn, (T)cfg.gravity[0], (T)cfg.gravity[1], (T)cfg.gravity[2], dscal.p + 1, gred(grid, hscal + 1, true), vmask);
     }
@@ -882,29 +923,6 @@
 }
 
 template <class T>
-__device__ __forceinline__ void mat3_vec(const T* __restrict__ M, const T* v, T* o)
-{
-    o[0] = M[0] * v[0] + M[3] * v[1] + M[6] * v[2];
-    o[1] = M[1] * v[0] + M[4] * v[1] + M[7] * v[2];
-    o[2] = M[2] * v[0] + M[5] * v[1] + M[8] * v[2];
-}
-template <class T>
-__device__ __forceinline__ void bc_project(int c, const T* __restrict__ P, const uint8_t* __restrict__ slip, bool slipmode, T* v)
-{
-    if (slipmode) {
-        if (slip[c])
-            v[0] = (T)0;
-        else
-            v[0] = v[1] = v[2] = (T)0;
-    }
-    else {
-        T o[3];
-        mat3_vec(P + 9 * c, v, o);
-        v[0] = o[0], v[1] = o[1], v[2] = o[2];
-    }
-}
-
-template <class T>
 __global__ void k_residual(const T* __restrict__ gF, const int32_t* __restrict__ dofSlot, const T* __restrict__ mass, const T* __restrict__ dv, const int32_t* __restrict__ bcIdx,
     const T* __restrict__ bcP, const T* __restrict__ bcR, const uint8_t* __restrict__ bcSlip, T* r, T* r2 , int nn, int64_t slots, T g0, T g1, T g2, T dt, int slipmode)
 {
@@ -926,6 +944,51 @@
     r2[3 * n] = v[0], r2[3 * n + 1] = v[1], r2[3 * n + 2] = v[2];
 }
 template <class T>
+__global__ __launch_bounds__(256) void k_residual_norm(const T* __restrict__ gF, const int32_t* __restrict__ dofSlot, const T* __restrict__ mass, const T* __restrict__ dv, const int32_t* __restrict__ bcIdx,
+    const T* __restrict__ bcP, const T* __restrict__ bcR, const uint8_t* __restrict__ bcSlip, T* __restrict__ r, T* __restrict__ r2, int nn, int64_t slots, T g0, T g1, T g2, T dt, int slipmode, const T* __restrict__ tol, int useCN,
+    double* out, GridRed gr)
+{
+    __shared__ double red[4];
+    double sum = 0;
+    const int stride = gridDim.x * 256;
+    for (int n0 = blockIdx.x * 256 + threadIdx.x; n0 < nn; n0 += 2 * stride) {
+        const int n1 = n0 + stride < nn ? n0 + stride : n0;
+        T w[2][3], t[2];
+#pragma unroll
+        for (int u = 0; u < 2; ++u) {
+            const int n = u ? n1 : n0;
+            int64_t s = dofSlot[n];
+            T m = mass[n];
+            T v[3] = { g0 * dt * m + gF[s] - dv[3 * n] * m, g1 * dt * m + gF[slots + s] - dv[3 * n + 1] * m, g2 * dt * m + gF[2 * slots + s] - dv[3 * n + 2] * m };
+            int c = bcIdx[n];
+            if (c >= 0) {
+                if (slipmode && bcSlip[c]) {
+                    T o[3];
+                    mat3_vec(bcR + 9 * c, v, o);
+                    v[0] = o[0], v[1] = o[1], v[2] = o[2];
+                }
+                bc_project(c, bcP, bcSlip, slipmode != 0, v);
+            }
+            w[u][0] = v[0], w[u][1] = v[1], w[u][2] = v[2];
+            t[u] = useCN ? tol[n] : (T)1;
+            if (u == 0 || n1 != n0) {
+                r[3 * n] = v[0], r[3 * n + 1] = v[1], r[3 * n + 2] = v[2];
+                r2[3 * n] = v[0], r2[3 * n + 1] = v[1], r2[3 * n + 2] = v[2];
+            }
+        }
+        T q = w[0][0] * w[0][0] + w[0][1] * w[0][1] + w[0][2] * w[0][2];
+        if (useCN) q = q / (t[0] * t[0]);
+        sum += (double)q;
+        if (n1 != n0) {
+            T q1 = w[1][0] * w[1][0] + w[1][1] * w[1][1] + w[1][2] * w[1][2];
+            if (useCN) q1 = q1 / (t[1] * t[1]);
+            sum += (double)q1;
+        }
+    }
+    double tt = block_sum_256<double>(sum, red);
+    grid_sum_store(tt, 0.0, 1, gr, out, nullptr, red);
+}
+template <class T>
 __global__ void k_project(const int32_t* __restrict__ bcNode, const T* __restrict__ bcP, const uint8_t* __restrict__ bcSlip, T* v, int nc, int slipmode)
 {
     int c = blockIdx.x * blockDim.x + threadIdx.x;
@@ -947,9 +1010,16 @@
 }
 
 template <class T>
-void Ctx<T>::residual_dev(T* r)
+void Ctx<T>::residual_dev(T* r, bool with_norm , bool ticket )
 {
     int slipmode = (cfg.systemBCProject && cfg.boundaryType == 1) ? 1 : 0;
+    if (with_norm) {
+        HOT_CHECK(!vmask && !sharded(), HOT_ERR_INVALID, "residual_dev: the exit norm rides with the residual on one rank only");
+        const int grid = std::min(div_up(Nn, 512), 1024);
+        HOT_LAUNCH(this, "residual", k_residual_norm<T>, grid, 256, 0, gF.p, dofSlot.p, mass.p, dv.p, bcIdx.p, bcP.p, bcR.p, bcSlip.p, r, rhs.p, Nn, (int64_t)Nb * EPB, (T)cfg.gravity[0], (T)cfg.gravity[1], (T)cfg.gravity[2], dt,
+            slipmode, cnTol.p, cfg.useCN, dscal.p + 90, gred(grid, hscal + 90, ticket));
+        return;
+    }
     HOT_LAUNCH(this, "residual", k_residual<T>, div_up(Nn, 256), 256, 0, gF.p, dofSlot.p, mass.p, dv.p, bcIdx.p, bcP.p, bcR.p, bcSlip.p, r, rhs.p, Nn, (int64_t)Nb * EPB, (T)cfg.gravity[0],
         (T)cfg.gravity[1], (T)cfg.gravity[2], dt, slipmode);
 }
diff --git a/hot_amd/csrc/hot_impl.h b/hot_amd/csrc/hot_impl.h
--- a/hot_amd/csrc/hot_impl.h
+++ b/hot_amd/csrc/hot_impl.h
@@ -335,6 +335,7 @@
     bool attr_tiles_set = false, attr_rows_set = false, attr_rows_det_set = false, attr_gs_set = false, attr_winv_set = false;
     double* hscal = nullptr;
     DBuf<T> hist_dx[9], hist_dg[9];
+    DBuf<T> lb_z0;
     std::vector<Level<T>*> levels;
     std::vector<Level<T>*> level_pool[12];
     Level<T>* acquire_level(int id)
@@ -497,9 +498,10 @@
     void eval_halfspaces();
     void eval_collision_objects();
     void trial_batch(const T* ddv, T alpha, int K, double* Ek_out);
-    double state_pass(const T* dv_in, bool want_force, bool energy_only = false);
+    double state_pass(const T* dv_in, bool want_force, bool energy_only = false, bool inertia_done = false);
+    void combine_inertia(T alpha, const T* ddv, T* dvnew);
     void force_pass();
-    void residual_dev(T* r);
+    void residual_dev(T* r, bool with_norm = false, bool ticket = false);
     void project_dev(T* v);
     void transform_dev(T* v, bool inverse);
     void cn_tolerance_dev();
@@ -522,8 +524,8 @@
     void smooth_dev(int level, int kind, int iterations, T tol, T* u, T* r, T* du, T* dAu, bool final_residual = true);
     void gs_smooth_dev(int level, int iterations, T* u, T* r, T* du, T* dAu, bool final_residual, bool tmp_marked);
     void ic_smooth_dev(Level<T>& L, T* u, T* r, T* dAu);
-    void vcycle_dev(const T* in, T* out);
-    void precondition_dev(const T* in, T* out);
+    void vcycle_dev(const T* in, T* out, bool started = false);
+    void precondition_dev(const T* in, T* out, bool started = false);
     void matfree_dev(const T* x, T* y);
     void axpy(size_t n, T a, const T* x, T* y);
     void axpy_dev(size_t n, const double* a, double sign, const T* x, T* y);
@@ -531,8 +533,8 @@
     void zero(size_t n, T* y);
     void dot_to(size_t n, const T* x, const T* y, double* out, double* mirror = nullptr);
     double dot_host(size_t n, const T* x, const T* y);
-    bool should_exit(const T* r);
-    T line_search(T* ddv, T* residual_out, T alpha);
+    bool should_exit(const T* r, bool have_norm = false);
+    T line_search(T* ddv, T* residual_out, T alpha, bool norm_with_residual = false);
     bool lbfgs_solve();
     bool newton_solve();
     void compute_step_dev(const T* residual, T* step);
@@ -575,6 +577,29 @@
 template <class T>
 __global__ void k_gs_fill_unset(size_t n, T* x);
 
+template <class T>
+__device__ __forceinline__ void mat3_vec(const T* __restrict__ M, const T* v, T* o)
+{
+    o[0] = M[0] * v[0] + M[3] * v[1] + M[6] * v[2];
+    o[1] = M[1] * v[0] + M[4] * v[1] + M[7] * v[2];
+    o[2] = M[2] * v[0] + M[5] * v[1] + M[8] * v[2];
+}
+template <class T>
+__device__ __forceinline__ void bc_project(int c, const T* __restrict__ P, const uint8_t* __restrict__ slip, bool slipmode, T* v)
+{
+    if (slipmode) {
+        if (slip[c])
+            v[0] = (T)0;
+        else
+            v[0] = v[1] = v[2] = (T)0;
+    }
+    else {
+        T o[3];
+        mat3_vec(P + 9 * c, v, o);
+        v[0] = o[0], v[1] = o[1], v[2] = o[2];
+    }
+}
+
 #define HOT_LAUNCH(ctx, name, kernel, grid, block, shmem, ...)                       \
     do {                                                                             \
         (ctx)->prof.begin(name, (ctx)->stream);                                      \
diff --git a/hot_amd/csrc/mg_solve.hip b/hot_amd/csrc/mg_solve.hip
--- a/hot_amd/csrc/mg_solve.hip
+++ b/hot_amd/csrc/mg_solve.hip
@@ -127,13 +127,19 @@
 }
 template <class T>
 __global__ __launch_bounds__(256) void k_apmv_sub(const int32_t* __restrict__ apc, const T* __restrict__ apv, const T* __restrict__ e, T* __restrict__ r, int n, const uint8_t* __restrict__ own,
-    T* unset )
+    T* unset ,
+    const int32_t* __restrict__ pcol = nullptr, const T* __restrict__ pw = nullptr, T* __restrict__ sol = nullptr )
 {
     const int lane = threadIdx.x & 63;
     const int row = xcd_block() * 4 + (threadIdx.x >> 6);
     if (row >= n) return;
     if (unset && lane < 3) gs_store_unset(unset + 3 * (int64_t)row + lane);
     if (own && !own[row]) return;
+    if (sol && lane < 3) {
+        T s = 0;
+        for (int l = 0; l < 8; ++l) s += pw[8 * (int64_t)row + l] * e[3 * (int64_t)pcol[8 * (int64_t)row + l] + lane];
+        sol[3 * (int64_t)row + lane] += s;
+    }
     const int j = nt_load(apc + (int64_t)row * 64 + lane);
     const int slot = __popcll(__ballot(j >= 0) & ((1ull << lane) - 1ull));
     T s0 = (T)0, s1 = (T)0, s2 = (T)0;
@@ -878,7 +884,7 @@
 }
 
 template <class T>
-void Ctx<T>::vcycle_dev(const T* in, T* out)
+void Ctx<T>::vcycle_dev(const T* in, T* out, bool started )
 {
     int levelCnt = (int)levels.size();
     int times = cfg.times, levelscale = cfg.levelscale;
@@ -901,7 +907,9 @@
     stats.vcycles++;
     Level<T>& L0 = *levels[0];
     size_t n0 = 3 * (size_t)L0.n;
-    HOT_LAUNCH(this, "vcycle_start", k_vcycle_start<T>, (int)std::min<size_t>(div_up(n0, 256), 2048), 256, 0, n0, in, L0.residual.p, levelCnt > 1 ? (T*)nullptr : L0.initialResidual.p, out);
+    HOT_CHECK(!started || levelCnt > 1, HOT_ERR_INVALID, "vcycle_dev: a single level's start also writes the top solver's initial residual");
+    if (!started)
+        HOT_LAUNCH(this, "vcycle_start", k_vcycle_start<T>, (int)std::min<size_t>(div_up(n0, 256), 2048), 256, 0, n0, in, L0.residual.p, levelCnt > 1 ? (T*)nullptr : L0.initialResidual.p, out);
     if (levelCnt > 1) restrict_dev(0, L0.residual.p, levels[1]->initialResidual.p);
     for (int l = 1; l < levelCnt - 1; ++l) restrict_dev(l, levels[l]->initialResidual.p, levels[l + 1]->initialResidual.p);
     int level;
@@ -915,9 +923,12 @@
         Level<T>& L = *levels[level];
         T* sol = level == 0 ? out : L.sol.p;
         size_t n3 = 3 * (size_t)L.n;
-        prolong_dev(level, levels[level + 1]->sol.p, L.du.p);
-        axpy(n3, (T)1, L.du.p, sol);
         const bool full_spmv = ab_flag("HOT_MG_FULL_SPMV");
+        const bool fold_prolong = !full_spmv && !L.part && !sharded() && !vmask && !ab_flag("HOT_MG_PROLONG_LAUNCHES");
+        if (!fold_prolong) {
+            prolong_dev(level, levels[level + 1]->sol.p, L.du.p);
+            axpy(n3, (T)1, L.du.p, sol);
+        }
         if (full_spmv) {
             spmv_dev(L, L.du.p, L.dAu.p);
             axpy(n3, (T)-1, L.dAu.p, L.residual.p);
@@ -925,7 +936,8 @@
         else
         {
             T* mark = gs_marks_wanted(level) ? L.tmp.p : (T*)nullptr;
-            HOT_LAUNCH(this, lname("apmv", L.id).c_str(), k_apmv_sub<T>, xcd_grid(div_up(L.n, 4)), 256, 0, L.apc.p, L.apv.p, levels[level + 1]->sol.p, L.residual.p, L.n, L.mask(), mark);
+            HOT_LAUNCH(this, lname("apmv", L.id).c_str(), k_apmv_sub<T>, xcd_grid(div_up(L.n, 4)), 256, 0, L.apc.p, L.apv.p, levels[level + 1]->sol.p, L.residual.p, L.n, L.mask(), mark,
+                fold_prolong ? L.pcol.p : (const int32_t*)nullptr, fold_prolong ? L.pw.p : (const T*)nullptr, fold_prolong ? sol : (T*)nullptr);
             unset_level = mark ? level : -1;
         }
         if (L.part && !halo_mode() && smoother_kind(level) != 5)
@@ -935,10 +947,10 @@
 }
 
 template <class T>
-void Ctx<T>::precondition_dev(const T* in, T* out)
+void Ctx<T>::precondition_dev(const T* in, T* out, bool started)
 {
     HOT_CHECK(!levels.empty() && levels[0]->built, HOT_ERR_INVALID, "preconditioner used before hot_build_mg");
-    vcycle_dev(in, out);
+    vcycle_dev(in, out, started);
 }
 
 template <class T>
diff --git a/hot_amd/csrc/solve.hip b/hot_amd/csrc/solve.hip
--- a/hot_amd/csrc/solve.hip
+++ b/hot_amd/csrc/solve.hip
@@ -62,6 +62,7 @@
 
 constexpr int LB_MAXV = 17;
 constexpr int LB_B = 512, LB_E = 536, LB_G = 560, LB_M = 600;
+constexpr int LB_PV = LB_MAXV + 9;
 template <class T>
 struct LbVecs {
     const T* dx[8];
@@ -69,8 +70,29 @@
     int ph[8];
     int m;
 };
-template <class T>
-__global__ __launch_bounds__(256) void k_lbfgs_dots(size_t n, LbVecs<T> hv, int use_dg, const T* __restrict__ y, double* out, GridRed gr, const uint8_t* __restrict__ mask)
+struct LbSrc {
+    int b[8];
+};
+template <class T>
+struct LbProj {
+    const int32_t* idx;
+    const T* P;
+    const uint8_t* slip;
+    int slipmode;
+};
+template <class T>
+__device__ __forceinline__ T lb_projected(const LbProj<T>& bc, const T* __restrict__ y, size_t i, T v)
+{
+    if (!bc.idx) return v;
+    const size_t n = i / 3;
+    const int d = (int)(i - 3 * n), c = bc.idx[n];
+    if (c < 0) return v;
+    T x[3] = { y[3 * n], y[3 * n + 1], y[3 * n + 2] };
+    bc_project(c, bc.P, bc.slip, bc.slipmode != 0, x);
+    return d == 0 ? x[0] : (d == 1 ? x[1] : x[2]);
+}
+template <class T>
+__global__ __launch_bounds__(256) void k_lbfgs_dots(size_t n, LbVecs<T> hv, int use_dg, const T* __restrict__ y, double* out, GridRed gr, const uint8_t* __restrict__ mask, LbProj<T> bc)
 {
     __shared__ double red[4 * 8];
     double acc[8];
@@ -79,7 +101,7 @@
     const size_t stride = (size_t)gridDim.x * 256;
     for (size_t i = (size_t)blockIdx.x * 256 + threadIdx.x; i < n; i += stride) {
         if (mask && !mask[i / 3]) continue;
-        const T yv = y[i];
+        const T yv = lb_projected(bc, y, i, y[i]);
 #pragma unroll
         for (int k = 0; k < 8; ++k)
             if (k < hv.m) acc[k] += (double)(use_dg ? hv.dg[k][i] : hv.dx[k][i]) * (double)yv;
@@ -89,7 +111,8 @@
     grid_sum_store_n<8>(acc, [m](int k) { return k < m ? k : -1; }, m, gr, out, red);
 }
 template <class T>
-__global__ __launch_bounds__(256) void k_lbfgs_apply(size_t n, double* s, LbVecs<T> hv, int mode, T* __restrict__ y, T* __restrict__ keep, const uint8_t* __restrict__ mask)
+__global__ __launch_bounds__(256) void k_lbfgs_apply(size_t n, double* s, LbVecs<T> hv, int mode, const T* yin, T* y, T* __restrict__ keep, const uint8_t* __restrict__ mask, LbSrc src, LbProj<T> bc,
+    T* __restrict__ y2 , T* __restrict__ zero_out )
 {
     __shared__ double coef[8];
     if (threadIdx.x == 0) {
@@ -97,7 +120,7 @@
         double t[8];
         if (mode == 0) {
             for (int i = m - 1; i >= 0; --i) {
-                double v = s[LB_B + i];
+                double v = s[src.b[i]];
                 for (int j = i + 1; j < m; ++j) v -= t[j] * s[LB_M + 9 * hv.ph[i] + hv.ph[j]];
                 t[i] = v * s[60 + hv.ph[i]];
                 coef[i] = -t[i];
@@ -117,8 +140,9 @@
     const size_t stride = (size_t)gridDim.x * 256;
     for (size_t i = (size_t)blockIdx.x * 256 + threadIdx.x; i < n; i += stride) {
         if (mask && !mask[i / 3]) continue;
-        T v = y[i];
+        T v = yin[i];
         if (keep) keep[i] = v;
+        if (mode != 0) v = lb_projected(bc, yin, i, v);
         if (mode == 0) {
 #pragma unroll
             for (int k = 7; k >= 0; --k)
@@ -130,19 +154,22 @@
                 if (k < hv.m) v = v + (T)coef[k] * hv.dx[k][i];
         }
         y[i] = v;
-    }
-}
-template <class T>
-__global__ __launch_bounds__(256) void k_lbfgs_pair(size_t n, LbVecs<T> hv, const T* __restrict__ dxw, T* __restrict__ dgw, const T* __restrict__ rnew, double* out, GridRed gr, const uint8_t* __restrict__ mask)
-{
-    __shared__ double red[4 * LB_MAXV];
-    double acc[LB_MAXV];
-#pragma unroll
-    for (int k = 0; k < LB_MAXV; ++k) acc[k] = 0;
+        if (y2) y2[i] = v;
+        if (zero_out) zero_out[i] = (T)0;
+    }
+}
+template <class T>
+__global__ __launch_bounds__(256) void k_lbfgs_pair(size_t n, LbVecs<T> hv, const T* __restrict__ dxw, T* __restrict__ dgw, const T* __restrict__ rnew, double* out, GridRed gr, const uint8_t* __restrict__ mask, int with_b)
+{
+    __shared__ double red[4 * LB_PV];
+    double acc[LB_PV];
+#pragma unroll
+    for (int k = 0; k < LB_PV; ++k) acc[k] = 0;
     const size_t stride = (size_t)gridDim.x * 256;
     for (size_t i = (size_t)blockIdx.x * 256 + threadIdx.x; i < n; i += stride) {
         if (mask && !mask[i / 3]) continue;
-        const T g = dgw[i] - rnew[i], x = dxw[i];
+        const T rn = rnew[i];
+        const T g = dgw[i] - rn, x = dxw[i];
         dgw[i] = g;
         acc[0] += (double)g * (double)x;
 #pragma unroll
@@ -151,19 +178,28 @@
 #pragma unroll
         for (int k = 0; k < 8; ++k)
             if (k < hv.m) acc[9 + k] += (double)hv.dx[k][i] * (double)g;
+        if (with_b) {
+#pragma unroll
+            for (int k = 0; k < 8; ++k)
+                if (k < hv.m) acc[17 + k] += (double)hv.dx[k][i] * (double)rn;
+            acc[25] += (double)x * (double)rn;
+        }
     }
     const int m = hv.m;
-    block_sum_256_n<LB_MAXV>(acc, [m](int k) { return k == 0 || ((k - 1) & 7) < m; }, red);
-    grid_sum_store_n<LB_MAXV>(acc, [m](int k) { return k == 0 ? 0 : (((k - 1) & 7) < m ? (k <= 8 ? k : k - 8 + m) : -1); }, 2 * m + 1, gr, out, red);
-}
-template <class T>
-__global__ void k_lbfgs_file(double* s, LbVecs<T> hv, int wk, double* host_curv)
+    block_sum_256_n<LB_PV>(acc, [m, with_b](int k) { return k == 0 || (k <= 16 && ((k - 1) & 7) < m) || (with_b && (k == 25 || (k >= 17 && k - 17 < m))); }, red);
+    grid_sum_store_n<LB_PV>(
+        acc, [m, with_b](int k) { return k == 0 ? 0 : (k <= 16 ? (((k - 1) & 7) < m ? (k <= 8 ? k : k - 8 + m) : -1) : (!with_b ? -1 : (k == 25 ? 3 * m + 1 : (k - 17 < m ? 2 * m + 1 + k - 17 : -1)))); },
+        with_b ? 3 * m + 2 : 2 * m + 1, gr, out, red);
+}
+template <class T>
+__global__ void k_lbfgs_file(double* s, LbVecs<T> hv, int wk, double* host_curv, double* ticket , double ticket_val)
 {
     const double* g = s + LB_G;
     s[71] = g[0];
     *host_curv = g[0];
     s[60 + wk] = (double)((T)1 / (T)g[0]);
     for (int j = 0; j < hv.m; ++j) s[LB_M + 9 * wk + hv.ph[j]] = g[1 + j], s[LB_M + 9 * hv.ph[j] + wk] = g[1 + hv.m + j];
+    if (ticket) host_ticket_store(ticket, ticket_val);
 }
 template <class T>
 __global__ void k_lbfgs_rho(double* s, int src, int dst)
@@ -172,10 +208,10 @@
 }
 
 template <class T>
-bool Ctx<T>::should_exit(const T* r)
+bool Ctx<T>::should_exit(const T* r, bool have_norm)
 {
     if (Nn == 0) return true;
-    {
+    if (!have_norm) {
         const int grid = std::min(div_up(Nn, 512), 1024);
         HOT_LAUNCH(this, "exit_norm", k_scaled_norm<T>, grid, 256, 0, r, cnTol.p, Nn, cfg.useCN, dscal.p + 90, gred(grid, hscal + 90, true), vmask);
     }
@@ -193,7 +229,7 @@
 }
 
 template <class T>
-T Ctx<T>::line_search(T* ddv, T* residual_out, T alpha)
+T Ctx<T>::line_search(T* ddv, T* residual_out, T alpha, bool norm_with_residual)
 {
     size_t n3 = 3 * (size_t)Nn;
     T* dvnew = work3.p;
@@ -227,8 +263,12 @@
             continue;
         }
         last_from_batch = false;
-        HOT_LAUNCH(this, "linesearch_combine", k_combine<T>, div_up(n3, 256), 256, 0, n3, dv0.p, alpha, ddv, dvnew, dv.p);
-        Ek = state_pass(dv.p, false, eo);
+        const bool inertia_here = !eo && !vmask && !sharded() && !ab_flag("HOT_LS_INERTIA_LAUNCH");
+        if (inertia_here)
+            combine_inertia(alpha, ddv, dvnew);
+        else
+            HOT_LAUNCH(this, "linesearch_combine", k_combine<T>, div_up(n3, 256), 256, 0, n3, dv0.p, alpha, ddv, dvnew, dv.p);
+        Ek = state_pass(dv.p, false, eo, inertia_here);
         last_eo = eo;
         if (eo_mode != 1) eo = true;
         ++trials;
@@ -247,10 +287,11 @@
     alpha *= 2;
     ls_prev_trials = trials;
     if (last_eo) Ek = state_pass(dv.p, false, false);
-    HOT_LAUNCH(this, "scal", k_scal<T>, div_up(n3, 256), 256, 0, n3, alpha, ddv);
+    if (alpha != (T)1 || ab_flag("HOT_LS_SCAL_ALWAYS"))
+        HOT_LAUNCH(this, "scal", k_scal<T>, div_up(n3, 256), 256, 0, n3, alpha, ddv);
     transform_dev(ddv, false);
     force_pass();
-    residual_dev(residual_out);
+    residual_dev(residual_out, norm_with_residual);
     updated = true;
     std::swap(dv0.p, work3.p), std::swap(dv0.cap, work3.cap);
     return alpha;
@@ -264,9 +305,13 @@
     T* x = dv.p;
     T* residual = work2.p;
     for (int k = 0; k < historySize + 1; ++k) hist_dx[k].reserve(n3, 1.25), hist_dg[k].reserve(n3, 1.25);
+    const bool unfused = ab_flag("HOT_LBFGS_UNFUSED");
+    const bool norm_fused = !unfused && !vmask && !sharded() && !ab_flag("HOT_EXIT_NORM_LAUNCH");
+    bool have_norm = false;
     if (!updated) {
         Ek = state_pass(x, true);
-        residual_dev(residual);
+        residual_dev(residual, norm_fused, norm_fused);
+        have_norm = norm_fused;
     }
     std::vector<int> order;
     std::vector<int> freeSlots;
@@ -297,9 +342,15 @@
         }
         push_back();
     };
+    int pair_m = -1, pair_wk = -1, pair_ph[8] = {};
+    const bool b_in_pair = !vmask && !sharded() && !ab_flag("HOT_LBFGS_DOTS_LAUNCH");
+    const bool fold_project = !vmask && !sharded() && Nc > 0 && !ab_flag("HOT_LBFGS_PROJECT_LAUNCH");
+    if (fold_project) lb_z0.reserve(n3, 1.25);
+    const int slipmode = (cfg.systemBCProject && cfg.boundaryType == 1) ? 1 : 0;
     for (int it = 0; it < cfg.max_iterations; ++it) {
         stats.iterations = it;
-        bool ex = should_exit(residual);
+        bool ex = should_exit(residual, have_norm);
+        have_norm = false;
         resolve_pair();
         if (ab_flag("HOT_DEBUG")) fprintf(stderr, "[hot] lbfgs it=%d scaled_res=%.6e Ek=%.12e hist=%d\n", it, stats.final_scaled_residual, Ek, (int)order.size() - 1);
         if (ex) {
@@ -312,16 +363,17 @@
             build_mg();
             while (!order.empty()) pop_back();
             push_back();
+            pair_m = -1;
         }
         int wk = order.back();
         const int m = (int)order.size() - 1;
-        const bool unfused = ab_flag("HOT_LBFGS_UNFUSED");
 #ifndef HOT_LB_PER_WG
 #define HOT_LB_PER_WG 1024
 #define HOT_LB_MAX_WG 1024
 #endif
         const int vgrid = (int)std::min<size_t>(div_up(n3, HOT_LB_PER_WG), HOT_LB_MAX_WG);
         LbVecs<T> hv{};
+        LbSrc src{};
         if (unfused) {
             copy(n3, residual, hist_dg[wk].p);
             for (int i = m - 1; i >= 0; --i) {
@@ -334,14 +386,29 @@
         else {
             for (int i = 0; i < m; ++i) hv.dx[i] = hist_dx[order[i]].p, hv.dg[i] = hist_dg[order[i]].p, hv.ph[i] = order[i];
             hv.m = m;
-            if (m > 0) {
-                HOT_LAUNCH(this, "lbfgs_dots", k_lbfgs_dots<T>, vgrid, 256, 0, n3, hv, 0, residual, s + LB_B, gred_n(vgrid, 8), vmask);
+            bool have_b = b_in_pair && pair_m >= 0;
+            for (int i = 0; i < m; ++i) {
+                int from = -1;
+                if (order[i] == pair_wk) from = LB_G + 3 * pair_m + 1;
+                for (int j = 0; j < pair_m; ++j)
+                    if (pair_ph[j] == order[i]) from = LB_G + 2 * pair_m + 1 + j;
+                have_b = have_b && from >= 0;
+                src.b[i] = from;
+            }
+            if (m > 0 && !have_b) {
+                for (int i = 0; i < m; ++i) src.b[i] = LB_B + i;
+                HOT_LAUNCH(this, "lbfgs_dots", k_lbfgs_dots<T>, vgrid, 256, 0, n3, hv, 0, residual, s + LB_B, gred_n(vgrid, 8), vmask, LbProj<T>{});
                 reduce_scalars(s + LB_B, m);
             }
-            HOT_LAUNCH(this, "lbfgs_apply", k_lbfgs_apply<T>, vgrid, 256, 0, n3, s, hv, 0, residual, hist_dg[wk].p, vmask);
-        }
-        precondition_dev(residual, hist_dx[wk].p);
-        project_dev(hist_dx[wk].p);
+        }
+        const bool proj_in_loop = fold_project && !unfused && m > 0;
+        T* z0 = proj_in_loop ? lb_z0.p : hist_dx[wk].p;
+        const bool start_here = !unfused && !vmask && !sharded() && levels.size() > 1 && !ab_flag("HOT_VCYCLE_START_LAUNCH");
+        if (!unfused)
+            HOT_LAUNCH(this, "lbfgs_apply", k_lbfgs_apply<T>, vgrid, 256, 0, n3, s, hv, 0, (const T*)residual, residual, hist_dg[wk].p, vmask, src, LbProj<T>{}, start_here ? levels[0]->residual.p : (T*)nullptr,
+                start_here ? z0 : (T*)nullptr);
+        precondition_dev(residual, z0, start_here);
+        if (!proj_in_loop) project_dev(z0);
         if (unfused) {
             for (int i = 0; i < m; ++i) {
                 int ph = order[i];
@@ -351,17 +418,19 @@
             }
         }
         else if (m > 0) {
-            HOT_LAUNCH(this, "lbfgs_dots", k_lbfgs_dots<T>, vgrid, 256, 0, n3, hv, 1, hist_dx[wk].p, s + LB_E, gred_n(vgrid, 8), vmask);
+            const LbProj<T> bc = proj_in_loop ? LbProj<T>{ bcIdx.p, bcP.p, bcSlip.p, slipmode } : LbProj<T>{};
+            HOT_LAUNCH(this, "lbfgs_dots", k_lbfgs_dots<T>, vgrid, 256, 0, n3, hv, 1, (const T*)z0, s + LB_E, gred_n(vgrid, 8), vmask, bc);
             reduce_scalars(s + LB_E, m);
-            HOT_LAUNCH(this, "lbfgs_apply", k_lbfgs_apply<T>, vgrid, 256, 0, n3, s, hv, 1, hist_dx[wk].p, (T*)nullptr, vmask);
-        }
-        if (cfg.linesearch) line_search(hist_dx[wk].p, residual, (T)1);
+            HOT_LAUNCH(this, "lbfgs_apply", k_lbfgs_apply<T>, vgrid, 256, 0, n3, s, hv, 1, (const T*)z0, hist_dx[wk].p, (T*)nullptr, vmask, LbSrc{}, bc, (T*)nullptr, (T*)nullptr);
+        }
+        if (cfg.linesearch) line_search(hist_dx[wk].p, residual, (T)1, norm_fused), have_norm = norm_fused;
         transform_dev(hist_dx[wk].p, true);
         axpy(n3, (T)1, hist_dx[wk].p, x);
         transform_dev(hist_dx[wk].p, false);
         if (!updated) {
             Ek = state_pass(x, true);
-            residual_dev(residual);
+            residual_dev(residual, norm_fused);
+            have_norm = norm_fused;
         }
         if (unfused) {
             axpy(n3, (T)-1, residual, hist_dg[wk].p);
@@ -369,9 +438,14 @@
             HOT_LAUNCH(this, "lbfgs_rho", k_lbfgs_rho<T>, 1, 1, 0, s, 71, 60 + wk);
         }
         else {
-            HOT_LAUNCH(this, "lbfgs_pair", k_lbfgs_pair<T>, vgrid, 256, 0, n3, hv, hist_dx[wk].p, hist_dg[wk].p, residual, s + LB_G, gred_n(vgrid, LB_MAXV), vmask);
+            HOT_LAUNCH(this, "lbfgs_pair", k_lbfgs_pair<T>, vgrid, 256, 0, n3, hv, hist_dx[wk].p, hist_dg[wk].p, residual, s + LB_G, gred_n(vgrid, LB_PV), vmask, b_in_pair ? 1 : 0);
             reduce_scalars(s + LB_G, 2 * m + 1);
-            HOT_LAUNCH(this, "lbfgs_file", k_lbfgs_file<T>, 1, 1, 0, s, hv, wk, hscal + 91);
+            if (b_in_pair) {
+                pair_m = m, pair_wk = wk;
+                for (int i = 0; i < m; ++i) pair_ph[i] = order[i];
+            }
+            const bool stamp = have_norm;
+            HOT_LAUNCH(this, "lbfgs_file", k_lbfgs_file<T>, 1, 1, 0, s, hv, wk, hscal + 91, stamp ? hscal + 251 : (double*)nullptr, stamp ? new_ticket() : 0.0);
         }
         pending = true;
     }
```

Result: slower. 3.127 ms/iter (+1.2%).
